# k2-fsa/Flow2GAN

Hardware: AMD Instinct MI355X
Metric: audio-seconds/sec (train step, G+D fwd/bwd) mel_24k_base (higher is better)
Workload: dtype f32 (fp32-class products on the bf16 matrix pipe for the long reductions and the direct MRD convs: every fp32 operand as three bf16 pieces = 24 significand bits, the six v_mfma_f32_32x32x16_bf16 products with i + j <= 2 per fp32 product, fp32 accumulate, error <= 2^-23 per product; short reductions ; 1 GPU; mel_24k_base GAN stage-2 train step: D-step + G-step, each on its own batch (MPD+MRD+FM+multi-scale mel), fwd+bwd+grad all-reduce, no optimizer (metric is fwd/bwd); per_gpu_batch=64, gan=gan_multi_scale_mel_recon, parallelism=dp1, optimizer=none

## Files before the change

### flow2gan_amd/csrc/multi.hip

```cpp
#include "common.h"
#include "split_f16.h"

namespace {

__device__ __forceinline__ void run_fill(const f2g_multi_entry& e, long long b, long long nb) {
  float* x = reinterpret_cast<float*>(e.out);
  const long long n = ((long long)e.n[1] << 32) | (unsigned)e.n[0];
  const float v = __int_as_float((int)e.s[0]);
  for (long long i = b * 256 + threadIdx.x; i < n; i += nb * 256) x[i] = v;
}

__device__ __forceinline__ void run_permute4(const f2g_multi_entry& e, long long b, long long nb) {
  float* out = reinterpret_cast<float*>(e.out);
  const float* in = reinterpret_cast<const float*>(e.in);
  const int n1 = e.n[1], n2 = e.n[2], n3 = e.n[3];
  const long long total = (long long)e.n[0] * n1 * n2 * n3;
  for (long long i = b * 256 + threadIdx.x; i < total; i += nb * 256) {
    long long r = i;
    const int i3 = (int)(r % n3); r /= n3;
    const int i2 = (int)(r % n2); r /= n2;
    const int i1 = (int)(r % n1); r /= n1;
    out[i] = in[r * e.s[0] + i1 * e.s[1] + i2 * e.s[2] + i3 * e.s[3]];
  }
}

__device__ __forceinline__ void run_copy3(const f2g_multi_entry& e, long long b, long long nb) {
  float* out = reinterpret_cast<float*>(e.out);
  const float* in = reinterpret_cast<const float*>(e.in);
  const int n1 = e.n[1], n2 = e.n[2], acc = e.n[3];
  const long long total = (long long)e.n[0] * n1 * n2;
  for (long long i = b * 256 + threadIdx.x; i < total; i += nb * 256) {
    const int c = (int)(i % n2);
    const long long q = i / n2;
    const int r = (int)(q % n1);
    const long long bb = q / n1;
    const float v = in[bb * e.s[2] + r * e.s[3] + c];
    float* o = out + bb * e.s[0] + r * e.s[1] + c;
    *o = acc ? *o + v : v;
  }
}

__device__ __forceinline__ void run_split3(const f2g_multi_entry& e, long long b, long long nb) {
  __bf16* dst = reinterpret_cast<__bf16*>(e.out);
  const float* src = reinterpret_cast<const float*>(e.in);
  const int K = e.n[1];
  const long long rows = e.n[0], ld = e.s[0], total = rows * (K / 4);
  for (long long i = b * 256 + threadIdx.x; i < total; i += nb * 256) {
    const long long r = i / (K / 4);
    const int k4 = (int)(i - r * (K / 4)) * 4;
    const float4 v = *reinterpret_cast<const float4*>(src + r * ld + k4);
    const float x[4] = {v.x, v.y, v.z, v.w};
    unsigned short p[3][4];
#pragma unroll
    for (int q = 0; q < 4; ++q) {
      const __bf16 a = (__bf16)x[q];
      const float r1 = x[q] - (float)a;
      const __bf16 c = (__bf16)r1;
      const __bf16 d = (__bf16)(r1 - (float)c);
      p[0][q] = __builtin_bit_cast(unsigned short, a);
      p[1][q] = __builtin_bit_cast(unsigned short, c);
      p[2][q] = __builtin_bit_cast(unsigned short, d);
    }
    __bf16* o = dst + (r * (K / 32) + k4 / 32) * 96 + (k4 & 31);
#pragma unroll
    for (int q = 0; q < 3; ++q)
      *reinterpret_cast<uint2*>(o + 32 * q) =
          make_uint2(p[q][0] | ((unsigned)p[q][1] << 16), p[q][2] | ((unsigned)p[q][3] << 16));
  }
}

__device__ __forceinline__ void run_split3g(const f2g_multi_entry& e, long long b, long long nb) {
  unsigned char* dst = reinterpret_cast<unsigned char*>(e.out);
  const float* src = reinterpret_cast<const float*>(e.in);
  const int K = e.n[1], K8 = K / 8, T = K / 32;
  const long long rows = e.n[0], ld = e.s[0], total = rows * K8;
  for (long long i = b * 256 + threadIdx.x; i < total; i += nb * 256) {
    const int li = (int)(i & 31);
    const long long q = i >> 5;
    const int c8 = (int)(q % K8);
    const long long j = q / K8;
    const float* p = src + (j * 32 + li) * ld + c8 * 8;
    const float4 v0 = *reinterpret_cast<const float4*>(p), v1 = *reinterpret_cast<const float4*>(p + 4);
    unsigned a[3], bq[3], c[3], dq[3];
    f2g_split3_pair(v0.x, v0.y, a[0], a[1], a[2]);
    f2g_split3_pair(v0.z, v0.w, bq[0], bq[1], bq[2]);
    f2g_split3_pair(v1.x, v1.y, c[0], c[1], c[2]);
    f2g_split3_pair(v1.z, v1.w, dq[0], dq[1], dq[2]);
    unsigned char* o = dst + ((((j * T + (c8 >> 2)) * 12 + (c8 & 3)) * 32) + li) * 16;
#pragma unroll
    for (int pc = 0; pc < 3; ++pc)
      *reinterpret_cast<uint4*>(o + pc * (4 * 32 * 16)) = make_uint4(a[pc], bq[pc], c[pc], dq[pc]);
  }
}

__device__ __forceinline__ void run_split_f16(const f2g_multi_entry& e, long long b, long long nb) {
  float* dst = reinterpret_cast<float*>(e.out);
  f2g_split_f16x2_rows<false>(dst, dst + e.s[1], reinterpret_cast<const float*>(e.in), e.s[0], e.n[0], e.n[1],
                       b * 4 + (threadIdx.x >> 6), nb * 4);
}

__global__ __launch_bounds__(256) void multi_kernel(const f2g_multi_desc d) {
  int i = 0;
  long long first = 0;
  while (i + 1 < d.n && (long long)blockIdx.x >= first + d.e[i].blocks) first += d.e[i++].blocks;
  const f2g_multi_entry& e = d.e[i];
  const long long b = (long long)blockIdx.x - first, nb = e.blocks;
  switch (e.kind) {
    case F2G_MULTI_FILL: run_fill(e, b, nb); break;
    case F2G_MULTI_PERMUTE4: run_permute4(e, b, nb); break;
    case F2G_MULTI_COPY3: run_copy3(e, b, nb); break;
    case F2G_MULTI_SPLIT3: run_split3(e, b, nb); break;
    case F2G_MULTI_SPLIT_F16: run_split_f16(e, b, nb); break;
    default: run_split3g(e, b, nb); break;
  }
}

}

extern "C" int f2g_multi(const f2g_multi_desc* d, f2g_stream_t stream) {
  if (!d || d->n < 0 || d->n > F2G_MULTI_MAX) return F2G_EINVAL;
  long long grid = 0;
  for (int i = 0; i < d->n; ++i) {
    const f2g_multi_entry& e = d->e[i];
    if (!e.out || (e.kind != F2G_MULTI_FILL && !e.in) || e.blocks < 1 || e.kind < 0 || e.kind > F2G_MULTI_SPLIT_F16)
      return F2G_EINVAL;
    if (e.kind == F2G_MULTI_SPLIT3G && (e.n[0] & 31)) return F2G_EINVAL;
    if ((e.kind == F2G_MULTI_SPLIT3 || e.kind == F2G_MULTI_SPLIT3G) &&
        (e.n[1] < 32 || (e.n[1] % 32) || e.s[0] < e.n[1] || (e.s[0] & 3) || (((uintptr_t)e.in) & 15) ||
         (((uintptr_t)e.out) & 15)))
      return F2G_EINVAL;
    if (e.kind == F2G_MULTI_SPLIT_F16 &&
        (e.n[0] < 0 || e.n[1] < 32 || (e.n[1] % 32) || e.n[1] > F2G_F16_MAX_K || e.s[0] < e.n[1] || (e.s[0] & 3) ||
         e.s[1] <= 0 || (((uintptr_t)e.in) & 15) || (((uintptr_t)e.out) & 15)))
      return F2G_EINVAL;
    grid += e.blocks;
  }
  if (grid == 0) return F2G_OK;
  if (grid >= (1ll << 31)) return F2G_EINVAL;
  hipLaunchKernelGGL(multi_kernel, dim3((unsigned)grid), dim3(256), 0, (hipStream_t)stream, *d);
  return f2g_check_launch();
}
```

### flow2gan_amd/fused.py

```python
from __future__ import annotations

import os
import random
from typing import List, Optional

import torch

from . import ops
from .models.modules import dft_matrices
from .ops import gemm, mat, win1d

LIMIT_PROB = 0.6


def _limit_draw(training: bool) -> bool:
    return bool(training and random.random() < LIMIT_PROB)


def frames_lens(audio_lens_cpu: Optional[List[int]], hop: int, device):
    if audio_lens_cpu is None:
        return None
    return torch.tensor([1 + int(l) // hop for l in audio_lens_cpu], dtype=torch.int32,
                        device=device)


BLOCK_KEYS = ("dwconv.weight", "dwconv.bias", "norm.log_scale", "norm.bias", "pwconv1.weight",
              "pwconv1.bias", "act.weight", "pwconv2.weight", "pwconv2.bias",
              "residual_scale.scale")


def block_params(blk) -> list:
    return [blk.dwconv.weight, blk.dwconv.bias, blk.norm.log_scale, blk.norm.bias,
            blk.pwconv1.weight, blk.pwconv1.bias, blk.act.weight, blk.pwconv2.weight,
            blk.pwconv2.bias, blk.residual_scale.scale]


class _Blk:

    __slots__ = ("w_dw", "b_dw", "log_scale", "beta", "w1", "b1", "alpha", "w2", "b2", "gamma",
                 "C", "H", "K")

    def __init__(self, p: list):
        (self.w_dw, self.b_dw, self.log_scale, self.beta, self.w1, self.b1, self.alpha, self.w2,
         self.b2, self.gamma) = p
        self.C = self.w_dw.shape[0]
        self.K = self.w_dw.shape[2]
        self.H = self.w1.shape[0]


_APPLY_GRAD = True

GRAD_SINK = None


def sink_register(params):
    sink = GRAD_SINK
    if sink is None or not _APPLY_GRAD:
        return None
    key = sink.add_use(params)
    return None if key is None else (sink, key)


def deliver_grads(ticket, params, grads):
    if ticket is None:
        return grads
    sink, key = ticket
    if GRAD_SINK is not sink:
        return grads
    sink.deliver(key, params, grads)
    return [None] * len(grads)


class GradAwareFunction(torch.autograd.Function):

    @classmethod
    def apply(cls, *args):
        global _APPLY_GRAD
        prev = _APPLY_GRAD
        _APPLY_GRAD = torch.is_grad_enabled()
        try:
            return super().apply(*args)
        finally:
            _APPLY_GRAD = prev


def _keep(ctx) -> bool:
    return _APPLY_GRAD and any(ctx.needs_input_grad)


def block_fwd(bp: _Blk, x, B, F, lens, cproj=None, ldcp=0, Fc=0, up=1, cp_off=0, te=None, ldte=0,
              te_off=0, keep: bool = True):
    dev = x.device
    rows, Cc, Hh = B * F, bp.C, bp.H
    fmt = ops.operand_formats_ok(Cc, Hh)
    if fmt == 2 and not keep and bp.K == 7 and ops.fused_mlp_applies(Cc, Hh) \
            and x.stride(0) % 4 == 0:
        out = ops.empty(rows, Cc, device=dev)
        ops.fused_block(x, B, F, Cc, bp.K, lens, bp.w_dw, bp.b_dw, bp.beta, bp.log_scale.reshape(1),
                        ops.mlp_pack(bp.w1, bp.w2), bp.b1, bp.alpha, bp.b2, bp.gamma.reshape(Cc), out,
                        Hh, cproj, ldcp, Fc, up, cp_off, te, ldte, te_off)
        return out, None, (None, None, None, 0)
    if fmt == 2 and not keep:
        z = torch.empty(rows, Cc, device=dev, dtype=torch.bfloat16)
        ops.dwnorm_fwd(x, z, B, F, Cc, bp.K, lens, bp.w_dw, bp.b_dw, bp.beta, bp.log_scale.reshape(1),
                       cproj, ldcp, Fc, up, cp_off, te, ldte, te_off, z_format=2)
        if ops.fused_mlp_applies(Cc, Hh):
            out = ops.empty(rows, Cc, device=dev)
            ops.fused_mlp(z, ops.mlp_pack(bp.w1, bp.w2), bp.b1,
                          bp.alpha, bp.b2, x, bp.gamma.reshape(Cc), out, rows, Cc, Hh)
            return out, z, (None, None, None, 0)
        a = torch.empty(rows, Hh, device=dev, dtype=torch.bfloat16)
        gemm(mat(z, rows, Cc, split=2), mat(bp.w1.reshape(Hh, Cc)), a, bias=bp.b1, prelu=bp.alpha,
             split_k=1)
        out = ops.empty(rows, Cc, device=dev)
        gemm(mat(a, rows, Hh, split=2), mat(bp.w2.reshape(Cc, Hh)), out, bias=bp.b2, res=x,
             gamma=bp.gamma.reshape(Cc))
        return out, z, (a, a, None, 0)
    zsplit = 1 if fmt == 1 else 0
    z = ops.empty(rows, Cc, device=dev)
    ops.dwnorm_fwd(x, z, B, F, Cc, bp.K, lens, bp.w_dw, bp.b_dw, bp.beta, bp.log_scale.reshape(1),
                   cproj, ldcp, Fc, up, cp_off, te, ldte, te_off, z_format=zsplit)
    a = ops.empty(rows, Hh, device=dev)
    if keep:
        p = ops.empty(rows, Hh, device=dev)
        share = ops.split_sharing(z, p)
        with share:
            gemm(mat(z, rows, Cc, split=zsplit), mat(bp.w1.reshape(Hh, Cc)), a, bias=bp.b1,
                 prelu=bp.alpha, prelu_out=p)
            out = ops.empty(rows, Cc, device=dev)
            gemm(mat(p, rows, Hh), mat(bp.w2.reshape(Cc, Hh)), out, bias=bp.b2, res=x,
                 gamma=bp.gamma.reshape(Cc))
        return out, z, (a, p, share, zsplit)
    p = a
    gemm(mat(z, rows, Cc, split=zsplit), mat(bp.w1.reshape(Hh, Cc)), a, bias=bp.b1, prelu=bp.alpha)
    out = ops.empty(rows, Cc, device=dev)
    gemm(mat(p, rows, Hh), mat(bp.w2.reshape(Cc, Hh)), out, bias=bp.b2, res=x,
         gamma=bp.gamma.reshape(Cc))
    return out, z, (a, p, None, zsplit)


def block_bwd(bp: _Blk, x, z, a, gout, B, F, lens, limit_norm: bool, limit_scale: bool,
              cproj=None, ldcp=0, Fc=0, up=1, cp_off=0, te=None, ldte=0, te_off=0, g_cproj=None,
              g_te=None, g_cproj_store=False):
    a, p_act, share, zsplit = a
    if share is None:
        share = ops.split_sharing()
    dev = x.device
    rows, Cc, Hh = B * F, bp.C, bp.H
    (g_w2, g_b2, g_alpha, g_b1, g_w1, g_beta, g_ls, g_wdw, g_bdw, g_gamma) = ops.zeros_many(
        [(Cc, Hh), (Cc,), (Hh,), (Hh,), (Hh, Cc), (Cc,), (1,), (Cc, 1, bp.K), (Cc,), (Cc, 1)], dev)
    ops.colsum(g_b2, gout, rows, Cc)
    with share, ops.split_sharing(gout):
        ops.wgrad(gout, Cc, gout.stride(0), mat(p_act, rows, Hh), g_w2)
        gemm(mat(gout, rows, Cc), mat(bp.w2.reshape(Cc, Hh)), a, form=1, aux=a, alpha_n=bp.alpha,
             colsum_alpha=g_alpha, colsum=g_b1)
    with share, ops.split_sharing(a):
        ops.wgrad(a, Hh, a.stride(0), mat(z, rows, Cc, split=zsplit), g_w1)
        gemm(mat(a, rows, Hh), mat(bp.w1.reshape(Hh, Cc)), z, form=1)
    share.drop()
    du = ops.empty(rows, Cc, device=dev)
    ops.dwnorm_bwd(x, z, du, B, F, Cc, bp.K, lens, bp.w_dw, bp.b_dw, bp.beta,
                   bp.log_scale.reshape(1), cproj, ldcp, Fc, up, cp_off, te, ldte, te_off,
                   g_cproj=g_cproj, g_te=g_te, g_beta=g_beta, g_log_scale=g_ls,
                   g_cproj_store=g_cproj_store)
    gx = ops.empty(rows, Cc, device=dev)
    ops.dwconv_bwd(du, x, gx, B, F, Cc, bp.K, lens, bp.w_dw, gres=gout, gamma=bp.gamma.reshape(Cc),
                   g_w=g_wdw, g_b=g_bdw, g_gamma=g_gamma)
    if limit_norm:
        ops.limit_grad(g_ls, bp.log_scale.reshape(1), -1.5, 1.5)
    if limit_scale:
        ops.limit_grad(g_gamma, bp.gamma, 0.5, 1.0)
    grads = [g_wdw, g_bdw, g_ls.reshape(()), g_beta, g_w1.reshape(Hh, Cc, 1), g_b1, g_alpha,
             g_w2.reshape(Cc, Hh, 1), g_b2, g_gamma]
    return gx, grads


def cond_encoder_params(enc) -> list:
    p = [enc.in_proj.weight, enc.in_proj.bias, enc.in_norm.log_scale, enc.in_norm.bias]
    for blk in enc.blocks:
        p += block_params(blk)
    return p


class CondEncoderFn(GradAwareFunction):

    @staticmethod
    def forward(ctx, mel, training: bool, lens_cpu, *params):
        dev = mel.device
        B, nm, Fm = mel.shape
        lens = None if lens_cpu is None else torch.tensor([int(v) for v in lens_cpu], dtype=torch.int32,
                                                          device=dev)
        w_in, b_in, ls_in, beta_in = params[:4]
        Cc = w_in.shape[0]
        nblk = (len(params) - 4) // len(BLOCK_KEYS)
        blks = [_Blk(list(params[4 + i * 10: 14 + i * 10])) for i in range(nblk)]
        rows = B * Fm
        melr = ops.empty(rows, nm, device=dev)
        ops.bct_to_rows(melr, mel.contiguous(), B, nm, Fm)
        wp = ops.empty(Cc, 3 * nm, device=dev)
        ops.permute4(wp, w_in, (Cc, 3, nm, 1), (nm * 3, 1, 3, 0))
        h0 = ops.empty(rows, Cc, device=dev)
        gemm(win1d(melr, B, Fm, nm, Fm, 1, 1, 3), mat(wp), h0, bias=b_in)
        flags = [_limit_draw(training)]
        x = ops.empty(rows, Cc, device=dev)
        ops.biasnorm_fwd(h0, x, rows, Cc, beta_in, ls_in.reshape(1))
        saved = []
        for bp in blks:
            fn = _limit_draw(training)
            y, z, a = block_fwd(bp, x, B, Fm, lens, keep=_keep(ctx))
            flags.append((fn, _limit_draw(training)))
            saved.append((x, z, a))
            x = y
        if _keep(ctx):
            ctx.saved = (melr, wp, h0, saved)
            ctx.params = params
            ctx.dims = (B, nm, Fm, Cc)
            ctx.flags = flags
            ctx.lens = lens
        return x

    @staticmethod
    def backward(ctx, g):
        melr, wp, h0, saved = ctx.saved
        params = ctx.params
        B, nm, Fm, Cc = ctx.dims
        dev = g.device
        rows = B * Fm
        w_in, b_in, ls_in, beta_in = params[:4]
        nblk = len(saved)
        blks = [_Blk(list(params[4 + i * 10: 14 + i * 10])) for i in range(nblk)]
        g = g.contiguous()
        grads_blocks = [None] * nblk
        for i in reversed(range(nblk)):
            x, z, a = saved[i]
            fn, fs = ctx.flags[1 + i]
            g, gb = block_bwd(blks[i], x, z, a, g, B, Fm, ctx.lens, fn, fs)
            grads_blocks[i] = gb
        g_beta, g_ls, g_bin, g_wp = ops.zeros_many([(Cc,), (1,), (Cc,), (Cc, 3 * nm)], dev)
        gh0 = ops.empty(rows, Cc, device=dev)
        ops.biasnorm_bwd(h0, g, gh0, rows, Cc, beta_in, ls_in.reshape(1), g_beta, g_ls)
        if ctx.flags[0]:
            ops.limit_grad(g_ls, ls_in.reshape(1), -1.5, 1.5)
        ops.colsum(g_bin, gh0, rows, Cc)
        ops.wgrad(gh0, Cc, gh0.stride(0), win1d(melr, B, Fm, nm, Fm, 1, 1, 3), g_wp)
        g_win = ops.empty(Cc, nm, 3, device=dev)
        ops.permute4(g_win, g_wp, (Cc, nm, 3, 1), (3 * nm, 1, nm, 0))
        g_mel = None
        if ctx.needs_input_grad[0]:
            gw = ops.empty(rows, 3 * nm, device=dev)
            gemm(mat(gh0, rows, Cc), mat(wp), gw, form=1)
            gm = ops.zeros(rows, nm, device=dev)
            for tap in range(3):
                sh = tap - 1
                f0, n = max(0, -sh), Fm - abs(sh)
                if n > 0:
                    ops.copy3(gm, Fm * nm, nm, gw, Fm * 3 * nm, 3 * nm, B, n, nm, accumulate=True,
                              out_offset=(f0 + sh) * nm, in_offset=f0 * 3 * nm + tap * nm)
            g_mel = ops.rows_to_bct(ops.empty(B, nm, Fm, device=dev), gm, B, nm, Fm)
        out = [g_mel, None, None, g_win, g_bin, g_ls.reshape(()), g_beta]
        for gb in grads_blocks:
            out += gb
        ctx.saved = None
        return tuple(out)


def cond_path_params(dec) -> list:
    p = [dec.cond_mlp[0].weight, dec.cond_mlp[0].bias, dec.cond_mlp[1].weight,
         dec.cond_mlp[2].weight, dec.cond_mlp[2].bias]
    for blk in dec.blocks:
        p += [blk.cond_proj.weight, blk.cond_proj.bias]
    return p


def _stack_rows(ws, cols, dev):
    def build(ts):
        Cc = ts[0].shape[0]
        out = ops.empty(len(ts) * Cc, cols, device=dev)
        for j, w in enumerate(ts):
            ops.copy3(out, 0, cols, w, 0, cols, 1, Cc, cols, out_offset=j * Cc * cols)
        return out
    return ops.derived_multi(list(ws), ("stack_rows", cols), build)


def _stack_vecs(bs, dev):
    def build(ts):
        Cc = ts[0].shape[0]
        out = ops.empty(len(ts) * Cc, device=dev)
        for j, b in enumerate(ts):
            ops.copy3(out, 0, 0, b, 0, 0, 1, 1, Cc, out_offset=j * Cc)
        return out
    return ops.derived_multi(list(bs), "stack_vecs", build)


class CondPathFn(GradAwareFunction):

    @staticmethod
    def forward(ctx, cond, B: int, Fc: int, Fce: int, *params):
        dev = cond.device
        w0, b0, alpha, w2, b2 = params[:5]
        wcs, bcs = list(params[5::2]), list(params[6::2])
        Dc, Hc = w0.shape[1], w0.shape[0]
        Cc, nblk = wcs[0].shape[0], len(wcs)
        if Fce == Fc:
            cext = cond
        else:
            cext = ops.zeros(B * Fce, Dc, device=dev)
            n = min(Fc, Fce)
            ops.copy3(cext, Fce * Dc, Dc, cond, Fc * Dc, Dc, B, n, Dc)
        rows = B * Fce
        keep = _keep(ctx)
        wstack = _stack_rows(wcs, Dc, dev)
        bstack = _stack_vecs(bcs, dev)
        cproj = ops.empty(rows, nblk * Cc, device=dev)
        if (not keep) and ops.GEMM_PRECISION == 2 and Dc % 64 == 0 and Hc % 64 == 0:
            a = torch.empty(rows, Hc, device=dev, dtype=torch.bfloat16)
            gemm(mat(cext, rows, Dc), mat(w0.reshape(Hc, Dc)), a, bias=b0, prelu=alpha, split_k=1)
            cm = torch.empty(rows, Dc, device=dev, dtype=torch.bfloat16)
            gemm(mat(a, rows, Hc, split=2), mat(w2.reshape(Dc, Hc)), cm, bias=b2, split_k=1)
            gemm(mat(cm, rows, Dc, split=2), mat(wstack), cproj, bias=bstack)
            return cproj
        a = ops.empty(rows, Hc, device=dev)
        pact = ops.empty(rows, Hc, device=dev) if keep else a
        gemm(mat(cext, rows, Dc), mat(w0.reshape(Hc, Dc)), a, bias=b0, prelu=alpha,
             prelu_out=pact if keep else None)
        cm = ops.empty(rows, Dc, device=dev)
        gemm(mat(pact, rows, Hc), mat(w2.reshape(Dc, Hc)), cm, bias=b2)
        gemm(mat(cm, rows, Dc), mat(wstack), cproj, bias=bstack)
        if keep:
            ctx.saved = (cext, (a, pact), cm, wstack)
            ctx.params = params
            ctx.dims = (B, Fc, Fce, Dc, Hc, Cc, nblk)
        return cproj

    @staticmethod
    def backward(ctx, g):
        cext, (a, pact), cm, wstack = ctx.saved
        params = ctx.params
        B, Fc, Fce, Dc, Hc, Cc, nblk = ctx.dims
        w0, b0, alpha, w2, b2 = params[:5]
        dev = g.device
        rows = B * Fce
        g = g.contiguous()
        NC = nblk * Cc
        g_wstack, g_bstack, g_b2, g_w2, g_alpha, g_b0, g_w0 = ops.zeros_many(
            [(NC, Dc), (NC,), (Dc,), (Dc, Hc), (Hc,), (Hc,), (Hc, Dc)], dev)
        ops.colsum(g_bstack, g, rows, NC)
        ops.wgrad(g, NC, g.stride(0), mat(cm, rows, Dc), g_wstack)
        g_cm = ops.empty(rows, Dc, device=dev)
        gemm(mat(g, rows, NC), mat(wstack), g_cm, form=1)
        ops.colsum(g_b2, g_cm, rows, Dc)
        ops.wgrad(g_cm, Dc, g_cm.stride(0), mat(pact, rows, Hc), g_w2)
        gemm(mat(g_cm, rows, Dc), mat(w2.reshape(Dc, Hc)), a, form=1, aux=a, alpha_n=alpha,
             colsum_alpha=g_alpha, colsum=g_b0)
        ops.wgrad(a, Hc, a.stride(0), mat(cext, rows, Dc), g_w0)
        g_cond = None
        if ctx.needs_input_grad[0]:
            g_cext = ops.empty(rows, Dc, device=dev)
            gemm(mat(a, rows, Hc), mat(w0.reshape(Hc, Dc)), g_cext, form=1)
            if Fce == Fc:
                g_cond = g_cext
            else:
                g_cond = ops.zeros(B * Fc, Dc, device=dev)
                n = min(Fc, Fce)
                ops.copy3(g_cond, Fc * Dc, Dc, g_cext, Fce * Dc, Dc, B, n, Dc)
        out = [g_cond, None, None, None, g_w0.reshape(Hc, Dc, 1), g_b0, g_alpha,
               g_w2.reshape(Dc, Hc, 1), g_b2]
        for j in range(nblk):
            out.append(g_wstack[j * Cc:(j + 1) * Cc].reshape(Cc, Dc, 1))
            out.append(g_bstack[j * Cc:(j + 1) * Cc])
        ctx.saved = None
        return tuple(out)


def decoder_params(d) -> list:
    p = [d.in_proj.weight, d.in_proj.bias, d.in_norm.log_scale, d.in_norm.bias,
         d.time_mlp[0].weight, d.time_mlp[0].bias, d.time_mlp[2].weight, d.time_mlp[2].bias,
         d.out_proj.weight, d.out_proj.bias]
    for blk in d.blocks:
        p += block_params(blk) + [blk.time_embed_proj.weight, blk.time_embed_proj.bias]
    return p


def branch_params(est) -> list:
    return decoder_params(est.decoder)


N_BRANCH_HEAD = 10
N_PER_BLOCK = 12


class _BranchView:
    def __init__(self, params: list):
        (self.w_in, self.b_in, self.ls_in, self.beta_in, self.tw0, self.tb0, self.tw2, self.tb2,
         self.w_out, self.b_out) = params[:N_BRANCH_HEAD]
        rest = params[N_BRANCH_HEAD:]
        self.nblk = len(rest) // N_PER_BLOCK
        self.blks = [_Blk(list(rest[i * N_PER_BLOCK: i * N_PER_BLOCK + 10]))
                     for i in range(self.nblk)]
        self.tew = [rest[i * N_PER_BLOCK + 10] for i in range(self.nblk)]
        self.teb = [rest[i * N_PER_BLOCK + 11] for i in range(self.nblk)]
        self.C = self.w_in.shape[0]
        self.Cin = self.w_in.shape[1]
        self.Dt = self.tw0.shape[1]
        self.Ht = self.tw0.shape[0]


def _spec_ld(Cin: int) -> int:
    return (Cin + 63) // 64 * 64


def _pad_cols(w2d, Kp: int):
    def build(t):
        n, k = t.shape
        out = ops.zeros(n, Kp, device=t.device)
        ops.copy3(out, 0, Kp, t, 0, t.stride(0), 1, n, k)
        return out
    return w2d if w2d.shape[1] == Kp else ops.derived(w2d, ("padc", Kp), build)


def _pad_rows(w2d, Np: int):
    def build(t):
        n, k = t.shape
        out = ops.zeros(Np, k, device=t.device)
        ops.copy3(out, 0, k, t, 0, t.stride(0), 1, n, k)
        return out
    return w2d if w2d.shape[0] == Np else ops.derived(w2d, ("padr", Np), build)


def _pad_vec(b, Np: int):
    def build(t):
        out = ops.zeros(Np, device=t.device)
        ops.copy3(out, 0, 0, t, 0, 0, 1, 1, t.shape[0])
        return out
    return b if b.shape[0] == Np else ops.derived(b, ("padv", Np), build)


def _time_path(bv: _BranchView, t):
    dev = t.device
    n = t.shape[0]
    Dt, Ht = bv.Dt, bv.Ht
    emb = ops.empty(n, Dt, device=dev)
    ops.time_embedding(emb, t, Dt)
    th = ops.empty(n, Ht, device=dev)
    gemm(mat(emb), mat(bv.tw0), th, bias=bv.tb0)
    ts = ops.empty(n, Ht, device=dev)
    ops.silu(ts, th)
    te = ops.empty(n, Dt, device=dev)
    gemm(mat(ts), mat(bv.tw2), te, bias=bv.tb2)
    tew = _stack_rows(bv.tew, Dt, dev)
    teb = _stack_vecs(bv.teb, dev)
    te_all = ops.empty(n, bv.nblk * bv.C, device=dev)
    gemm(mat(te), mat(tew), te_all, bias=teb)
    return emb, th, ts, te, tew, te_all


def time_path_bwd(bv: _BranchView, tp, g_te_all, B: int, acc):
    emb, th, ts, te, tew, _ = tp
    g_tew, g_teb, g_tb2, g_tw2, g_tb0, g_tw0 = acc
    dev = g_te_all.device
    Dt, Ht, NC = bv.Dt, bv.Ht, bv.nblk * bv.C
    ops.colsum(g_teb, g_te_all, B, NC)
    ops.wgrad(g_te_all, NC, NC, mat(te, B, Dt), g_tew)
    g_te = ops.empty(B, Dt, device=dev)
    gemm(mat(g_te_all, B, NC), mat(tew), g_te, form=1)
    ops.colsum(g_tb2, g_te, B, Dt)
    ops.wgrad(g_te, Dt, Dt, mat(ts, B, Ht), g_tw2)
    g_ts = ops.empty(B, Ht, device=dev)
    gemm(mat(g_te, B, Dt), mat(bv.tw2), g_ts, form=1)
    g_th = ops.empty(B, Ht, device=dev)
    ops.silu_bwd(g_th, g_ts, th)
    ops.colsum(g_tb0, g_th, B, Ht)
    ops.wgrad(g_th, Ht, Ht, mat(emb, B, Dt), g_tw0)


def time_paths_ahead(flat, nparams, t_all, n_steps: int):
    dev = t_all.device
    nb = len(nparams)
    B = t_all.shape[0] // n_steps
    views, off = [], 0
    for i in range(nb):
        views.append(_BranchView(list(flat[off: off + nparams[i]])))
        off += nparams[i]
    lanes = ops.Lanes(dev, nb, "timepath")
    full = []
    for i in range(nb):
        with lanes.lane(i):
            full.append(_time_path(views[i], t_all)[-1])
    return lanes, [[full[i][k * B: (k + 1) * B] for i in range(nb)] for k in range(n_steps)]


def _branch_pre(bv: _BranchView, meta, x, t, cproj, training, keep, te_pre=None):
    n_fft, hop, up, window = meta
    dev = x.device
    B, T = x.shape
    N = n_fft
    F = 1 + T // hop
    rows = B * F
    Cc, Cin = bv.C, bv.Cin
    Wd, Wi = dft_matrices(N, dev)
    ldp = _spec_ld(Cin)
    bf16_chain = (not keep) and ops.GEMM_PRECISION == 2 and N % 64 == 0
    if ops.fft_applies(N):
        packed = torch.empty(rows, ldp, device=dev, dtype=torch.bfloat16) if bf16_chain \
            else ops.empty(rows, ldp, device=dev)
        ops.stft_fft(x, N, hop, F, packed, zero_pad=True)
        pk = mat(packed, rows, ldp, split=2 if bf16_chain else 0)
    elif bf16_chain:
        packed = torch.empty(rows, ldp, device=dev, dtype=torch.bfloat16)
        gemm(ops.stft_frames(x, N, hop, F), mat(_pad_rows(Wd, ldp)), packed, split_k=1, true_n=Cin)
        pk = mat(packed, rows, ldp, split=2)
    else:
        packed = ops.empty(rows, ldp, device=dev)
        gemm(ops.stft_frames(x, N, hop, F), mat(_pad_rows(Wd, ldp)), packed, split_k=1, true_n=Cin)
        pk = mat(packed, rows, ldp)
    h0 = ops.empty(rows, Cc, device=dev)
    gemm(pk, mat(_pad_cols(bv.w_in.reshape(Cc, Cin), ldp)), h0, bias=bv.b_in, split_k=1, true_k=Cin)
    flags = [_limit_draw(training)]
    xcur = ops.empty(rows, Cc, device=dev)
    ops.biasnorm_fwd(h0, xcur, rows, Cc, bv.beta_in, bv.ls_in.reshape(1))
    NC = bv.nblk * Cc
    if te_pre is not None:
        emb = th = ts = te = tew = None
        te_all = te_pre
    else:
        emb, th, ts, te, tew, te_all = _time_path(bv, t)
    return dict(packed=packed, h0=h0, xcur=xcur, emb=emb, th=th, ts=ts, te=te, tew=tew, te_all=te_all,
                flags=flags, F=F, rows=rows, NC=NC, Fce=cproj.shape[0] // B, ldp=ldp,
                bf16_chain=bf16_chain, blocks=[])


def _branch_post(st, bv: _BranchView, meta, x_shape, wbranch_row, wscale, pred, accumulate, lens_f,
                 lanes=None, ola: bool = True):
    n_fft, hop, up, window = meta
    B, T = x_shape
    N, F, rows, ldp = n_fft, st["F"], st["rows"], st["ldp"]
    Cc, Cin = bv.C, bv.Cin
    xcur = st["xcur"]
    dev = xcur.device
    Wd, Wi = dft_matrices(N, dev)
    ifft = ops.fft_applies(N)
    ybf = st["bf16_chain"] and lens_f is None
    yspec = torch.empty(rows, ldp, device=dev, dtype=torch.bfloat16) if ybf else ops.empty(rows, ldp, device=dev)
    gemm(mat(xcur, rows, Cc), mat(_pad_rows(bv.w_out.reshape(Cin, Cc), ldp)), yspec,
         bias=_pad_vec(bv.b_out, ldp), split_k=1, true_n=Cin)
    if lens_f is not None:
        ops.mask_rows(yspec, B, F, Cin, lens_f)
    frames = ops.empty(rows, N, device=dev)
    if ifft:
        ops.istft_fft(yspec, N, F, frames)
    else:
        gemm(mat(yspec, rows, ldp, split=2 if ybf else 0), mat(_pad_cols(Wi, ldp)), frames, split_k=1, true_k=Cin)
    if not ola:
        return frames
    if lanes is not None:
        lanes.chain_enter()
    ops.istft_ola(frames, pred, B, F, N, hop, T, window, wbranch_row, wscale, accumulate)
    if lanes is not None:
        lanes.chain_leave()
    return None


def _branch_forward(bv: _BranchView, meta, x, t, cproj, wbranch_row, wscale, pred, accumulate,
                    lens_f, training, keep, lanes=None, te_pre=None):
    up = meta[2]
    B = x.shape[0]
    st = _branch_pre(bv, meta, x, t, cproj, training, keep, te_pre)
    Cc, F, NC = bv.C, st["F"], st["NC"]
    xcur = st["xcur"]
    for j, bp in enumerate(bv.blks):
        fn = _limit_draw(training)
        y, z, a = block_fwd(bp, xcur, B, F, lens_f, cproj, NC, st["Fce"], up, j * Cc, st["te_all"], NC,
                            j * Cc, keep=keep)
        st["flags"].append((fn, _limit_draw(training)))
        if keep:
            st["blocks"].append((xcur, z, a))
        xcur = y
    st["xcur"] = xcur
    _branch_post(st, bv, meta, x.shape, wbranch_row, wscale, pred, accumulate, lens_f, lanes)
    if keep:
        return dict(packed=st["packed"], h0=st["h0"], blocks=st["blocks"], x_last=xcur, emb=st["emb"],
                    th=st["th"], ts=st["ts"], te=st["te"], tew=st["tew"], te_all=st["te_all"],
                    flags=st["flags"], F=F)
    return None


def _multi_applies(views, x, keep) -> bool:
    if keep or not ops.FUSED_MULTI:
        return False
    if not (2 <= len(views) <= 4) or len({bv.nblk for bv in views}) != 1:
        return False
    for bv in views:
        for bp in bv.blks:
            if ops.operand_formats_ok(bp.C, bp.H) != 2 or bp.K != 7 or not ops.fused_mlp_applies(bp.C, bp.H):
                return False
    return True


def _branches_forward_multi(views, metas, x, t, cprojs, wbranch, wscale, pred, lens_list, training,
                            te_pre=None):
    nb = len(views)
    dev = x.device
    B = x.shape[0]
    sts = [None] * nb
    lanes = ops.Lanes(dev, nb, "branch")
    for i in range(nb):
        with lanes.lane(i):
            sts[i] = _branch_pre(views[i], metas[i], x, t, cprojs[i], training, False,
                                 None if te_pre is None else te_pre[i])
            for _ in range(2 * views[i].nblk):
                _limit_draw(training)
    lanes.join()
    for j in range(views[0].nblk):
        entries = []
        for i in range(nb):
            bv, st = views[i], sts[i]
            bp = bv.blks[j]
            Cc = bv.C
            entries.append(dict(
                x=st["xcur"], B=B, F=st["F"], Cc=Cc, K=bp.K, lens=lens_list[i], w_dw=bp.w_dw, b_dw=bp.b_dw,
                beta=bp.beta, log_scale=bp.log_scale.reshape(1), wp=ops.mlp_pack(bp.w1, bp.w2), b1=bp.b1,
                alpha=bp.alpha, b2=bp.b2, gamma=bp.gamma.reshape(Cc), out=ops.empty(st["rows"], Cc, device=dev),
                Hh=bp.H, cproj=cprojs[i], ldcp=st["NC"], Fc=st["Fce"], up=metas[i][2], cp_off=j * Cc,
                te=st["te_all"], ldte=st["NC"], te_off=j * Cc))
        outs = ops.fused_block_multi(entries)
        for i in range(nb):
            sts[i]["xcur"] = outs[i]
    lanes = ops.Lanes(dev, nb, "branch")
    frames = [None] * nb
    for i in range(nb):
        with lanes.lane(i):
            frames[i] = _branch_post(sts[i], views[i], metas[i], x.shape, None, wscale, pred, i > 0,
                                     lens_list[i], lanes, ola=False)
    lanes.join()
    ops.istft_ola_multi([(frames[i], sts[i]["F"], metas[i][0], metas[i][1], metas[i][3],
                          None if wbranch is None else wbranch[i]) for i in range(nb)],
                        pred, B, x.shape[1], wscale)


def _branch_backward(bv: _BranchView, meta, sv, x_shape, cproj, g_pred, wbranch_row, wscale,
                     lens_f, g_x, accumulate_gx, g_cproj, need_gx, lanes=None):
    n_fft, hop, up, window = meta
    dev = g_pred.device
    B, T = x_shape
    N = n_fft
    F = sv["F"]
    rows = B * F
    Cc, Cin = bv.C, bv.Cin
    NC = bv.nblk * Cc
    Wd, Wi = dft_matrices(N, dev)
    ldp = _spec_ld(Cin)
    Fce = cproj.shape[0] // B
    gfr = ops.empty(rows, N, device=dev)
    ops.istft_ola_bwd(g_pred, gfr, B, F, N, hop, T, window, wbranch_row, wscale)
    if ops.fft_applies(N):
        gy = ops.empty(rows, ldp, device=dev)
        ops.istft_fft_adjoint(gfr, N, F, gy, zero_pad=True)
    else:
        gy = ops.empty(rows, ldp, device=dev)
        gemm(mat(gfr, rows, N), mat(_pad_cols(Wi, ldp)), gy, form=1, true_n=Cin)
    if lens_f is not None:
        ops.mask_rows(gy, B, F, Cin, lens_f)
    Dt, Ht = bv.Dt, bv.Ht
    (g_wout, g_bout, g_te_all, g_beta, g_ls, g_bin, g_win, g_tew, g_teb, g_tb2, g_tw2, g_tb0,
     g_tw0) = ops.zeros_many([(Cin, Cc), (Cin,), (B, NC), (Cc,), (1,), (Cc,), (Cc, Cin), (NC, Dt), (NC,), (Dt,),
                              (Dt, Ht), (Ht,), (Ht, Dt)], dev)
    ops.colsum(g_bout, gy, rows, Cin)
    x_last = sv["x_last"]
    ops.wgrad(gy, Cin, ldp, mat(x_last, rows, Cc), g_wout)
    g = ops.empty(rows, Cc, device=dev)
    gemm(mat(gy, rows, ldp), mat(_pad_rows(bv.w_out.reshape(Cin, Cc), ldp)), g, form=1, true_k=Cin)
    block_grads = [None] * bv.nblk
    flags = sv["flags"]
    for j in reversed(range(bv.nblk)):
        xj, z, a = sv["blocks"][j]
        fn, fs = flags[1 + j]
        g, gb = block_bwd(bv.blks[j], xj, z, a, g, B, F, lens_f, fn, fs, cproj, NC, Fce, up,
                          j * Cc, sv["te_all"], NC, j * Cc, g_cproj=g_cproj, g_te=g_te_all,
                          g_cproj_store=True)
        block_grads[j] = gb
    gh0 = ops.empty(rows, Cc, device=dev)
    ops.biasnorm_bwd(sv["h0"], g, gh0, rows, Cc, bv.beta_in, bv.ls_in.reshape(1), g_beta, g_ls)
    if flags[0]:
        ops.limit_grad(g_ls, bv.ls_in.reshape(1), -1.5, 1.5)
    ops.colsum(g_bin, gh0, rows, Cc)
    ops.wgrad(gh0, Cc, gh0.stride(0), mat(sv["packed"], rows, Cin), g_win)
    if need_gx:
        gpacked = ops.empty(rows, ldp, device=dev)
        gemm(mat(gh0, rows, Cc), mat(_pad_cols(bv.w_in.reshape(Cc, Cin), ldp)), gpacked, form=1, true_n=Cin)
        gxf = ops.empty(rows, N, device=dev)
        if ops.fft_applies(N):
            ops.stft_fft_adjoint(gpacked, N, F, gxf)
        else:
            gemm(mat(gpacked, rows, ldp), mat(_pad_rows(Wd, ldp)), gxf, form=1, true_k=Cin)
        if lanes is not None:
            lanes.chain_enter()
        ops.frames_fold(gxf, g_x, B, F, N, hop, T, accumulate_gx)
        if lanes is not None:
            lanes.chain_leave()
    time_path_bwd(bv, (sv["emb"], sv["th"], sv["ts"], sv["te"], sv["tew"], sv["te_all"]), g_te_all, B,
                  (g_tew, g_teb, g_tb2, g_tw2, g_tb0, g_tw0))
    out = [g_win.reshape(Cc, Cin, 1), g_bin, g_ls.reshape(()), g_beta, g_tw0, g_tb0, g_tw2, g_tb2,
           g_wout.reshape(Cin, Cc, 1), g_bout]
    for j in range(bv.nblk):
        out += block_grads[j]
        out.append(g_tew[j * Cc:(j + 1) * Cc])
        out.append(g_teb[j * Cc:(j + 1) * Cc])
    return out


class ModelEvalFn(GradAwareFunction):

    @staticmethod
    def forward(ctx, x, t, wbranch, metas, lens_cpu, training: bool, nparams, *args):
        bscale = None
        te_pre = None
        if metas and metas[-1][0] == "te":
            te_pre = metas[-1][1]
            metas = metas[:-1]
        if metas and metas[-1][0] == "scale":
            bscale = float(metas[-1][1])
            metas = metas[:-1]
        nb = len(metas)
        if bscale is None:
            bscale = 1.0 / nb
        cprojs = list(args[:nb])
        flat = args[nb:]
        dev = x.device
        x = x.contiguous()
        B, T = x.shape
        pred = ops.empty(B, T, device=dev)
        keep = _keep(ctx)
        saved, views, lens_list = [], [], []
        off = 0
        for i in range(nb):
            views.append(_BranchView(list(flat[off: off + nparams[i]])))
            off += nparams[i]
            lens_list.append(frames_lens(lens_cpu, metas[i][1], dev))
            dft_matrices(metas[i][0], dev)
        if keep:
            te_pre = None
        if _multi_applies(views, x, keep):
            _branches_forward_multi(views, metas, x, t, cprojs, wbranch, bscale, pred, lens_list, training,
                                    te_pre)
            saved = [None] * nb
        else:
            lanes = ops.Lanes(dev, nb, "branch")
            for i in range(nb):
                wrow = None if wbranch is None else wbranch[i]
                with lanes.lane(i):
                    sv = _branch_forward(views[i], metas[i], x, t, cprojs[i], wrow, bscale, pred,
                                         i > 0, lens_list[i], training, keep, lanes,
                                         None if te_pre is None else te_pre[i])
                saved.append(sv)
            lanes.join()
        if keep:
            ctx.tickets = [sink_register(list(flat[sum(nparams[:i]): sum(nparams[:i + 1])]))
                           for i in range(nb)]
            ctx.flat = flat
            ctx.saved = saved
            ctx.views = views
            ctx.lens = lens_list
            ctx.x_shape = (B, T)
            ctx.cprojs = cprojs
            ctx.wbranch = wbranch
            ctx.metas = metas
            ctx.bscale = bscale
            ctx.nparams = nparams
        return pred

    @staticmethod
    def backward(ctx, g_pred):
        nb = len(ctx.metas)
        dev = g_pred.device
        g_pred = g_pred.contiguous()
        B, T = ctx.x_shape
        need_gx = ctx.needs_input_grad[0]
        g_x = ops.empty(B, T, device=dev) if need_gx else None
        g_cprojs, g_flat = [], []
        lanes = ops.Lanes(dev, nb, "branch")
        for i in range(nb):
            cproj = ctx.cprojs[i]
            need_gc = ctx.needs_input_grad[7 + i]
            wrow = None if ctx.wbranch is None else ctx.wbranch[i]
            with lanes.lane(i):
                g_cp = ops.zeros(cproj.shape[0], cproj.shape[1], device=dev) if need_gc else None
                gl = _branch_backward(ctx.views[i], ctx.metas[i], ctx.saved[i], (B, T), cproj,
                                      g_pred, wrow, ctx.bscale, ctx.lens[i], g_x, i > 0, g_cp,
                                      need_gx, lanes)
                off = sum(ctx.nparams[:i])
                g_flat += deliver_grads(ctx.tickets[i], list(ctx.flat[off: off + ctx.nparams[i]]), gl)
            g_cprojs.append(g_cp)
        lanes.join()
        ctx.saved = None
        ctx.flat = None
        return tuple([g_x, None, None, None, None, None, None] + g_cprojs + g_flat)


class AxpbyFn(torch.autograd.Function):

    @staticmethod
    def forward(ctx, x0, x1, a: float, b: float):
        ctx.ab = (a, b)
        y = torch.empty_like(x0)
        return ops.axpby_rows(y, x0.contiguous(), x1.contiguous(), sa=a, sb=b)

    @staticmethod
    def backward(ctx, g):
        a, b = ctx.ab
        g = g.contiguous()
        g0 = g1 = None
        if ctx.needs_input_grad[0]:
            g0 = ops.axpby_rows(torch.empty_like(g), g, None, sa=a)
        if ctx.needs_input_grad[1]:
            g1 = ops.axpby_rows(torch.empty_like(g), g, None, sa=b)
        return g0, g1, None, None


def stft_packed(x, n_fft: int, hop: int):
    dev = x.device
    B, T = x.shape
    F = 1 + T // hop
    Wd, _ = dft_matrices(n_fft, dev)
    packed = ops.empty(B * F, ops.pad4(n_fft + 2), device=dev)
    if ops.fft_applies(n_fft):
        ops.stft_fft(x, n_fft, hop, F, packed)
    else:
        gemm(ops.stft_frames(x, n_fft, hop, F), mat(Wd), packed, split_k=1)
    return packed, F


def filterbank_spec(x, n_fft: int, hop: int, fb, power: int):
    dev = x.device
    packed, F = stft_packed(x, n_fft, hop)
    rows = packed.shape[0]
    nb = n_fft // 2 + 1
    spec = ops.empty(rows, ops.pad4(nb), device=dev)
    ops.spec_power(spec, packed, rows, nb, power)
# ... 107 lines not shown
```

### flow2gan_amd/fused_disc.py

```python
from __future__ import annotations

from typing import List

import torch

from . import ops
from .fused import deliver_grads, filterbank_spec, filterbank_spec_bwd, sink_register
from .models.modules import dft_matrices
from .ops import gemm, mat, win1d, win2d

SLOPE = 0.1


def stack_pair(real, fake):
    B, T = real.shape
    x2 = ops.empty(2 * B, T, device=real.device)
    ops.copy3(x2, 0, T, real.contiguous(), 0, T, 1, B, T)
    ops.copy3(x2, 0, T, fake.contiguous(), 0, T, 1, B, T, out_offset=B * T)
    return x2


def pack_conv_weight(w):
    Cout, Cin, kh, kw = w.shape
    out = ops.empty(Cout, kh * kw * Cin, device=w.device)
    ops.permute4(out, w, (Cout, kh * kw, Cin, 1), (Cin * kh * kw, 1, kh * kw, 0))
    return out


def unpack_conv_grad(gp, shape):
    Cout, Cin, kh, kw = shape
    out = ops.empty(Cout, Cin, kh, kw, device=gp.device)
    ops.permute4(out, gp, (Cout, Cin, kh * kw, 1), (Cin * kh * kw, 1, Cin, 0))
    return out


def _residues(k: int, stride: int, pad: int, n_in: int):
    out = []
    for rho in range(stride):
        j0 = (rho + pad) % stride
        nt = len(range(j0, k, stride))
        e0 = (rho + pad - j0) // stride
        Lq = (n_in - rho + stride - 1) // stride
        out.append((rho, j0, nt, e0, max(Lq, 0)))
    return out


MPD_CH = (1, 32, 128, 512, 1024, 1024)
MPD_STRIDE = (3, 3, 3, 3, 1)


def mpd_params(mpd) -> list:
    p = []
    for d in mpd.discriminators:
        for c in d.convs:
            p += [c.weight, c.bias]
        p += [d.conv_post.weight, d.conv_post.bias]
    return p


HALO = 2


def _halo_rows(S: int, H: int, Cc: int, dev, x3: bool = False):
    buf = ops.empty(S * (H + 2 * HALO), Cc, device=dev)
    if Cc % 4 == 0:
        ops.zero_halo(buf, S, H + 2 * HALO, Cc, HALO, HALO)
    else:
        ops.fill_(buf, 0.0)
    if x3:
        ops.x3_reserve(buf, (S, H + 2 * HALO, Cc, HALO, HALO))
    return buf


def _halo_map(H: int, Cc: int):
    return (H, (H + 2 * HALO) * Cc, Cc, HALO * Cc)


def unhalo(y, S: int, H: int):
    return y.view(S, H + 2 * HALO, y.shape[1])[:, HALO:HALO + H]


def _mpd_forward_one(x2, p: int, prm: list, keep_images: bool = False):
    dev = x2.device
    S2, T = x2.shape
    H = (T + p - 1) // p
    S = S2 * p
    img = ops.empty(S * H, 1, device=dev)
    ops.period_fold(img, x2, S2, T, p, H)
    acts, hs = [img], [H]
    shares = [None] * 6
    x = img
    for l in range(5):
        w, b = prm[2 * l], prm[2 * l + 1]
        Cin, Cout, st = MPD_CH[l], MPD_CH[l + 1], MPD_STRIDE[l]
        Hout = (H + 4 - 5) // st + 1
        wp = ops.derived(w, "pack", pack_conv_weight)
        y = _halo_rows(S, Hout, Cout, dev, x3=(0 < l < 4))
        if l == 0:
            ops.mpd0_fwd(x, S, H, Hout, HALO, w.reshape(Cout, 5), b, SLOPE, y)
        else:
            A = win1d(x, S, H + 2 * HALO, Cin, Hout, st, 0, 5)
            if keep_images:
                shares[l] = ops.split_sharing(x)
                with shares[l]:
                    gemm(A, mat(wp), y, bias=b, lrelu=SLOPE, rowmap=_halo_map(Hout, Cout), x3_out=(l < 4))
            else:
                gemm(A, mat(wp), y, bias=b, lrelu=SLOPE, rowmap=_halo_map(Hout, Cout), x3_out=(l < 4))
        acts.append(y)
        hs.append(Hout)
        x, H = y, Hout
    wpost, bpost = prm[10], prm[11]
    wpp = ops.derived(wpost, "pack", pack_conv_weight)
    scores = ops.empty(S * H, 1, device=dev)
    ops.mpdpost_fwd(x, S, H, HALO, wpp, bpost, scores)
    return dict(acts=acts, hs=hs, scores=scores, S=S, p=p, shares=shares)


def _dgrad_weight(w, stride: int, j0: int, nt: int):
    def build(t):
        Cout, Cin, K = t.shape[0], t.shape[1], t.shape[2] * t.shape[3]
        out = ops.empty(Cin, nt * Cout, device=t.device)
        ops.permute4(out, t, (Cin, nt, Cout, 1), (K, -stride, Cin * K, 0),
                     in_offset=j0 + stride * (nt - 1))
        return out
    return ops.derived(w, ("dgradT", stride, j0, nt), build)


def _conv1d_dgrad(g_pre, S, Hout, Cout, w, stride, pad, Hin, mask=None, fm=None, colsum=None):
    Cin, K = w.shape[1], w.shape[2] * w.shape[3]
    dev = g_pre.device
    want_img = 2 * Cin >= ops.X6_MIN_K
    gx = _halo_rows(S, Hin, Cin, dev, x3=want_img)
    for rho, j0, nt, e0, Lq in _residues(K, stride, pad, Hin):
        if Lq == 0:
            continue
        wq = _dgrad_weight(w, stride, j0, nt)
        wpad = (nt - 1) - e0
        A = win1d(g_pre, S, Hout + 2 * HALO, Cout, Lq, 1, wpad - HALO, nt)
        rm = (Lq, (Hin + 2 * HALO) * Cin, stride * Cin, (HALO + rho) * Cin)
        gemm(A, mat(wq), gx, rowmap=rm, mask=mask, fm=fm, colsum=colsum, x3_out=want_img)
    return gx


class MPDFusedLanding:

    def __init__(self, st, Sx: int, roff: int, g1, train_disc: bool):
        self.acts, self.hs, self.Sx, self.roff, self.g1, self.train_disc = st["acts"], st["hs"], Sx, roff, g1, train_disc

    def __call__(self, l_out, producer, cs):
        y, Sx, g1 = self.acts[l_out], self.Sx, self.g1
        Hp_, C_ = self.hs[l_out] + 2 * HALO, y.shape[1]
        mk = (y, self.roff * Hp_ * C_, SLOPE)
        fk = None
        if (not self.train_disc) and l_out >= 2:
            fk = (y, 0, 1.0 / (Sx * self.hs[l_out] * C_), g1)
        if l_out == 5 or (ops.GEMM_PRECISION == 3 and l_out in (3, 4)):
            return producer(mk, fk, cs)
        gm = producer(None, None, None)
        gm._f2g_x3_bad = True
        n_ = Sx * Hp_ * C_
        if self.train_disc:
            ops.lrelu_bwd_colsum(gm, y, None, 0.0, SLOPE, Sx * Hp_, C_, C_, cs, y_off=mk[1])
        elif fk is not None:
            ops.lrelu_bwd(gm, y, y, fk[2], SLOPE, 1, n_, n_, wdev=g1, y_off=mk[1], r_off=0)
        else:
            ops.lrelu_bwd(gm, y, None, 0.0, SLOPE, 1, n_, n_, y_off=mk[1])
        return gm


class MPDUpstreamLanding:

    def __init__(self, st, B: int, ups: dict):
        self.acts, self.hs, self.S, self.p, self.B, self.ups = st["acts"], st["hs"], st["S"], st["p"], B, ups

    def __call__(self, l_out, producer, cs):
        gm = producer(None, None, None)
        gm._f2g_x3_bad = True
        y, Hl, p = self.acts[l_out], self.hs[l_out], self.p
        Hp_, C_ = Hl + 2 * HALO, y.shape[1]
        u = self.ups.get(l_out)
        if u is not None:
            ub, uc, uh, uw = u.stride()
            ops.lrelu_bwd_add(gm, y, (self.B, p, Hl), (p * Hp_ * C_, Hp_ * C_, C_), C_, u, (ub, uw, uh, uc),
                              SLOPE, colsum=cs, g_off=HALO * C_)
        elif cs is not None:
            ops.lrelu_bwd_colsum(gm, y, None, 0.0, SLOPE, self.S * Hp_, C_, C_, cs)
        else:
            n_ = self.S * Hp_ * C_
            ops.lrelu_bwd(gm, y, None, 0.0, SLOPE, 1, n_, n_)
        return gm


def _mpd_backward_one(st, prm: list, gs, seqs, need_w: bool, need_x: bool, land, top: int = 4):
    acts, hs, S = st["acts"], st["hs"], st["S"]
    Sx, roff = seqs
    dev = acts[0].device
    grads_p = [None] * 12
    unpack = []
    zbuf = None
    if need_w:
        zshapes = [(1, 3 * 1024), (1,)]
        for l in range(5):
            zshapes += [(MPD_CH[l + 1], 5 * MPD_CH[l]), (MPD_CH[l + 1],)]
        zbuf = ops.zeros_many(zshapes, dev)

    def bias_acc(l_out):
        return zbuf[2 * l_out + 1] if need_w else None

    if gs is not None:
        H5, wpost = hs[5], prm[10]
        if need_w:
            ops.mpdpost_wgrad(acts[5], S, H5, HALO, gs, zbuf[0])
            unpack.append((10, zbuf[0], wpost.shape))
            ops.colsum(zbuf[1], gs, S * H5, 1)
            grads_p[11] = zbuf[1]
        g = land(5, lambda mk, fk, ck: ops.mpdpost_dgrad(
            gs, Sx, H5, HALO, ops.derived(wpost, "pack", pack_conv_weight),
            _halo_rows(Sx, H5, 1024, dev, x3=mk is not None), g_off=roff * H5, mask=mk, fm=fk, colsum=ck), bias_acc(5))
        top = 4
    else:
        g = land(top + 1, lambda mk, fk, ck: ops.zeros(Sx * (hs[top + 1] + 2 * HALO), MPD_CH[top + 1], device=dev),
                 bias_acc(top + 1))
    for l in reversed(range(top + 1)):
        w = prm[2 * l]
        Cin, Cout, stv = MPD_CH[l], MPD_CH[l + 1], MPD_STRIDE[l]
        Hin, Hout = hs[l], hs[l + 1]
        Hp = Hout + 2 * HALO
        with ops.split_sharing(g), (st["shares"][l] or ops.split_sharing()):
            if need_w:
                grads_p[2 * l + 1] = zbuf[2 + 2 * l + 1]
                gwp = zbuf[2 + 2 * l]
                if l == 0:
                    ops.mpd0_wgrad(acts[0], S, Hin, Hout, HALO, g, gwp)
                else:
                    X = win1d(acts[l], S, Hin + 2 * HALO, Cin, Hp, stv, HALO * stv, 5,
                              unbounded=True)
                    ops.wgrad(g, Cout, Cout, X, gwp)
                unpack.append((2 * l, gwp, w.shape))
            if l > 0:
                g = land(l, lambda mk, fk, ck: _conv1d_dgrad(g, Sx, Hout, Cout, w, stv, 2, Hin, mask=mk, fm=fk,
                                                             colsum=ck), bias_acc(l))
            elif need_x:
                gx0 = ops.empty(Sx * Hin, 1, device=dev)
                g = ops.mpd0_dgrad(g, Sx, Hin, Hout, HALO, w.reshape(Cout, 5), gx0)
    if need_w:
        with ops.weight_batch():
            for slot_, gwp_, shape_ in unpack:
                grads_p[slot_] = unpack_conv_grad(gwp_, shape_)
    return (g if need_x else None), grads_p


class MPDLossFn(torch.autograd.Function):

    @staticmethod
    def forward(ctx, real, fake, train_disc: bool, periods, *params):
        dev = real.device
        B, T = real.shape
        x2 = stack_pair(real, fake)
        losses = ops.zeros(2, device=dev)
        saved = []
        lanes = ops.Lanes(dev, len(periods), "mpd")
        for i, p in enumerate(periods):
          with lanes.lane(i):
            prm = list(params[12 * i: 12 * i + 12])
            st = _mpd_forward_one(x2, p, prm, keep_images=train_disc)
            S, H5 = st["S"], st["hs"][5]
            nh = (S // 2) * H5
            sc = st["scores"]
            if train_disc:
                ops.hinge_loss(losses, None, sc, nh, -1.0, 1.0 / nh)
                ops.hinge_loss(losses, None, sc, nh, +1.0, 1.0 / nh, s_off=nh)
            else:
                ops.hinge_loss(losses, None, sc, nh, -1.0, 1.0 / nh, s_off=nh)
                for l in range(2, 6):
                    y = st["acts"][l]
                    Hl, Cl = st["hs"][l], y.shape[1]
                    nflat = (S // 2) * (Hl + 2 * HALO) * Cl
                    nval = (S // 2) * Hl * Cl
                    ops.l1_loss_ab(losses, None, y, 0, y, nflat, 1, nflat, nflat, 1.0 / nval,
                                   loss_offset=1)
                ops.l1_loss_ab(losses, None, sc, 0, sc, nh, 1, nh, nh, 1.0 / nh, loss_offset=1)
            saved.append(st)
        lanes.join()
        ctx.saved = saved
        ctx.params = params
        ctx.meta = (B, T, train_disc, tuple(periods))
        ctx.tickets = [sink_register(list(params[12 * i: 12 * i + 12])) if train_disc else None
                       for i in range(len(periods))]
        return losses[0], losses[1]

    @staticmethod
    def backward(ctx, g0, g1):
        B, T, train_disc, periods = ctx.meta
        params = ctx.params
        dev = g0.device
        g0 = g0.reshape(1).contiguous()
        g1 = g1.reshape(1).contiguous()
        pgrads: List = []
        g_fake = None if train_disc else ops.zeros(B, T, device=dev)
        lanes = ops.Lanes(dev, len(periods), "mpd")
        for i, p in enumerate(periods):
          with lanes.lane(i):
            prm = list(params[12 * i: 12 * i + 12])
            st = ctx.saved[i]
            sc, S = st["scores"], st["S"]
            H5 = st["hs"][5]
            nh = (S // 2) * H5
            gs = ops.empty(S * H5, 1, device=dev)
            if train_disc:
                ops.hinge_loss(None, gs, sc, nh, -1.0, 1.0 / nh, wdev=g0)
                ops.hinge_loss(None, gs, sc, nh, +1.0, 1.0 / nh, wdev=g0, s_off=nh)
                Sx, roff = S, 0
            else:
                ops.hinge_loss(None, gs, sc, nh, -1.0, 1.0 / nh, wdev=g0, s_off=nh)
                ops.lrelu_bwd(gs, sc, sc, 1.0 / nh, 1.0, 1, nh, nh, wdev=g1, g_off=nh, y_off=nh,
                              r_off=0)
                Sx, roff = S // 2, S // 2
            g, grads_p = _mpd_backward_one(st, prm, gs, (Sx, roff), train_disc, not train_disc,
                                           MPDFusedLanding(st, Sx, roff, g1, train_disc))
            if not train_disc:
                lanes.chain_enter()
                ops.period_fold_bwd(g_fake, g, B, T, p, st["hs"][0], True)
                lanes.chain_leave()
            pgrads += deliver_grads(ctx.tickets[i], prm, grads_p)
        lanes.join()
        ctx.saved = None
        return tuple([None, g_fake, None, None] + pgrads)


MRD_BANDS = ((0.0, 0.1), (0.1, 0.25), (0.25, 0.5), (0.5, 0.75), (0.75, 1.0))
MRD_LAYERS = ((9, 1), (9, 2), (9, 2), (9, 2), (3, 1))
MRD_CH = 32

_DFT_INT_CACHE = {}


def dft_interleaved(n_fft: int, device):
    key = (n_fft, str(device))
    if key not in _DFT_INT_CACHE:
        wd, _ = dft_matrices(n_fft, device)
        nb = n_fft // 2 + 1
        wi = torch.stack([wd[:nb], wd[nb:]], dim=1).reshape(2 * nb, n_fft).contiguous()
        wi._f2g_const = True
        _DFT_INT_CACHE[key] = wi
    return _DFT_INT_CACHE[key]


def mrd_params(mrd) -> list:
    p = []
    for d in mrd.discriminators:
        for stack in d.band_convs:
            for c in stack:
                p += [c.weight, c.bias]
        p += [d.conv_post.weight, d.conv_post.bias]
    return p


N_MRD_PARAMS = 5 * 5 * 2 + 2


def _band_edges(n_fft: int):
    nb = n_fft // 2 + 1
    return [(int(lo * nb), int(hi * nb)) for lo, hi in MRD_BANDS]


def _mrd_forward_one(x2, win: int, prm: list):
    dev = x2.device
    S, T = x2.shape
    hop = win // 4
    Ft = 1 + T // hop
    nb = win // 2 + 1
    xn = ops.empty(S, T, device=dev)
    stats = ops.empty(S, 3, device=dev)
    ops.peaknorm_fwd(xn, stats, x2, S, T)
    ldp = ops.pad4(2 * nb)
    packed = ops.empty(S * Ft, ldp, device=dev)
    if ops.fft_applies(win):
        ops.stft_fft(xn, win, hop, Ft, packed, interleaved=True)
    else:
        gemm(ops.stft_frames(xn, win, hop, Ft), mat(dft_interleaved(win, dev)),
             packed, split_k=1)
    bands = _band_edges(win)
    widths = []
    for lo, hi in bands:
        w = [hi - lo]
        for kw, sw in MRD_LAYERS:
            w.append((w[-1] + 2 * (kw // 2) - kw) // sw + 1)
        widths.append(w)
    Wcat = sum(w[5] for w in widths)
    cat = ops.empty(S * Ft * Wcat, MRD_CH, device=dev)
    acts = []
    foff = 0
    foffs = []
    for bi in range(len(bands)):
        foffs.append(foff)
        foff += widths[bi][5]
    for bi, (lo, hi) in enumerate(bands):
        foff = foffs[bi]
        ws = widths[bi]
# ... 12 lines not shown
            if l == 0 and ops.GEMM_PRECISION in (0, 1, 3):
                y = ops.empty(S * Ft * Wout, MRD_CH, device=dev)
                ops.conv2ch_fwd(packed, Ft * ldp, ldp, lo * 2, S, Ft, Win, wp, b, SLOPE, y)
            elif l in (1, 2, 3) and ops.GEMM_PRECISION in (0, 1, 3):
                y = ops.empty(S * Ft * Wout, MRD_CH, device=dev)
                ops.conv32_s2_fwd(x, S, Ft, Win, Wout, wp, b, SLOPE, y)
            elif l < 4:
                y = ops.empty(S * Ft * Wout, MRD_CH, device=dev)
                gemm(A, mat(wp), y, bias=b, lrelu=SLOPE)
            elif ops.GEMM_PRECISION == 3 and Wout <= ops.CONV33_MAX_W:
                y = None
                ops.conv33(x, S, Ft, Wout, wp, b, SLOPE, cat, y_off=foff * MRD_CH, y_line=Wcat * MRD_CH,
                           y_seq=Ft * Wcat * MRD_CH)
            else:
                y = None
                gemm(A, mat(wp), cat, bias=b, lrelu=SLOPE,
                     rowmap=(Wout, Wcat * MRD_CH, MRD_CH, foff * MRD_CH))
            layer_out.append(y)
            x, x_is_spec = y, False
        acts.append(layer_out)
    wpost, bpost = prm[50], prm[51]
    scores = ops.empty(S * Ft * Wcat, 1, device=dev)
    w9 = ops.derived(wpost, "pack", pack_conv_weight)
    if ops.GEMM_PRECISION in (0, 1, 3):
        ops.convpost_fwd(cat, S, Ft, Wcat, w9, bpost, scores)
    else:
        gemm(win2d(cat, S, Ft, Wcat, MRD_CH, Wcat, 3, 3, 1, 1, 1), mat(w9), scores, bias=bpost)
    return dict(xn=xn, stats=stats, packed=packed, ldp=ldp, Ft=Ft, nb=nb, hop=hop, bands=bands,
                widths=widths, Wcat=Wcat, cat=cat, acts=acts, scores=scores)


def _conv2d_dgrad(g_pre, S, H, Wout, Cout, w, sw, Win, gx, *, g_line=None, g_seq=None, g_off=0,
                  x_line=None, x_off=0, mask=None, fm=None, colsum=None):
    Cin, kh, kw = w.shape[1], w.shape[2], w.shape[3]
    dev = g_pre.device
    pw = kw // 2
    if (ops.GEMM_PRECISION in (0, 1, 3) and Cin == MRD_CH and Cout == MRD_CH and kw == 9
            and sw == 2 and x_line is None and x_off == 0):
        def build_t(t):
            out = ops.empty(kh * kw, Cin, Cout, device=t.device)
            ops.permute4(out, t, (kh * kw, Cin, Cout, 1), (1, kh * kw, Cin * kh * kw, 0))
            return out
        wT = ops.derived(w, "dgrad_taps", build_t)
        ops.conv32_s2_dgrad(g_pre, S, H, Win, Wout, wT, gx, g_seq=g_seq, g_line=g_line, g_off=g_off,
                            mask=mask, fm=fm, colsum=colsum)
        return gx
    if (ops.GEMM_PRECISION == 3 and Cin == MRD_CH and Cout == MRD_CH
            and kh == 3 and kw == 3 and sw == 1 and x_line is None and x_off == 0 and fm is None
            and Win <= ops.CONV33_MAX_W):
        def build_f(t):
            out = ops.empty(Cin, kh * kw * Cout, device=t.device)
            ops.permute4(out, t, (Cin, kh * kw, Cout, 1), (kh * kw, -1, Cin * kh * kw, 0), in_offset=kh * kw - 1)
            return out
        wf = ops.derived(w, "dgrad33", build_f)
        ops.conv33(g_pre, S, H, Win, wf, None, 0.0, gx, x_off=g_off, x_line=g_line, x_seq=g_seq, form=1,
                   mask=mask, colsum=colsum)
        return gx
    if x_line is None:
        x_line = Win * Cin
    for rho, j0, ntw, e0, Lq in _residues(kw, sw, pw, Win):
        if Lq == 0:
            continue
        def build(t, j0=j0, ntw=ntw):
            out = ops.empty(kh * ntw * Cout, Cin, device=t.device)
            ops.permute4(out, t, (kh, ntw, Cout, Cin), (-kw, -sw, Cin * kh * kw, kh * kw),
                         in_offset=(kh - 1) * kw + j0 + sw * (ntw - 1))
            return out
        wq = ops.derived(w, ("dgrad2d", sw, j0, ntw), build)
        A = win2d(g_pre, S, H, Wout, Cout, Lq, kh, ntw, 1, 1, (ntw - 1) - e0, line_stride=g_line,
                  seq_stride=g_seq, offset=g_off)
        gemm(A, mat(wq), gx, form=1, rowmap=(Lq, x_line, sw * Cin, x_off + rho * Cin), mask=mask,
             fm=fm, colsum=colsum)
    return gx


def _mrd_foffs(st) -> list:
    foffs, foff = [], 0
    for ws in st["widths"]:
        foffs.append(foff)
        foff += ws[5]
    return foffs


class MRDFusedLanding:
    fused = True

    def __init__(self, st, Sx: int, soff: int, g1, train_disc: bool):
        self.st, self.Sx, self.soff, self.g1, self.train_disc = st, Sx, soff, g1, train_disc
        self.foffs = _mrd_foffs(st)

    def __call__(self, bi, l_out, producer, cs):
        st, Sx, soff, g1, train_disc = self.st, self.Sx, self.soff, self.g1, self.train_disc
        Ft, C = st["Ft"], MRD_CH
        Wl = st["widths"][bi][l_out + 1]
        if l_out == 4:
            gcat, cat, ldc, foff = producer(None, None, None), st["cat"], st["Wcat"] * C, self.foffs[bi]
            y_off = soff * Ft * ldc + foff * C
            if train_disc:
                ops.lrelu_bwd(gcat, cat, None, 0.0, SLOPE, Sx * Ft, Wl * C, ldc, g_off=foff * C, y_off=y_off)
            else:
                ops.lrelu_bwd(gcat, cat, cat, 1.0 / (Sx * Ft * Wl * C), SLOPE, Sx * Ft, Wl * C, ldc,
                              wdev=g1, g_off=foff * C, y_off=y_off, r_off=foff * C)
            return gcat
        yb = st["acts"][bi][l_out]
        nb_ = Sx * Ft * Wl * C
        mk = (yb, soff * Ft * Wl * C, SLOPE)
        fmk = (yb, 0, 1.0 / nb_, g1) if ((not train_disc) and l_out >= 1) else None
        if (train_disc and ops.GEMM_PRECISION == 3 and ops.CONV32_X6
                and (l_out < 3 or Wl <= ops.CONV33_MAX_W)):
            return producer(mk, fmk, cs)
        gx = producer(None, None, None)
        if train_disc:
            ops.lrelu_bwd_colsum(gx, yb, None, 0.0, SLOPE, Sx * Ft * Wl, C, C, cs, y_off=mk[1])
        elif fmk is not None:
            ops.lrelu_bwd(gx, yb, yb, fmk[2], SLOPE, 1, nb_, nb_, wdev=g1, y_off=mk[1], r_off=0)
        else:
            ops.lrelu_bwd(gx, yb, None, 0.0, SLOPE, 1, nb_, nb_, y_off=mk[1])
        return gx


class MRDUpstreamLanding:
    fused = False

    def __init__(self, st, S: int, g_maps):
        self.st, self.S, self.g_maps = st, S, g_maps
        self.foffs = _mrd_foffs(st)

    def __call__(self, bi, l_out, producer, cs):
        st, S = self.st, self.S
        Ft, C = st["Ft"], MRD_CH
        Wl = st["widths"][bi][l_out + 1]
        gm = producer(None, None, None)
        u = self.g_maps[4 * bi + l_out - 1] if l_out >= 1 else None
        if l_out == 4:
            y, line, off = st["cat"], st["Wcat"] * C, self.foffs[bi] * C
        else:
            y, line, off = st["acts"][bi][l_out], Wl * C, 0
        if u is not None:
            ub, uc, uf, uw = u.stride()
            ops.lrelu_bwd_add(gm, y, (S, Ft, Wl), (Ft * line, line, C), C, u, (ub, uf, uw, uc), SLOPE,
                              colsum=cs, g_off=off)
        elif l_out == 4:
            ops.lrelu_bwd(gm, y, None, 0.0, SLOPE, S * Ft, Wl * C, line, g_off=off, y_off=off)
            if cs is not None:
                ops.colsum_strided(cs, gm, S * Ft, Wl, C, line, off)
        elif cs is not None:
            ops.lrelu_bwd_colsum(gm, y, None, 0.0, SLOPE, S * Ft * Wl, C, C, cs)
        else:
            nb_ = S * Ft * Wl * C
            ops.lrelu_bwd(gm, y, None, 0.0, SLOPE, 1, nb_, nb_)
        return gm


def _mrd_backward_one(st, prm: list, x, win: int, gs, seqs, need_w: bool, need_x: bool, land, tops=None):
    Ft, Wcat, nb, ldp, hop = st["Ft"], st["Wcat"], st["nb"], st["ldp"], st["hop"]
    cat, packed = st["cat"], st["packed"]
    S, T = x.shape
    Sx, soff = seqs
    dev = cat.device
    C = MRD_CH
    direct = ops.GEMM_PRECISION in (0, 1, 3)
    grads_w = [None] * N_MRD_PARAMS
    unpack = []
    gcat = None
    if gs is not None:
        wpost = prm[50]
        if need_w:
            if land.fused:
                gwp = ops.zeros(1, 9 * C, device=dev)
            else:
                gwp, gb = ops.zeros_many([(1, 9 * C), (1,)], dev)
            if direct:
                ops.convpost_wgrad(cat, S, Ft, Wcat, gs, gwp)
            else:
                ops.wgrad(gs, 1, 1, win2d(cat, S, Ft, Wcat, C, Wcat, 3, 3, 1, 1, 1), gwp)
            unpack.append((50, gwp, wpost.shape))
            if land.fused:
                gb = ops.zeros(1, device=dev)
            ops.colsum(gb, gs, S * Ft * Wcat, 1)
            grads_w[51] = gb
        gcat = ops.empty(Sx * Ft * Wcat, C, device=dev)
        if direct:
            ops.convpost_dgrad(gs, Sx, Ft, Wcat, ops.derived(wpost, "pack", pack_conv_weight),
                               gcat, g_off=soff * Ft * Wcat)
        else:
            _conv2d_dgrad(gs, Sx, Ft, Wcat, 1, wpost, 1, Wcat, gcat, g_off=soff * Ft * Wcat)
        tops = [4] * len(st["bands"])
    elif 4 in tops:
        gcat = ops.zeros(Sx * Ft * Wcat, C, device=dev)
    g_packed = None
    if need_x:
        g_packed = ops.empty(Sx * Ft, ldp, device=dev) if gs is not None else ops.zeros(Sx * Ft, ldp, device=dev)
    ldc = Wcat * C
    foffs = _mrd_foffs(st)

    def accumulators():
        return ops.zeros_many([(C,)] * 5 + [(C, 3 * kw_ * (2 if l_ == 0 else C))
                                            for l_, (kw_, _sw) in enumerate(MRD_LAYERS)], dev)

    for bi, (lo, hi) in enumerate(st["bands"]):
        foff, ws, top = foffs[bi], st["widths"][bi], tops[bi]
        if top is None:
            continue
        W4 = ws[5]
        gbs = [None] * 5
        if need_w and not land.fused:
            zs = accumulators()
            gbs, gwps = zs[:5], zs[5:]
        g = None
        if top == 4:
            land(bi, 4, lambda mk, fk, ck: gcat, gbs[4])
        else:
            g = land(bi, top, lambda mk, fk, ck: ops.zeros(Sx * Ft * ws[top + 1], C, device=dev), gbs[top])
        if need_w and land.fused:
            zs = accumulators()
            gbs, gwps = zs[:5], zs[5:]
        for l in reversed(range(top + 1)):
            kw, sw = MRD_LAYERS[l]
            w = prm[(bi * 5 + l) * 2]
            Cin = 2 if l == 0 else C
            Win, Wout = ws[l], ws[l + 1]
            if l == 4:
                dy_line, dy_seq, dy_off, dy_t = ldc, Ft * ldc, foff * C, gcat
            else:
                dy_line, dy_seq, dy_off, dy_t = None, None, 0, g
            if need_w:
                x_in = packed if l == 0 else st["acts"][bi][l - 1]
                if l == 0:
                    X = win2d(x_in, S, Ft, Win, Cin, Wout, 3, kw, sw, 1, kw // 2,
                              line_stride=ldp, seq_stride=Ft * ldp, offset=lo * 2)
                else:
                    X = win2d(x_in, S, Ft, Win, Cin, Wout, 3, kw, sw, 1, kw // 2)
                gwp = gwps[l]
                if l == 4:
                    dY = win1d(gcat, S * Ft, Wcat, C, W4, 1, -foff, 1)
                else:
                    dY = mat(g, S * Ft * Wout, C)
                tiles = ((3 * kw * Cin + 255) // 256)
                if l == 0 and direct:
                    ops.conv2ch_wgrad(packed, Ft * ldp, ldp, lo * 2, S, Ft, Win, g, gwp)
                elif l in (1, 2, 3) and direct:
                    ops.conv32_s2_wgrad(x_in, g, S, Ft, Win, Wout, gwp)
                elif (l == 4 and ops.GEMM_PRECISION == 3
                      and Wout <= ops.CONV33_MAX_W):
                    ops.conv33_wgrad(x_in, gcat, S, Ft, Wout, gwp, g_off=foff * C, g_line=ldc, g_seq=Ft * ldc)
                else:
                    gemm(dY, X, gwp, form=2, atomic=True,
                         split_k=ops.split_for(X.rows, tiles))
                unpack.append(((bi * 5 + l) * 2, gwp, w.shape))
                if l == 4 and land.fused:
                    ops.colsum_strided(gbs[4], gcat, S * Ft, W4, C, ldc, foff * C)
                grads_w[(bi * 5 + l) * 2 + 1] = gbs[l]
            if l > 0:
                gx = ops.empty(Sx * Ft * Win, Cin, device=dev)
                g = land(bi, l - 1, lambda mk, fk, ck: _conv2d_dgrad(
                    dy_t, Sx, Ft, Wout, C, w, sw, Win, gx, g_line=dy_line, g_seq=dy_seq, g_off=dy_off,
                    mask=mk, fm=fk, colsum=ck), gbs[l - 1])
            elif need_x and direct:
                def build_c2t(t):
                    out = ops.empty(27, 2, C, device=t.device)
                    ops.permute4(out, t, (27, 2, C, 1), (1, 27, 2 * 27, 0))
                    return out
                ops.conv2ch_dgrad(g, Sx, Ft, Win, ops.derived(w, "c2t", build_c2t), g_packed,
                                  Ft * ldp, ldp, lo * 2)
            elif need_x:
                _conv2d_dgrad(dy_t, Sx, Ft, Wout, C, w, sw, Win, g_packed, g_line=dy_line,
                              g_seq=dy_seq, g_off=dy_off, x_line=ldp, x_off=lo * 2)
    g_x = None
    if need_x:
        gfr = ops.empty(Sx * Ft, win, device=dev)
        if ops.fft_applies(win):
            ops.stft_fft_adjoint(g_packed, win, Ft, gfr, interleaved=True)
        else:
            gemm(mat(g_packed, Sx * Ft, 2 * nb), mat(dft_interleaved(win, dev)), gfr, form=1)
        gxn = ops.empty(Sx, T, device=dev)
        ops.frames_fold(gfr, gxn, Sx, Ft, win, hop, T, False)
        g_x = ops.empty(Sx, T, device=dev)
        ops.peaknorm_bwd(g_x, gxn, x, st["stats"], Sx, T, row_off=soff)
    if need_w:
        with ops.weight_batch():
            for slot_, gwp_, shape_ in unpack:
                grads_w[slot_] = unpack_conv_grad(gwp_, shape_)
    return g_x, grads_w


class MRDLossFn(torch.autograd.Function):

    @staticmethod
    def forward(ctx, real, fake, train_disc: bool, fft_sizes, *params):
        dev = real.device
        B, T = real.shape
        x2 = stack_pair(real, fake)
        losses = ops.zeros(2, device=dev)
        saved = []
        for win in fft_sizes:
            dft_interleaved(win, dev)
        lanes = ops.Lanes(dev, len(fft_sizes), "mrd")
        for i, win in enumerate(fft_sizes):
          with lanes.lane(i):
            prm = list(params[N_MRD_PARAMS * i: N_MRD_PARAMS * (i + 1)])
            st = _mrd_forward_one(x2, win, prm)
            Ft, Wcat = st["Ft"], st["Wcat"]
            nh = B * Ft * Wcat
            sc = st["scores"]
            if train_disc:
                ops.hinge_loss(losses, None, sc, nh, -1.0, 1.0 / nh)
                ops.hinge_loss(losses, None, sc, nh, +1.0, 1.0 / nh, s_off=nh)
            else:
                ops.hinge_loss(losses, None, sc, nh, -1.0, 1.0 / nh, s_off=nh)
                foff = 0
                for bi in range(5):
                    ws = st["widths"][bi]
                    for l in range(1, 4):
                        y = st["acts"][bi][l]
                        n = y.numel() // 2
                        ops.l1_loss_ab(losses, None, y, 0, y, n, 1, n, n, 1.0 / n, loss_offset=1)
                    cat = st["cat"]
                    cols = ws[5] * MRD_CH
                    ld = Wcat * MRD_CH
                    half = B * Ft * ld
                    ops.l1_loss_ab(losses, None, cat, foff * MRD_CH, cat, half + foff * MRD_CH,
                                   B * Ft, cols, ld, 1.0 / (B * Ft * cols), loss_offset=1)
                    foff += ws[5]
                ops.l1_loss_ab(losses, None, sc, 0, sc, nh, 1, nh, nh, 1.0 / nh, loss_offset=1)
            saved.append(st)
        lanes.join()
        ctx.saved = saved
        ctx.x2 = x2
        ctx.params = params
        ctx.meta = (B, T, train_disc, tuple(fft_sizes))
        return losses[0], losses[1]

    @staticmethod
    def backward(ctx, g0, g1):
        B, T, train_disc, fft_sizes = ctx.meta
        params = ctx.params
        dev = g0.device
        g0 = g0.reshape(1).contiguous()
        g1 = g1.reshape(1).contiguous()
        pgrads: List = []
        g_fake = None if train_disc else ops.zeros(B, T, device=dev)
        lanes = ops.Lanes(dev, len(fft_sizes), "mrd")
        for i, win in enumerate(fft_sizes):
          with lanes.lane(i):
            prm = list(params[N_MRD_PARAMS * i: N_MRD_PARAMS * (i + 1)])
            st = ctx.saved[i]
            sc = st["scores"]
            S = 2 * B
            nh = B * st["Ft"] * st["Wcat"]
            gs = ops.empty(S * st["Ft"] * st["Wcat"], 1, device=dev)
            if train_disc:
                ops.hinge_loss(None, gs, sc, nh, -1.0, 1.0 / nh, wdev=g0)
                ops.hinge_loss(None, gs, sc, nh, +1.0, 1.0 / nh, wdev=g0, s_off=nh)
                Sx, soff = S, 0
            else:
                ops.hinge_loss(None, gs, sc, nh, -1.0, 1.0 / nh, wdev=g0, s_off=nh)
                ops.lrelu_bwd(gs, sc, sc, 1.0 / nh, 1.0, 1, nh, nh, wdev=g1, g_off=nh, y_off=nh,
                              r_off=0)
                Sx, soff = B, B
            gx2, grads_w = _mrd_backward_one(st, prm, ctx.x2, win, gs, (Sx, soff), train_disc, not train_disc,
                                             MRDFusedLanding(st, Sx, soff, g1, train_disc))
            if not train_disc:
                lanes.chain_enter()
                ops.axpby_rows(g_fake, g_fake, gx2, sa=1.0, sb=1.0)
                lanes.chain_leave()
            pgrads += grads_w
        lanes.join()
        ctx.saved = None
        return tuple([None, g_fake, None, None] + pgrads)


class MelReconLossFn(torch.autograd.Function):

    @staticmethod
    def forward(ctx, real, fake, specs):
        dev = real.device
        B, T = real.shape
        x2 = stack_pair(real, fake)
        loss = ops.zeros(1, device=dev)
        saved = []
        for n_fft, hop, fb in specs:
            dft_matrices(n_fft, dev)
        lanes = ops.Lanes(dev, len(specs), "mel")
        for i, (n_fft, hop, fb) in enumerate(specs):
          with lanes.lane(i):
            S, packed, spec, F = filterbank_spec(x2, n_fft, hop, fb, 1)
            n = B * F * fb.shape[1]
            ops.l1_loss_ab(loss, None, S, 0, S, n, 1, n, n, 1.0 / n, clip=1e-7)
            saved.append((S, packed, F))
        lanes.join()
        ctx.saved = saved
        ctx.specs = specs
        ctx.dims = (B, T)
        return loss.reshape(())

    @staticmethod
    def backward(ctx, g):
        B, T = ctx.dims
        dev = g.device
        gw = g.reshape(1).contiguous()
        g_fake = ops.empty(B, T, device=dev)
        lanes = ops.Lanes(dev, len(ctx.specs), "mel")
        for i, (n_fft, hop, fb) in enumerate(ctx.specs):
          with lanes.lane(i):
            S, packed, F = ctx.saved[i]
            nm = fb.shape[1]
            n = B * F * nm
            gS = ops.empty(B * F, nm, device=dev)
            ops.call("f2g_l1_loss", None, ops.ptr(gS), ops.ptr(S), ops.ptr(S) + 4 * n, 1, n, n,
                     1.0 / n, 1e-7, ops.ptr(gw))
            filterbank_spec_bwd(gS, packed[B * F:], n_fft, hop, fb, 1, B, T, F, g_fake, i > 0,
                                lanes)
        lanes.join()
        ctx.saved = None
        return None, g_fake, None
```

### flow2gan_amd/leaf.py

```python
from __future__ import annotations

from typing import List, Optional

import torch

from . import fused, ops
from . import fused_disc as FD
from .fused import GradAwareFunction, _Blk, _BranchView, _keep, _limit_draw
from .ops import gemm, mat


class BctToRowsFn(torch.autograd.Function):

    @staticmethod
    def forward(ctx, x):
        B, Cc, F = x.shape
        ctx.dims = (B, Cc, F)
        rows = ops.empty(B * F, Cc, device=x.device)
        return ops.bct_to_rows(rows, x.contiguous().float(), B, Cc, F)

    @staticmethod
    def backward(ctx, g):
        B, Cc, F = ctx.dims
        g = g.contiguous()
# ... 98 lines not shown
    @staticmethod
    def backward(ctx, g):
        n_fft, hop, B, K, F, T = ctx.meta
        dev = g.device
        rows = B * F
        gfr = ops.empty(rows, n_fft, device=dev)
        ops.istft_ola_bwd(g.contiguous(), gfr, B, F, n_fft, hop, T, ctx.window, None, 1.0)
        ld = ops.pad4(2 * K)
        gy = ops.empty(rows, ld, device=dev)
        if ops.fft_applies(n_fft):
            ops.istft_fft_adjoint(gfr, n_fft, F, gy, zero_pad=True)
        else:
            _, Wi = fused.dft_matrices(n_fft, dev)
            gemm(mat(gfr, rows, n_fft), mat(Wi), gy, form=1)
        out = ops.empty(B, K, F, 2, device=dev)
        ops.permute4(out, gy, (B, K, F, 2), (F * ld, 1, ld, K))
        return out, None, None, None


def istft(spec, n_fft: int, hop: int, window):
    return IstftFn.apply(torch.view_as_real(spec), n_fft, hop, window)


class FilterbankSpecFn(torch.autograd.Function):

    @staticmethod
    def forward(ctx, x, n_fft: int, hop: int, fb, power: int):
        x = x.contiguous().float()
        B, T = x.shape
        S, packed, _, F = fused.filterbank_spec(x, n_fft, hop, fb, power)
        nf = fb.shape[1]
        out = ops.rows_to_bct(ops.empty(B, nf, F, device=x.device), S, B, nf, F)
        ctx.saved = packed
        ctx.meta = (n_fft, hop, power, B, T, F, nf)
        ctx.fb = fb
        return out

    @staticmethod
    def backward(ctx, g):
        n_fft, hop, power, B, T, F, nf = ctx.meta
        dev = g.device
        gS = ops.bct_to_rows(ops.empty(B * F, nf, device=dev), g.contiguous(), B, nf, F)
        gx = ops.empty(B, T, device=dev)
        fused.filterbank_spec_bwd(gS, ctx.saved, n_fft, hop, ctx.fb, power, B, T, F, gx, False)
        ctx.saved = None
        return gx, None, None, None, None


def filterbank_spectrogram(waveform, n_fft: int, hop: int, fb, power: int):
    lead = waveform.shape[:-1]
    x = waveform.reshape(-1, waveform.shape[-1])
    y = FilterbankSpecFn.apply(x, n_fft, hop, fb, power)
    return y.reshape(*lead, y.shape[1], y.shape[2])


class ChannelScaleFn(torch.autograd.Function):

    @staticmethod
    def forward(ctx, x, scale, limit: bool):
        x = x.contiguous().float()
        B, Cc, T = x.shape
        dev = x.device
        tiled = ops.empty(B, Cc, device=dev)
        ops.copy3(tiled, Cc, 0, scale, 0, 0, B, 1, Cc)
        y = ops.axpby_rows(ops.empty(B * Cc, T, device=dev), x.view(B * Cc, T), None, ca=tiled.view(-1))
        ctx.saved = (x, scale, tiled)
        ctx.limit = limit
        return y.view(B, Cc, T)

    @staticmethod
    def backward(ctx, g):
        x, scale, tiled = ctx.saved
        B, Cc, T = x.shape
        dev = g.device
        g = g.contiguous()
        gx = ops.axpby_rows(ops.empty(B * Cc, T, device=dev), g.view(B * Cc, T), None, ca=tiled.view(-1))
        gr = ops.bct_to_rows(ops.empty(B * T, Cc, device=dev), g, B, Cc, T)
        xr = ops.bct_to_rows(ops.empty(B * T, Cc, device=dev), x, B, Cc, T)
        gs = ops.zeros(Cc, 1, device=dev)
        ops.colsum(gs, gr, B * T, Cc, b=xr)
        if ctx.limit:
            ops.limit_grad(gs, scale, 0.5, 1.0)
        ctx.saved = None
        return gx.view(B, Cc, T), gs, None


class BiasNormFn(torch.autograd.Function):

    @staticmethod
    def forward(ctx, x, bias, log_scale, limit: bool):
        B, Cc, T = x.shape
        dev = x.device
        xr = ops.bct_to_rows(ops.empty(B * T, Cc, device=dev), x.contiguous().float(), B, Cc, T)
        yr = ops.biasnorm_fwd(xr, ops.empty(B * T, Cc, device=dev), B * T, Cc, bias, log_scale.reshape(1))
        ctx.saved = (xr, bias, log_scale)
        ctx.limit = limit
        ctx.dims = (B, Cc, T)
        return ops.rows_to_bct(ops.empty(B, Cc, T, device=dev), yr, B, Cc, T)

    @staticmethod
    def backward(ctx, g):
        xr, bias, log_scale = ctx.saved
        B, Cc, T = ctx.dims
        dev = g.device
        gr = ops.bct_to_rows(ops.empty(B * T, Cc, device=dev), g.contiguous(), B, Cc, T)
        g_beta, g_ls = ops.zeros_many([(Cc,), (1,)], dev)
        gxr = ops.biasnorm_bwd(xr, gr, ops.empty(B * T, Cc, device=dev), B * T, Cc, bias,
                               log_scale.reshape(1), g_beta, g_ls)
        if ctx.limit:
            ops.limit_grad(g_ls, log_scale.reshape(1), -1.5, 1.5)
        ctx.saved = None
        return ops.rows_to_bct(ops.empty(B, Cc, T, device=dev), gxr, B, Cc, T), g_beta, g_ls.reshape(()), None


class BlockFn(GradAwareFunction):

    @staticmethod
    def forward(ctx, x, cond, te, lens_cpu, training: bool, *params):
        dev = x.device
        B, Cc, F = x.shape
        bp = _Blk(list(params[:10]))
        rest = list(params[10:])
        wc = bc = wt = bt = None
        if cond is not None:
            wc, bc = rest[0], rest[1]
            rest = rest[2:]
        if te is not None:
            wt, bt = rest[0], rest[1]
        rows = B * F
        keep = _keep(ctx)
        xr = ops.bct_to_rows(ops.empty(rows, Cc, device=dev), x.contiguous().float(), B, Cc, F)
        cr = cproj = tep = None
        if cond is not None:
            Dc = cond.shape[1]
            cr = ops.bct_to_rows(ops.empty(rows, Dc, device=dev), cond.contiguous().float(), B, Dc, F)
            cproj = ops.empty(rows, Cc, device=dev)
            gemm(mat(cr, rows, Dc), mat(wc.reshape(Cc, Dc)), cproj, bias=bc)
        if te is not None:
            te = te.contiguous().float()
            tep = ops.empty(B, Cc, device=dev)
            gemm(mat(te), mat(wt), tep, bias=bt)
        lens = _lens_dev(lens_cpu, dev)
        fn = _limit_draw(training)
        y, z, a = fused.block_fwd(bp, xr, B, F, lens, cproj, Cc, F, 1, 0, tep, Cc, 0, keep=keep)
        fs = _limit_draw(training)
        if keep:
            ctx.saved = (xr, z, a, cr, cproj, te, tep, lens)
            ctx.params = params
            ctx.flags = (fn, fs)
            ctx.dims = (B, Cc, F)
        return ops.rows_to_bct(ops.empty(B, Cc, F, device=dev), y, B, Cc, F)

    @staticmethod
    def backward(ctx, g):
        xr, z, a, cr, cproj, te, tep, lens = ctx.saved
        params = ctx.params
        B, Cc, F = ctx.dims
        dev = g.device
        rows = B * F
        bp = _Blk(list(params[:10]))
        rest = list(params[10:])
        gr = ops.bct_to_rows(ops.empty(rows, Cc, device=dev), g.contiguous(), B, Cc, F)
        g_cp = ops.zeros(rows, Cc, device=dev) if cproj is not None else None
        g_tep = ops.zeros(B, Cc, device=dev) if tep is not None else None
        gx, gb = fused.block_bwd(bp, xr, z, a, gr, B, F, lens, ctx.flags[0], ctx.flags[1], cproj, Cc, F, 1, 0,
                                 tep, Cc, 0, g_cproj=g_cp, g_te=g_tep, g_cproj_store=True)
        out = [ops.rows_to_bct(ops.empty(B, Cc, F, device=dev), gx, B, Cc, F), None, None, None, None] + gb
        if cproj is not None:
            wc = rest[0]
            rest = rest[2:]
            Dc = cr.shape[1]
            g_wc, g_bc = ops.zeros_many([(Cc, Dc), (Cc,)], dev)
            ops.colsum(g_bc, g_cp, rows, Cc)
            ops.wgrad(g_cp, Cc, g_cp.stride(0), mat(cr, rows, Dc), g_wc)
            if ctx.needs_input_grad[1]:
                g_cr = ops.empty(rows, Dc, device=dev)
                gemm(mat(g_cp, rows, Cc), mat(wc.reshape(Cc, Dc)), g_cr, form=1)
                out[1] = ops.rows_to_bct(ops.empty(B, Dc, F, device=dev), g_cr, B, Dc, F)
            out += [g_wc.reshape(Cc, Dc, 1), g_bc]
        if tep is not None:
            wt = rest[0]
            Dt = te.shape[1]
            g_wt, g_bt = ops.zeros_many([(Cc, Dt), (Cc,)], dev)
            ops.colsum(g_bt, g_tep, B, Cc)
            ops.wgrad(g_tep, Cc, Cc, mat(te, B, Dt), g_wt)
            if ctx.needs_input_grad[2]:
                out[2] = ops.empty(B, Dt, device=dev)
                gemm(mat(g_tep, B, Cc), mat(wt), out[2], form=1)
            out += [g_wt, g_bt]
        ctx.saved = None
        return tuple(out)


def block_forward(blk, x, cond=None, time_embed=None, mask=None):
    B, _, F = x.shape
    params = fused.block_params(blk)
    if cond is not None:
        params += [blk.cond_proj.weight, blk.cond_proj.bias]
    if time_embed is not None:
        params += [blk.time_embed_proj.weight, blk.time_embed_proj.bias]
    return BlockFn.apply(x, cond, time_embed, mask_to_lens(mask, B, F), blk.training, *params)


class DecoderRowsFn(GradAwareFunction):

    @staticmethod
    def forward(ctx, xr, t, cproj, B: int, F: int, lens_cpu, training: bool, *params):
        dev = xr.device
        bv = _BranchView(list(params))
        Cc, Cin, Cout = bv.C, bv.Cin, bv.w_out.shape[0]
        rows, NC = B * F, bv.nblk * bv.C
        keep = _keep(ctx)
        lens = _lens_dev(lens_cpu, dev)
        h0 = ops.empty(rows, Cc, device=dev)
        gemm(mat(xr, rows, Cin), mat(bv.w_in.reshape(Cc, Cin)), h0, bias=bv.b_in, split_k=1)
        flags = [_limit_draw(training)]
        xcur = ops.biasnorm_fwd(h0, ops.empty(rows, Cc, device=dev), rows, Cc, bv.beta_in, bv.ls_in.reshape(1))
        tp = fused._time_path(bv, t) if t is not None else None
        te_all = None if tp is None else tp[-1]
        blocks = []
        for j, bp in enumerate(bv.blks):
            fn = _limit_draw(training)
            y, z, a = fused.block_fwd(bp, xcur, B, F, lens, cproj, NC, F, 1, j * Cc, te_all, NC, j * Cc, keep=keep)
            flags.append((fn, _limit_draw(training)))
            if keep:
                blocks.append((xcur, z, a))
            xcur = y
        out = ops.empty(rows, Cout, device=dev)
        gemm(mat(xcur, rows, Cc), mat(bv.w_out.reshape(Cout, Cc)), out, bias=bv.b_out, split_k=1)
        if keep:
            ctx.saved = (xr, h0, blocks, xcur, tp, cproj, lens)
            ctx.params = params
            ctx.flags = flags
            ctx.dims = (B, F)
        return out

    @staticmethod
    def backward(ctx, gy):
        xr, h0, blocks, x_last, tp, cproj, lens = ctx.saved
        B, F = ctx.dims
        bv = _BranchView(list(ctx.params))
        flags = ctx.flags
        dev = gy.device
        Cc, Cin, Cout = bv.C, bv.Cin, bv.w_out.shape[0]
        rows, NC = B * F, bv.nblk * bv.C
        Dt, Ht = bv.Dt, bv.Ht
        gy = gy.contiguous()
        (g_wout, g_bout, g_te_all, g_beta, g_ls, g_bin, g_win, g_tew, g_teb, g_tb2, g_tw2, g_tb0,
         g_tw0) = ops.zeros_many([(Cout, Cc), (Cout,), (B, NC), (Cc,), (1,), (Cc,), (Cc, Cin), (NC, Dt), (NC,),
                                  (Dt,), (Dt, Ht), (Ht,), (Ht, Dt)], dev)
        ops.colsum(g_bout, gy, rows, Cout)
        ops.wgrad(gy, Cout, gy.stride(0), mat(x_last, rows, Cc), g_wout)
        g = ops.empty(rows, Cc, device=dev)
        gemm(mat(gy, rows, Cout), mat(bv.w_out.reshape(Cout, Cc)), g, form=1)
        need_gc = ctx.needs_input_grad[2]
        g_cp = ops.zeros(rows, NC, device=dev)
        block_grads = [None] * bv.nblk
        te_all = None if tp is None else tp[-1]
        for j in reversed(range(bv.nblk)):
            xj, z, a = blocks[j]
            fn, fs = flags[1 + j]
            g, gb = fused.block_bwd(bv.blks[j], xj, z, a, g, B, F, lens, fn, fs, cproj, NC, F, 1, j * Cc,
                                    te_all, NC, j * Cc, g_cproj=g_cp, g_te=g_te_all if tp is not None else None,
                                    g_cproj_store=True)
            block_grads[j] = gb
        gh0 = ops.empty(rows, Cc, device=dev)
        ops.biasnorm_bwd(h0, g, gh0, rows, Cc, bv.beta_in, bv.ls_in.reshape(1), g_beta, g_ls)
        if flags[0]:
            ops.limit_grad(g_ls, bv.ls_in.reshape(1), -1.5, 1.5)
        ops.colsum(g_bin, gh0, rows, Cc)
        ops.wgrad(gh0, Cc, gh0.stride(0), mat(xr, rows, Cin), g_win)
        g_xr = None
        if ctx.needs_input_grad[0]:
            g_xr = ops.empty(rows, Cin, device=dev)
            gemm(mat(gh0, rows, Cc), mat(bv.w_in.reshape(Cc, Cin)), g_xr, form=1)
        if tp is not None:
            fused.time_path_bwd(bv, tp, g_te_all, B, (g_tew, g_teb, g_tb2, g_tw2, g_tb0, g_tw0))
        out = [g_xr, None, g_cp if need_gc else None, None, None, None, None,
               g_win.reshape(Cc, Cin, 1), g_bin, g_ls.reshape(()), g_beta, g_tw0, g_tb0, g_tw2, g_tb2,
               g_wout.reshape(Cout, Cc, 1), g_bout]
        for j in range(bv.nblk):
            out += block_grads[j]
            out.append(g_tew[j * Cc:(j + 1) * Cc])
            out.append(g_teb[j * Cc:(j + 1) * Cc])
        ctx.saved = None
        return tuple(out)


def decoder_forward(dec, x, cond, t=None, mask=None):
    B, _, F = x.shape
    assert cond.shape[0] == B and cond.shape[2] == F, "cond must be at the frame rate of x"
    xr = BctToRowsFn.apply(x)
    cr = BctToRowsFn.apply(cond)
    cproj = fused.CondPathFn.apply(cr, B, F, F, *fused.cond_path_params(dec))
    tt = None if t is None else t.flatten().contiguous().float()
    yr = DecoderRowsFn.apply(xr, tt, cproj, B, F, mask_to_lens(mask, B, F), dec.training,
                             *fused.decoder_params(dec))
    return RowsToBctFn.apply(yr, B, dec.out_channels, F)


def audio_convnext_forward(est, audio, cond, t=None, audio_lens=None):
    assert t is not None, "the HIP branch is time-conditioned (generator.py always passes t)"
    B, T = audio.shape
    cr = BctToRowsFn.apply(cond)
    F = 1 + T // est.hop_length
    up = est.cond_upsample_factor
    Fce = (F + up - 1) // up
    cproj = fused.CondPathFn.apply(cr, B, cond.shape[2], Fce, *fused.cond_path_params(est.decoder))
    params = fused.branch_params(est)
    metas = ((est.n_fft, est.hop_length, up, est.ifft.window), ("scale", 1.0))
    lens_cpu = None if audio_lens is None else [int(v) for v in audio_lens]
    return fused.ModelEvalFn.apply(audio.float(), t.flatten().contiguous().float(), None, metas, lens_cpu,
                                   est.training, (len(params),), cproj, *params)


def cond_encoder_forward(enc, x, mask=None):
    B, _, F = x.shape
    rows = fused.CondEncoderFn.apply(x.float(), enc.training, mask_to_lens(mask, B, F),
                                     *fused.cond_encoder_params(enc))
    return RowsToBctFn.apply(rows, B, enc.channels, F)


class DiscPFn(GradAwareFunction):

    @staticmethod
    def forward(ctx, x, p: int, *params):
        ctx.set_materialize_grads(False)
        keep = _keep(ctx)
        x = x.contiguous()
        B, T = x.shape
        st = FD._mpd_forward_one(x, p, list(params), keep_images=keep and any(ctx.needs_input_grad[2:]))
        outs = []
        for l in range(2, 6):
            y = st["acts"][l]
            H, Cc = st["hs"][l], y.shape[1]
            outs.append(FD.unhalo(y, B * p, H).reshape(B, p, H, Cc).permute(0, 3, 2, 1))
        sc = st["scores"].view(B, p, st["hs"][5], 1).permute(0, 3, 2, 1)
        if keep:
            ctx.saved = st
            ctx.params = params
            ctx.dims = (B, T, p)
        return (sc,) + tuple(outs)

    @staticmethod
    def backward(ctx, g_sc, *g_maps):
        st, prm = ctx.saved, list(ctx.params)
        B, T, p = ctx.dims
        need_x, need_w = ctx.needs_input_grad[0], any(ctx.needs_input_grad[2:])
        hs, S = st["hs"], st["S"]
        dev = st["scores"].device
        ups = {l: g_maps[l - 2] for l in range(2, 6)}
        ctx.saved = None
        if g_sc is None and all(u is None for u in g_maps):
            return tuple([None, None] + [None] * 12)
        gs, top = None, 4
        if g_sc is not None:
            gs = ops.empty(S * hs[5], 1, device=dev)
            sb, _, sh, sw = g_sc.stride()
            ops.permute4(gs, g_sc, (B, p, hs[5], 1), (sb, sw, sh, 0))
        else:
            top = max(l for l in range(2, 6) if ups[l] is not None) - 1
        g, grads_p = FD._mpd_backward_one(st, prm, gs, (S, 0), need_w, need_x, FD.MPDUpstreamLanding(st, B, ups), top)
        g_x = None
        if need_x:
            g_x = ops.empty(B, T, device=dev)
            ops.period_fold_bwd(g_x, g, B, T, p, hs[0], False)
        return tuple([g_x, None] + grads_p)


def discriminator_p_forward(d, x):
    out = DiscPFn.apply(x, d.period, *d._params())
    sc = out[0]
    return torch.flatten(sc, 1, -1), list(out[1:]) + [sc]


class DiscRFn(GradAwareFunction):

    @staticmethod
    def forward(ctx, x, win: int, *params):
        ctx.set_materialize_grads(False)
        keep = _keep(ctx)
        x = x.contiguous()
        B, T = x.shape
        st = FD._mrd_forward_one(x, win, list(params))
        Ft, Wcat, C = st["Ft"], st["Wcat"], FD.MRD_CH
        cat = st["cat"].view(B, Ft, Wcat, C)
        outs = []
        foff = 0
        for bi in range(5):
            ws = st["widths"][bi]
# ... 119 lines not shown
```

### flow2gan_amd/ops.py

```python
from __future__ import annotations

import ctypes as C
from typing import Optional

import torch

from . import _lib as L
from ._opts import opt
from ._lib import DwconvBwd, DwnormBwd, DwnormFwd, Epilogue, GemmDesc, Operand, call, ptr


def empty(*shape, device, dtype=torch.float32):
    return torch.empty(*shape, device=device, dtype=dtype)


def zeros(*shape, device):
    t = torch.empty(*shape, device=device, dtype=torch.float32)
    fill_(t, 0.0)
    return t


def fill_(t, v: float):
    if BATCH is not None and t.numel() > 0:
        import struct
        n = t.numel()
        BATCH.add(0, ptr(t), 4 * n, None, 0, (n & 0xffffffff, n >> 32, 0, 0),
                  (struct.unpack("<i", struct.pack("<f", float(v)))[0], 0, 0, 0), n, (t,))
        return t
    call("f2g_fill", ptr(t), float(v), t.numel())
    return t


def zero_halo(buf, nseq: int, rows_per_seq: int, Cc: int, lo: int, hi: int):
    call("f2g_zero_halo", ptr(buf), nseq, rows_per_seq, Cc, lo, hi)
    return buf


def pad4(n: int) -> int:
    return (n + 3) // 4 * 4


import weakref

WEIGHT_EPOCH = 0
_OWNER_EPOCH: dict = {}
_DERIVED: dict = {}


def bump_weight_epoch(params=None) -> None:
    global WEIGHT_EPOCH
    if params is None:
        WEIGHT_EPOCH += 1
        return
    for t in params:
        owner = t._base if t._base is not None else t
        _OWNER_EPOCH[id(owner)] = _OWNER_EPOCH.get(id(owner), 0) + 1


def _stamp(owner) -> tuple:
    if getattr(owner, "_f2g_const", False) and not isinstance(owner, torch.nn.Parameter):
        return (owner._version,)
    return (owner._version, WEIGHT_EPOCH, _OWNER_EPOCH.get(id(owner), 0))


DERIVED_KEEP = None


def weights_signature(params) -> tuple:
    ps = list(params)
    return (WEIGHT_EPOCH, tuple(p._version for p in ps),
            tuple(_OWNER_EPOCH.get(id(p), 0) for p in ps))


def derived(t, tag, build):
    out = _derived(t, tag, build)
    if DERIVED_KEEP is not None:
        DERIVED_KEEP.append(out)
    return out


def _derived(t, tag, build):
    import os
    if os.environ.get("F2G_WEIGHT_CACHE", "1") == "0":
        return build(t)
    owner = t._base if t._base is not None else t
    oid = id(owner)
    ent = _DERIVED.get(oid)
    if ent is None or ent[0]() is not owner:
        def _gone(_r, oid=oid, d=_DERIVED, e=_OWNER_EPOCH, rc=_RECIPES):
            d.pop(oid, None)
            e.pop(oid, None)
            rc.pop(oid, None)
        ent = (weakref.ref(owner, _gone), {})
        _DERIVED[oid] = ent
    slot = ent[1]
    key = (tag, t.data_ptr(), tuple(t.shape), tuple(t.stride()))
    stamp = _stamp(owner)
    hit = slot.get(key)
    if hit is not None and hit[0] == stamp:
        if hit[2] is not None and not _REPLAYING:
            hit[2][2] = True
        return hit[1]
    out = build(t)
    rec = None
    if isinstance(out, torch.Tensor):
        out._f2g_const = True
        spec = (tuple(t.shape), tuple(t.stride()), t.storage_offset() - owner.storage_offset())
        parent = getattr(owner, "_f2g_recipe", None)
        if isinstance(owner, torch.nn.Parameter) or parent is not None:
            root_ref, chain = (weakref.ref(owner), ()) if parent is None else parent
            chain = chain + ((tag, build, spec),)
            root = root_ref()
            if root is not None and len(chain) <= 4:
                ckey = tuple((c[0], c[2]) for c in chain)
                rec = _RECIPES.setdefault(id(root), {}).get(ckey)
                if rec is None or rec[0]() is not root:
                    rec = [root_ref, chain, False]
                    _RECIPES[id(root)][ckey] = rec
                else:
                    rec[1] = chain
                if not _REPLAYING:
                    rec[2] = True
                out._f2g_recipe = (root_ref, chain)
    slot[key] = (stamp, out, rec)
    return out


_DERIVED_MULTI: dict = {}


def derived_multi(ts, tag, build):
    out = _derived_multi(ts, tag, build)
    if DERIVED_KEEP is not None:
        DERIVED_KEEP.append(out)
    return out


def _derived_multi(ts, tag, build):
    import os
    if os.environ.get("F2G_WEIGHT_CACHE", "1") == "0":
        return build(ts)
    key = (tag,) + tuple(id(t) for t in ts)
    stamp = tuple(_stamp(t._base if t._base is not None else t) for t in ts)
    ent = _DERIVED_MULTI.get(key)
    if ent is not None and ent[0] == stamp and all(r() is t for r, t in zip(ent[2], ts)):
        return ent[1]
    out = build(ts)
    out._f2g_const = True
    if len(_DERIVED_MULTI) > 4096:
        _DERIVED_MULTI.clear()
    _DERIVED_MULTI[key] = (stamp, out, [weakref.ref(t) for t in ts])
    return out



BATCH = None
EAGER_REBUILD = opt("eager_rebuild", True)
_RECIPES: dict = {}
_REPLAYING = False


MULTI_CAP = min(L.MULTI_MAX, max(1, opt("multi_cap", L.MULTI_MAX)))


class WeightBatch:

    MAX_BLOCKS = 512

    def __init__(self):
        self.ops = []
        self.keep = []
        self.starts = []
        self.ranges = {}
        self.rstarts = []
        self.rranges = {}
        self.longest = 0

    def _level_over(self, starts, ranges, lo, hi):
        import bisect
        lvl = -1
        i = bisect.bisect_left(starts, hi)
        while i > 0:
            i -= 1
            st = starts[i]
            if lo - st >= self.longest:
                break
            end, l = ranges[st]
            if end > lo:
                lvl = max(lvl, l)
        return lvl

    def add(self, kind, out_ptr, out_bytes, rd_ptr, rd_bytes, n, s, items, tensors, in_ptr=None, reads_out=False):
        import bisect
        self.longest = max(self.longest, out_bytes, rd_bytes or 0)
        lvl = self._level_over(self.starts, self.ranges, out_ptr, out_ptr + out_bytes)
        lvl = max(lvl, self._level_over(self.rstarts, self.rranges, out_ptr, out_ptr + out_bytes))
        if rd_ptr is not None:
            lvl = max(lvl, self._level_over(self.starts, self.ranges, rd_ptr, rd_ptr + rd_bytes))
        lvl += 1
        old = self.ranges.get(out_ptr)
        if old is None:
            bisect.insort(self.starts, out_ptr)
        self.ranges[out_ptr] = (max(out_ptr + out_bytes, old[0] if old else 0), max(lvl, old[1] if old else 0))
        if rd_ptr is not None:
            oldr = self.rranges.get(rd_ptr)
            if oldr is None:
                bisect.insort(self.rstarts, rd_ptr)
            self.rranges[rd_ptr] = (max(rd_ptr + rd_bytes, oldr[0] if oldr else 0), max(lvl, oldr[1] if oldr else 0))
        self.ops.append((lvl, kind, out_ptr, in_ptr if in_ptr is not None else rd_ptr, tuple(n), tuple(s), items))
        self.keep.extend(tensors)

    def flush(self):
        if not self.ops:
            return 0
        launches = 0
        ops_, self.ops = sorted(self.ops, key=lambda o: o[0]), []
        i = 0
        while i < len(ops_):
            lvl = ops_[i][0]
            d = L.MultiDesc()
            k = 0
            while i < len(ops_) and ops_[i][0] == lvl and k < MULTI_CAP:
                _, kind, out_ptr, in_ptr, n, s, items = ops_[i]
                e = d.e[k]
                e.out, e.inp, e.kind = out_ptr, in_ptr, kind
                e.blocks = max(1, min(self.MAX_BLOCKS, (items + 255) // 256))
                for j in range(4):
                    e.n[j], e.s[j] = int(n[j]), int(s[j])
                k += 1
                i += 1
            d.n = k
            call("f2g_multi", C.byref(d))
            launches += 1
        self.keep = []
        self.starts, self.ranges, self.rstarts, self.rranges, self.longest = [], {}, [], {}, 0
        return launches


class weight_batch:

    def __enter__(self):
        global BATCH
        self.prev = BATCH
        if self.prev is None:
            BATCH = WeightBatch()
            L.PRE_CALL = BATCH.flush
        return BATCH

    def __exit__(self, *exc):
        global BATCH
        if self.prev is None:
            b, BATCH = BATCH, None
            L.PRE_CALL = None
            b.flush()
        return False


def rebuild_derived(params) -> int:
    global _REPLAYING
    if not EAGER_REBUILD or GEMM_PRECISION in (1, 2):
        return 0
    n = 0
    roots = {}
    for p_ in params:
        o = p_._base if p_._base is not None else p_
        roots[id(o)] = o
    import time
    t_host = time.perf_counter()
    _REPLAYING = True
    try:
        with torch.no_grad(), weight_batch():
            for rid, root in roots.items():
                rec = _RECIPES.get(rid)
                if not rec:
                    continue
                for key in sorted(rec, key=len):
                    ent = rec[key]
                    if ent[0]() is not root:
                        del rec[key]
                        continue
                    if not ent[2]:
                        continue
                    ent[2] = False
                    cur = root
                    for tag, build, spec in ent[1]:
                        shape, stride, off = spec
                        cur = _derived(cur.as_strided(shape, stride, cur.storage_offset() + off), tag, build)
                    n += 1
    finally:
        _REPLAYING = False
        REBUILD_STATS[0] += time.perf_counter() - t_host
        REBUILD_STATS[1] += n
    return n


REBUILD_STATS = [0.0, 0]


def transposed(w2d):
    def build(t):
        n, k = t.shape
        out = torch.empty(k, n, device=t.device, dtype=torch.float32)
        permute4(out, t, (k, n, 1, 1), (1, t.stride(0), 0, 0))
        return out
    return derived(w2d, "T", build)


def mat(t, rows: Optional[int] = None, cols: Optional[int] = None, ld: Optional[int] = None,
        alpha=None, lrelu_src=None, slope: float = 0.0, offset: int = 0, split: int = 0) -> Operand:
    if rows is None:
        rows = t.shape[0]
    if ld is None:
        ld = t.stride(0) if t.dim() == 2 else (cols if cols is not None else t.shape[-1])
    if cols is None:
        cols = t.shape[-1]
    o = Operand()
    o.base = ptr(t) + (2 if split == 2 else 4) * offset
    o.split = split
    o.rows, o.cols = rows, cols
    o.P1 = o.P0 = 1
    o.seglen = cols
    o.step1, o.pad1, o.L1 = 0, 0, 1
    o.step0, o.pad0, o.unit, o.L0u = 0, 0, 1, cols
    o.seq_stride, o.line_stride = ld, 0
    o.reflect = 0
    o.alpha = ptr(alpha)
    o.lrelu_src = None if lrelu_src is None else ptr(lrelu_src) + 4 * offset
    o.lrelu_slope = slope
    o._keep = (t, alpha, lrelu_src)
    o._src = t if (offset == 0 and t.dim() == 2 and rows == t.shape[0] and cols == t.shape[1]
                   and ld == t.stride(0) and alpha is None and lrelu_src is None) else None
    return o


def win1d(t, nseq: int, L_in: int, unit: int, L_out: int, step: int, pad: int, taps: int,
          reflect: bool = False, seq_stride: Optional[int] = None, lrelu_src=None,
          slope: float = 0.0, offset: int = 0, unbounded: bool = False) -> Operand:
    o = Operand()
    o.base = ptr(t) + 4 * offset
    o.rows, o.cols = nseq * L_out, taps * unit
    o.P1, o.P0 = 1, L_out
    o.seglen = taps * unit
    o.step1, o.pad1, o.L1 = 0, 0, 1
    o.step0, o.pad0, o.unit, o.L0u = step, pad, unit, L_in * unit
    o.seq_stride = seq_stride if seq_stride is not None else L_in * unit
    o.line_stride = 0
    o.reflect = 1 if reflect else 0
    o.alpha = None
    o.lrelu_src = None if lrelu_src is None else ptr(lrelu_src) + 4 * offset
    o.lrelu_slope = slope
    o.unbounded = 1 if (unbounded and offset == 0 and t.is_contiguous()
                        and t.numel() == nseq * o.seq_stride) else 0
    o._keep = (t, lrelu_src)
    return o


def win2d(t, nseq: int, H: int, W: int, Cin: int, W_out: int, kh: int, kw: int, stride_w: int,
          pad_h: int, pad_w: int, line_stride: Optional[int] = None,
          seq_stride: Optional[int] = None, offset: int = 0, lrelu_src=None,
          slope: float = 0.0) -> Operand:
    o = Operand()
    o.base = ptr(t) + 4 * offset
    o.rows, o.cols = nseq * H * W_out, kh * kw * Cin
    o.P1, o.P0 = H, W_out
    o.seglen = kw * Cin
    o.step1, o.pad1, o.L1 = 1, pad_h, H
    o.step0, o.pad0, o.unit, o.L0u = stride_w, pad_w, Cin, W * Cin
    o.line_stride = line_stride if line_stride is not None else W * Cin
    o.seq_stride = seq_stride if seq_stride is not None else H * o.line_stride
    o.reflect = 0
    o.alpha = None
    o.lrelu_src = None if lrelu_src is None else ptr(lrelu_src) + 4 * offset
    o.lrelu_slope = slope
    o._keep = (t, lrelu_src)
    return o


def _ask_with_x3_out(d, out, out_offset: int, x3_out: bool, prelu_out, ask):
    buf = getattr(out, "_f2g_x3_buf", None) if x3_out else None
    if buf is not None and X6F != 1 and not getattr(out, "_f2g_x3_bad", False) \
            and out_offset % 32 == 0 and prelu_out is None:
        d.E.x3_out = ptr(buf) + (out_offset // 32) * 192
    how = ask()
    if not how and d.E.x3_out:
        d.E.x3_out = None
        how = ask()
    return how


def gemm(A: Operand, Bm: Operand, out, form: int = 0, ldc: Optional[int] = None, *, bias=None,
         res=None, ldres: Optional[int] = None, gamma=None, aux=None, ldaux: Optional[int] = None,
         alpha_n=None, colsum_alpha=None, colsum=None, lrelu: float = 0.0, scale: float = 0.0,
         accumulate: bool = False, atomic: bool = False, split_k: int = 0, out_offset: int = 0,
         rowmap=None, prelu=None, prelu_out=None, mask=None, fm=None, x3_out: bool = False,
         true_k: Optional[int] = None, true_n: Optional[int] = None):
    if form == 1:
        src = getattr(Bm, "_src", None)
        if src is not None and src.shape[0] % 32 == 0 and src.shape[1] > 64:
            Bm, form = mat(transposed(src)), 0
    d = GemmDesc()
    d.A, d.B = A, Bm
    e = Epilogue()
    e.C = ptr(out) + 4 * out_offset
    e.ldc = ldc if ldc is not None else out.stride(0)
    e.c_bf16 = 1 if out.dtype == torch.bfloat16 else 0
    if rowmap is not None:
        e.P0o, e.seq_stride_o, e.row_stride_o, e.off_o = rowmap
    else:
        e.P0o = 0
    e.bias = ptr(bias)
    e.res = ptr(res)
    e.ldres = ldres if ldres is not None else (res.stride(0) if res is not None else 0)
    e.gamma = ptr(gamma)
    e.aux = ptr(aux)
    e.ldaux = ldaux if ldaux is not None else (aux.stride(0) if aux is not None else 0)
    e.alpha_n = ptr(alpha_n)
    e.colsum_alpha = ptr(colsum_alpha)
    e.colsum = ptr(colsum)
    e.lrelu_slope = lrelu
    e.scale = scale
    e.accumulate = 1 if accumulate else 0
    e.atomic = 1 if atomic else 0
    e.prelu_slope = ptr(prelu)
    e.prelu_out = ptr(prelu_out)
    e.ld_prelu_out = prelu_out.stride(0) if prelu_out is not None else 0
    if mask is not None:
        e.mask_src = ptr(mask[0]) + 4 * mask[1]
        e.mask_slope = float(mask[2])
        if fm is not None:
            e.fm_ref = ptr(fm[0]) + 4 * fm[1]
            e.fm_w = float(fm[2])
            e.fm_wdev = ptr(fm[3])
    d.E = e
    d.form = form
    if split_k == -1:
        tiles = ((A.cols + 127) // 128) * ((Bm.cols + 127) // 128)
        split_k = split_for(A.rows, tiles)
        if form == 2 and GEMM_PRECISION == 0 and atomic:
            d.split_k, d.precision = split_k, 0
            if L.lib.f2g_gemm_wgrad_lean(C.byref(d)):
                split_k = split_for(A.rows, tiles, True)
    d.split_k = split_k
    d.precision = GEMM_PRECISION
    f16 = _fp16x3_gemm(d, A, Bm, out, form, atomic, split_k, out_offset, x3_out, prelu_out)
    if GEMM_PRECISION == 3 and f16:
        if x3_out and not d.E.x3_out:
            out._f2g_x3_bad = True
    elif GEMM_PRECISION == 3:
        d.precision = 0
        in_kernel = X6F == 1
        if X6F == 2 and X6F_MIN_K <= A.cols < X6_MIN_K and (
                (Bm.rows >= X6F_MIN_N and ((A.rows + 127) // 128) * ((Bm.rows + 127) // 128) >= X6F_MIN_TILES)
                or (A.rows >= X6F_TALL_ROWS and Bm.rows >= 128)):
            in_kernel = True
        if X6F == 2 and 128 <= A.cols < X6_MIN_K and A.rows >= X6F_TALL_ROWS and Bm.rows == 32:
            in_kernel = True
        if X6F == 2 and X6_MIN_K <= A.cols < X6_NOPASS_K and A.P0 == 1 and A.P1 == 1 and not _is_const(A._keep[0]):
            in_kernel = True
        if form == 0 and A.split == 0 and Bm.split == 0 and A.rows >= X6_MIN_ROWS \
                and (A.cols >= X6_MIN_K or in_kernel) and not atomic \
                and split_k <= 1 and out.dtype == torch.float32 and _x3_window_ok(A):
            how = _ask_with_x3_out(d, out, out_offset, x3_out, prelu_out, lambda: L.lib.f2g_gemm_x6_ok(C.byref(d)))
            if how:
                if in_kernel and not (how & 4):
                    in_kernel = False
                    how = how if A.cols >= X6_MIN_K else 0
                if how:
                    if not in_kernel:
                        d.A, d.B = _x3_operand(A), _x3_operand(Bm)
                    elif Bm.P0 == 1 and Bm.P1 == 1 and _is_const(Bm._keep[0]):
                        d.B = _x3_operand(Bm, frag_major=X6G and Bm.rows % 32 == 0 and Bm.rows > 32)
                    d.precision = 3
            if d.precision != 3:
                d.E.x3_out = None
        if form == 2 and atomic and A.split == 0 and Bm.split == 0 and A.lrelu_src is None \
                and A.rows >= X6_MIN_K and L.lib.f2g_gemm_lean_ok(C.byref(d)):
            d.precision = 3
        if x3_out:
            if d.E.x3_out:
                out._f2g_x3 = out._f2g_x3_buf
            else:
                out._f2g_x3_bad = True
    if (GEMM_PRECISION == 1 and form in (0, 2)) or (GEMM_PRECISION == 2 and form == 0):
        ok = L.lib.f2g_gemm_lean_ok(C.byref(d))
        if GEMM_PRECISION == 2 and (ok & 2):
            d.A, d.B = _bf16_operand(A), _bf16_operand(Bm)
        elif ok:
            d.A, d.B = _split_operand(A), _split_operand(Bm)
    parts = None
    if COLSUM_PARTS and d.precision in (3, 4) and form == 0 and (colsum is not None or colsum_alpha is not None) \
            and A.rows >= COLSUM_PARTS_MIN_ROWS:
        nrows = L.lib.f2g_gemm_colsum_part_rows(C.byref(d))
        if nrows > 0:
            ncol = Bm.rows
            both = colsum is not None and colsum_alpha is not None
            parts = torch.empty(nrows, (2 if both else 1) * ncol, device=out.device, dtype=torch.float32)
            d.E.colsum_part_ld = parts.stride(0)
            if colsum_alpha is not None:
                d.E.colsum_alpha = ptr(parts)
            if colsum is not None:
                d.E.colsum = ptr(parts) + (4 * ncol if both else 0)
    if GEMM_TIMER is not None:
        GEMM_TIMER.launch(d, A, Bm, form, true_k, true_n)
    else:
        call("f2g_gemm", C.byref(d))
    if parts is not None:
        nrows, ncol = parts.shape[0], Bm.rows
        if colsum is not None and colsum_alpha is not None and ptr(colsum) == ptr(colsum_alpha) + 4 * ncol:
            call("f2g_colsum", ptr(colsum_alpha), ptr(parts), parts.stride(0), None, 0, nrows, 2 * ncol)
            return out
        if colsum_alpha is not None:
            call("f2g_colsum", ptr(colsum_alpha), ptr(parts), parts.stride(0), None, 0, nrows, ncol)
        if colsum is not None:
            call("f2g_colsum", ptr(colsum), ptr(parts) + (4 * ncol if colsum_alpha is not None else 0),
                 parts.stride(0), None, 0, nrows, ncol)
    return out


import os as _os

COLSUM_PARTS = opt("colsum_parts", True)
COLSUM_PARTS_MIN_ROWS = 2048

def split3(img, src, src_off_bytes: int, ld: int, rows: int, K: int):
    if BATCH is not None and rows > 0:
        BATCH.add(3, ptr(img), rows * K * 6, ptr(src) + src_off_bytes, 4 * ((rows - 1) * ld + K), (rows, K, 0, 0),
                  (ld, 0, 0, 0), rows * (K // 4), (img, src))
        return img
    call("f2g_split_bf16x3", ptr(img), ptr(src) + src_off_bytes, ld, rows, K)
    return img


def split3g(img, src, src_off_bytes: int, ld: int, rows: int, K: int):
    assert rows % 32 == 0 and K % 32 == 0
    if BATCH is not None and rows > 0:
        BATCH.add(4, ptr(img), rows * K * 6, ptr(src) + src_off_bytes, 4 * ((rows - 1) * ld + K), (rows, K, 0, 0),
                  (ld, 0, 0, 0), rows * (K // 8), (img, src))
        return img
    d = L.MultiDesc()
    e = d.e[0]
    e.out, e.inp, e.kind = ptr(img), ptr(src) + src_off_bytes, 4
    e.blocks = max(1, min(WeightBatch.MAX_BLOCKS, (rows * (K // 8) + 255) // 256))
    e.n[0], e.n[1], e.s[0] = rows, K, ld
    d.n = 1
    call("f2g_multi", C.byref(d))
    return img


def split_bf16(t):
    out = torch.empty_like(t)
    call("f2g_split_bf16", ptr(out), ptr(t), t.numel())
    out._f2g_const = getattr(t, "_f2g_const", False)
    return out


_SHARES: dict = {}


class split_sharing:

    def __init__(self, *tensors):
        self.ts = [t for t in tensors if t is not None]
        self.imgs = {}

    def __enter__(self):
        for t in self.ts:
            _SHARES.setdefault(id(t), []).append(self)
        return self

    def __exit__(self, *exc):
        for t in self.ts:
            st = _SHARES.get(id(t))
            if st:
                st.pop()
                if not st:
                    del _SHARES[id(t)]
        return False

    def drop(self):
        self.imgs = {}

    def image(self, t, base: int):
        key = (id(t), base)
        img = self.imgs.get(key)
        if img is None:
            n = t.numel() - (base - ptr(t)) // 4
            img = torch.empty(n, device=t.device, dtype=torch.float32)
            call("f2g_split_bf16", ptr(img), base, n)
            self.imgs[key] = img
        return img


def to_bf16(t):
    out = torch.empty(t.shape, device=t.device, dtype=torch.bfloat16)
    call("f2g_to_bf16", ptr(out), ptr(t), t.numel())
    out._f2g_const = getattr(t, "_f2g_const", False)
    return out


def _bf16_operand(o: Operand) -> Operand:
    if o.split == 2:
        return o
    if o.split:
        raise L.F2GError("a split-bf16 image cannot serve as a bf16 operand")
    t = o._keep[0]
    n = Operand()
    C.memmove(C.byref(n), C.byref(o), C.sizeof(Operand))
    if _is_const(t) and t.is_contiguous() and t.numel() % 4 == 0 and (o.base - ptr(t)) % 16 == 0:
        img = derived(t, "bf16", to_bf16)
        n.base = ptr(img) + (o.base - ptr(t)) // 2
    else:
        nseq = o.rows // (o.P0 * o.P1)
        nseg = o.cols // min(o.seglen, o.cols)
        if o.P0 == 1 and o.P1 == 1:
            extent = (o.rows - 1) * o.seq_stride + o.cols
        else:
            extent = (nseq - 1) * o.seq_stride + \
                ((o.P1 - 1) * o.step1 - o.pad1 + nseg - 1) * o.line_stride + \
                ((o.P0 - 1) * o.step0 - o.pad0) * o.unit + min(o.seglen, o.cols)
        extent = (extent + 3) // 4 * 4
        img = torch.empty(extent, device=t.device, dtype=torch.bfloat16)
        call("f2g_to_bf16", ptr(img), o.base, extent)
        n.base = ptr(img)
    n.split = 2
    n._keep = (img,) + tuple(o._keep)
    return n


X6_MIN_ROWS = opt("x6_min_rows", 1024)
X6_MIN_K = opt("x6_min_k", 2048)


def _x3_operand(o: Operand, frag_major: bool = False) -> Operand:
    t = o._keep[0]
    rows, K, ld = o.rows, o.cols, o.seq_stride
    off = o.base - ptr(t)
    if o.P0 == 1 and o.P1 == 1:
        def build(tt):
            img = torch.empty(rows * K * 3, device=tt.device, dtype=torch.bfloat16)
            split3(img, tt, off, ld, rows, K)
            return img
        if frag_major:
            assert _is_const(t) and rows % 32 == 0

            def build_g(tt):
                imgf = torch.empty(rows * K * 3, device=tt.device, dtype=torch.bfloat16)
                split3g(imgf, tt, off, ld, rows, K)
                return imgf
            imgf = derived(t, ("x3g", off, rows, K, ld), build_g)
            n = Operand()
            C.memmove(C.byref(n), C.byref(o), C.sizeof(Operand))
            n.base = ptr(imgf)
            n.split = 4
            n._keep = (imgf,) + tuple(o._keep)
            return n
        img = derived(t, ("x3", off, rows, K, ld), build) if _is_const(t) else build(t)
        shift = 0
    else:
        img = getattr(t, "_f2g_x3", None)
        if img is None or getattr(t, "_f2g_x3_bad", False):
            img = x3_flat_image(t)
        elif X3_CHECK:
            ref = x3_flat_image(t)
            torch.cuda.synchronize()
            neq = img.view(torch.int16) != ref.view(torch.int16)
            if bool(neq.any()):
                idx = neq.nonzero()[:, 0]
                e = (idx // 96) * 32 + idx % 32
# ... 692 lines not shown
    return [e["out"] for e in entries]


FUSED_MULTI = opt("fused_multi", True)


def _dw_desc(x, ldx, z, ldz, B, F, Cc, K, lens, w_dw, b_dw, beta, log_scale, cproj, ldcp, Fc, up,
             cp_off, te, ldte, te_off, rstd) -> DwnormFwd:
    f = DwnormFwd()
    f.x, f.ldx = ptr(x), ldx
    f.z, f.ldz = ptr(z), ldz
    f.B, f.F, f.C, f.K = B, F, Cc, K
    f.lens = ptr(lens)
    f.w_dw, f.b_dw, f.beta, f.log_scale = ptr(w_dw), ptr(b_dw), ptr(beta), ptr(log_scale)
    f.cproj = None if cproj is None else ptr(cproj) + 4 * cp_off
    f.ldcp, f.Fc, f.up = ldcp, Fc, up
    f.te = None if te is None else ptr(te) + 4 * te_off
    f.ldte = ldte
    f.rstd = ptr(rstd)
    return f


def dwnorm_fwd(x, z, B, F, Cc, K, lens, w_dw, b_dw, beta, log_scale, cproj=None, ldcp=0, Fc=0,
               up=1, cp_off=0, te=None, ldte=0, te_off=0, rstd=None, z_format: int = 0):
    f = _dw_desc(x, x.stride(0), z, z.stride(0), B, F, Cc, K, lens, w_dw, b_dw, beta, log_scale,
                 cproj, ldcp, Fc, up, cp_off, te, ldte, te_off, rstd)
    f.z_format = z_format
    if GEMM_TIMER is not None:
        nb = 4.0 * B * F * Cc * (2.0 + (1.0 / up if cproj is not None else 0.0))
        GEMM_TIMER.time_hbm(lambda: call("f2g_dwnorm_fwd", C.byref(f)), nb, "dwnorm_fwd")
    else:
        call("f2g_dwnorm_fwd", C.byref(f))
    return z


def dwnorm_bwd(x, gz, du, B, F, Cc, K, lens, w_dw, b_dw, beta, log_scale, cproj=None, ldcp=0,
               Fc=0, up=1, cp_off=0, te=None, ldte=0, te_off=0, g_cproj=None, g_te=None,
               g_beta=None, g_log_scale=None, g_cproj_store=False):
    d = DwnormBwd()
    d.f = _dw_desc(x, x.stride(0), None, 0, B, F, Cc, K, lens, w_dw, b_dw, beta, log_scale, cproj,
                   ldcp, Fc, up, cp_off, te, ldte, te_off, None)
    d.gz, d.ldgz = ptr(gz), gz.stride(0)
    d.du, d.lddu = ptr(du), du.stride(0)
    d.g_cproj = None if g_cproj is None else ptr(g_cproj) + 4 * cp_off
    d.g_cproj_store = 1 if (g_cproj_store and g_cproj is not None) else 0
    d.g_te = None if g_te is None else ptr(g_te) + 4 * te_off
    d.g_beta, d.g_log_scale = ptr(g_beta), ptr(g_log_scale)
    ws = torch.empty(L.lib.f2g_dwnorm_bwd_workspace(B, F, Cc, up if cproj is not None else 1),
                     device=x.device, dtype=torch.float32)
    d.partials = ptr(ws)
    if GEMM_TIMER is not None:
        nb = 4.0 * B * F * Cc * (3.0 + ((1.0 / up if cproj is not None else 0.0)
                                      + (1.0 / up if g_cproj is not None else 0.0)))
        GEMM_TIMER.time_hbm(lambda: call("f2g_dwnorm_bwd", C.byref(d)), nb, "dwnorm_bwd")
    else:
        call("f2g_dwnorm_bwd", C.byref(d))
    return du


def dwconv_bwd(du, x, gx, B, F, Cc, K, lens, w_dw, gres=None, gamma=None, g_w=None, g_b=None,
               g_gamma=None):
    d = DwconvBwd()
    d.du, d.lddu = ptr(du), du.stride(0)
    d.x, d.ldx = ptr(x), x.stride(0)
    d.gx, d.ldgx = ptr(gx), gx.stride(0)
    d.B, d.F, d.C, d.K = B, F, Cc, K
    d.lens = ptr(lens)
    d.w_dw = ptr(w_dw)
    d.gres = ptr(gres)
    d.ldgres = gres.stride(0) if gres is not None else 0
    d.gamma = ptr(gamma)
    d.g_w, d.g_b, d.g_gamma = ptr(g_w), ptr(g_b), ptr(g_gamma)
    ws = torch.empty(L.lib.f2g_dwconv_bwd_workspace(B, F, Cc, K), device=x.device,
                     dtype=torch.float32)
    d.partials = ptr(ws)
    if GEMM_TIMER is not None:
        GEMM_TIMER.time_hbm(lambda: call("f2g_dwconv_bwd", C.byref(d)), 16.0 * B * F * Cc, "dwconv_bwd")
    else:
        call("f2g_dwconv_bwd", C.byref(d))
    return gx


def biasnorm_fwd(x, y, rows, Cc, beta, log_scale):
    call("f2g_biasnorm_fwd", ptr(x), x.stride(0), ptr(y), y.stride(0), rows, Cc, ptr(beta),
         ptr(log_scale))
    return y


def biasnorm_bwd(x, gy, gx, rows, Cc, beta, log_scale, g_beta, g_log_scale):
    call("f2g_biasnorm_bwd", ptr(x), x.stride(0), ptr(gy), gy.stride(0), ptr(gx), gx.stride(0),
         rows, Cc, ptr(beta), ptr(log_scale), ptr(g_beta), ptr(g_log_scale))
    return gx


def istft_ola(frames, out, B, F, n_fft, hop, T, window, wbranch, wscale, accumulate):
    call("f2g_istft_ola", ptr(frames), frames.stride(0), ptr(out), B, F, n_fft, hop, T,
         ptr(window), ptr(wbranch), float(wscale), 1 if accumulate else 0)


def istft_ola_multi(entries, out, B, T, wscale, accumulate=False):
    d = L.OlaMultiDesc()
    d.n = len(entries)
    for i, (frames, F, n_fft, hop, window, wbranch) in enumerate(entries):
        d.frames[i], d.ldf[i] = ptr(frames), frames.stride(0)
        d.F[i], d.n_fft[i], d.hop[i] = F, n_fft, hop
        d.window[i], d.wbranch[i] = ptr(window), ptr(wbranch)
    call("f2g_istft_ola_multi", C.byref(d), ptr(out), B, T, float(wscale), 1 if accumulate else 0)
    return out


def istft_ola_bwd(gout, gframes, B, F, n_fft, hop, T, window, wbranch, wscale):
    call("f2g_istft_ola_bwd", ptr(gout), ptr(gframes), gframes.stride(0), B, F, n_fft, hop, T,
         ptr(window), ptr(wbranch), float(wscale))


def frames_fold(gframes, gx, B, F, n_fft, hop, T, accumulate):
    call("f2g_frames_fold", ptr(gframes), gframes.stride(0), ptr(gx), B, F, n_fft, hop, T,
         1 if accumulate else 0)


def axpby_rows(y, x0, x1, ca=None, cb=None, sa=1.0, sb=1.0):
    rows = x0.shape[0]
    cols = x0.numel() // rows
    call("f2g_axpby_rows", ptr(y), ptr(x0), ptr(x1), ptr(ca), ptr(cb), float(sa), float(sb), rows,
         cols)
    return y


def clamp(y, x, lo, hi):
    call("f2g_clamp", ptr(y), ptr(x), float(lo), float(hi), x.numel())
    return y


def silu(y, x):
    call("f2g_silu", ptr(y), ptr(x), x.numel())
    return y


def silu_bwd(gx, gy, x):
    call("f2g_silu_bwd", ptr(gx), ptr(gy), ptr(x), x.numel())
    return gx


def time_embedding(out, t, dim, scale=1000.0):
    call("f2g_time_embedding", ptr(out), ptr(t), t.numel(), dim, float(scale))
    return out


def mask_rows(x, B, F, Cc, lens):
    call("f2g_mask_rows", ptr(x), x.stride(0), B, F, Cc, ptr(lens))
    return x


def colsum(out, a, rows, cols, b=None, out_offset=0):
    call("f2g_colsum", ptr(out) + 4 * out_offset, ptr(a), a.stride(0), ptr(b),
         b.stride(0) if b is not None else 0, rows, cols)
    return out


def colsum_strided(out, a, nrows, W, Cc, ld, off):
    tmp = zeros(W * Cc, device=a.device)
    call("f2g_colsum", ptr(tmp), ptr(a) + 4 * off, ld, None, 0, nrows, W * Cc)
    call("f2g_colsum", ptr(out), ptr(tmp), Cc, None, 0, W, Cc)


def bct_to_rows(out, x, B, Cc, F):
    call("f2g_bct_to_rows", ptr(out), out.stride(0), ptr(x), B, Cc, F)
    return out


def rows_to_bct(out, x, B, Cc, F):
    call("f2g_rows_to_bct", ptr(out), ptr(x), x.stride(0), B, Cc, F)
    return out


def permute4(out, x, dims, strides, in_offset=0):
    n0, n1, n2, n3 = dims
    s0, s1, s2, s3 = strides
    if BATCH is not None and n0 * n1 * n2 * n3 > 0:
        lo = sum(min(0, (n - 1) * st) for n, st in zip(dims, strides))
        hi = sum(max(0, (n - 1) * st) for n, st in zip(dims, strides)) + 1
        BATCH.add(1, ptr(out), 4 * n0 * n1 * n2 * n3, ptr(x) + 4 * (in_offset + lo), 4 * (hi - lo), dims, strides,
                  n0 * n1 * n2 * n3, (out, x), in_ptr=ptr(x) + 4 * in_offset)
        return out
    call("f2g_permute4", ptr(out), ptr(x) + 4 * in_offset, n0, n1, n2, n3, s0, s1, s2, s3)
    return out


def copy3(out, so0, so1, x, si0, si1, n0, n1, n2, accumulate=False, out_offset=0, in_offset=0):
    if BATCH is not None and n0 * n1 * n2 > 0 and min(so0, so1, si0, si1) >= 0:
        BATCH.add(2, ptr(out) + 4 * out_offset, 4 * ((n0 - 1) * so0 + (n1 - 1) * so1 + n2),
                  ptr(x) + 4 * in_offset, 4 * ((n0 - 1) * si0 + (n1 - 1) * si1 + n2),
                  (n0, n1, n2, 1 if accumulate else 0), (so0, so1, si0, si1), n0 * n1 * n2, (out, x),
                  reads_out=bool(accumulate))
        return out
    call("f2g_copy3", ptr(out) + 4 * out_offset, so0, so1, ptr(x) + 4 * in_offset, si0, si1, n0,
         n1, n2, 1 if accumulate else 0)
    return out


def spec_power(out, packed, rows, nb, power):
    call("f2g_spec_power", ptr(out), out.stride(0), ptr(packed), packed.stride(0), rows, nb, power)
    return out


def spec_power_bwd(gpacked, gout, packed, rows, nb, power):
    call("f2g_spec_power_bwd", ptr(gpacked), gpacked.stride(0), ptr(gout), gout.stride(0),
         ptr(packed), rows, nb, power)
    return gpacked


def fm_spec_loss(loss, g_err, s_err, s_gt, B, F, nf, lens, eps, power, lo, hi, inv_denom):
    call("f2g_fm_spec_loss", ptr(loss), ptr(g_err), ptr(s_err), ptr(s_gt), B, F, nf, ptr(lens),
         float(eps), float(power), float(lo), float(hi), float(inv_denom))


def masked_mse(loss, g_err, pred, ref, B, T, lens, inv_denom):
    call("f2g_masked_mse", ptr(loss), ptr(g_err), ptr(pred), ptr(ref), B, T, ptr(lens),
         float(inv_denom))


def l1_loss(loss, gb, a, b, rows, cols, ld, w, clip=0.0, wdev=None, loss_offset=0, off=0):
    call("f2g_l1_loss", None if loss is None else ptr(loss) + 4 * loss_offset,
         None if gb is None else ptr(gb) + 4 * off, ptr(a) + 4 * off, ptr(b) + 4 * off, rows, cols,
         ld, float(w), float(clip), ptr(wdev))


def l1_loss_ab(loss, gb, a, a_off, b, b_off, rows, cols, ld, w, clip=0.0, wdev=None,
               loss_offset=0):
    call("f2g_l1_loss", None if loss is None else ptr(loss) + 4 * loss_offset,
         None if gb is None else ptr(gb) + 4 * b_off, ptr(a) + 4 * a_off, ptr(b) + 4 * b_off, rows,
         cols, ld, float(w), float(clip), ptr(wdev))


def hinge_loss(loss, gs, s, n, sgn, w, wdev=None, loss_offset=0, s_off=0):
    call("f2g_hinge_loss", None if loss is None else ptr(loss) + 4 * loss_offset,
         None if gs is None else ptr(gs) + 4 * s_off, ptr(s) + 4 * s_off, n, float(sgn), float(w),
         ptr(wdev))


def peaknorm_fwd(y, stats, x, rows, T):
    call("f2g_peaknorm_fwd", ptr(y), ptr(stats), ptr(x), rows, T)


def peaknorm_bwd(gx, gy, x, stats, rows, T, row_off=0):
    call("f2g_peaknorm_bwd", ptr(gx), ptr(gy), ptr(x) + 4 * row_off * T, ptr(stats) + 4 * 3 * row_off, rows, T)


def lrelu_bwd(g, y_act, f_real, w, slope, rows, cols, ld, wdev=None, g_off=0, y_off=0, r_off=0):
    call("f2g_lrelu_bwd", ptr(g) + 4 * g_off, ptr(y_act) + 4 * y_off,
         None if f_real is None else ptr(f_real) + 4 * r_off, float(w), ptr(wdev), float(slope),
         rows, cols, ld)


def lrelu_bwd_colsum(g, y_act, f_real, w, slope, rows, Cc, ld, colsum, wdev=None, g_off=0, y_off=0,
                     r_off=0):
    args = ("f2g_lrelu_bwd_colsum", ptr(g) + 4 * g_off, ptr(y_act) + 4 * y_off,
            None if f_real is None else ptr(f_real) + 4 * r_off, float(w), ptr(wdev), float(slope),
            rows, Cc, ld, ptr(colsum))
    if GEMM_TIMER is not None:
        GEMM_TIMER.time_hbm(lambda: call(*args), (12.0 + (4.0 if f_real is not None else 0.0)) * rows * Cc,
                            "lrelu_bwd_colsum")
    else:
        call(*args)


def lrelu_bwd_add(g, y_act, dims, g_strides, Cc, u, u_strides, slope, colsum=None, g_off=0):
    n0, n1, n2 = dims
    gs0, gs1, gs2 = g_strides
    us0, us1, us2, usc = u_strides
    call("f2g_lrelu_bwd_add", ptr(g), ptr(y_act), g_off, n0, n1, n2, Cc, gs0, gs1, gs2,
         ptr(u), us0, us1, us2, usc, float(slope), ptr(colsum))
    return g


def zeros_many(shapes, device):
    sizes = []
    for sh in shapes:
        n = 1
        for v in sh:
            n *= v
        sizes.append(n)
    offs, total = [], 0
    for n in sizes:
        offs.append(total)
        total += (n + 63) // 64 * 64
    flat = zeros(max(total, 1), device=device)
    return [flat[o:o + n].view(*sh) for o, n, sh in zip(offs, sizes, shapes)]


def _mpd0_desc(x, S, H, Hout, halo, w=None, bias=None, slope=0.0, y=None, x_off=0, y_off=0):
    d = L.Mpd0Desc()
    d.x = None if x is None else ptr(x) + 4 * x_off
    d.S, d.H, d.Hout, d.halo = S, H, Hout, halo
    d.w, d.bias, d.slope = ptr(w), ptr(bias), slope
    d.y = ptr(y) + 4 * y_off
    return d


def mpd0_fwd(x, S, H, Hout, halo, w5, bias, slope, y):
    d = _mpd0_desc(x, S, H, Hout, halo, w5, bias, slope, y)
    _timed_hbm("f2g_mpd0_fwd", 4.0 * S * (Hout * 32 + H), C.byref(d))
    return y


def mpd0_wgrad(x, S, H, Hout, halo, g, gw):
    d = _mpd0_desc(x, S, H, Hout, halo, y=g)
    _timed_hbm("f2g_mpd0_wgrad", 4.0 * S * (Hout * 32 + H), C.byref(d), ptr(gw))
    return gw


def mpd0_dgrad(g, S, H, Hout, halo, w5, gx, g_off=0):
    d = _mpd0_desc(None, S, H, Hout, halo, w5, None, 0.0, g, y_off=g_off)
    _timed_hbm("f2g_mpd0_dgrad", 4.0 * S * (Hout * 32 + H), C.byref(d), ptr(gx))
    return gx


def _mpdpost_desc(y, S, H, halo, w3=None, bias=None, out=None, g=None, g_off=0, y_off=0):
    d = L.MpdPostDesc()
    d.y = ptr(y) + 4 * y_off
    d.S, d.H, d.halo = S, H, halo
    d.w, d.bias, d.out = ptr(w3), ptr(bias), ptr(out)
    d.g = None if g is None else ptr(g) + 4 * g_off
    return d


def mpdpost_fwd(y, S, H, halo, w3, bias, out):
    _timed_hbm("f2g_mpdpost_fwd", 4.0 * S * H * (1024 + 1), C.byref(_mpdpost_desc(y, S, H, halo, w3, bias, out)))
    return out


def mpdpost_dgrad(g, S, H, halo, w3, gy, g_off=0, mask=None, fm=None, colsum=None):
    d = _mpdpost_desc(gy, S, H, halo, w3, None, None, g, g_off)
    nbytes = 4.0 * S * H * (1024 + 1)
    if mask is not None:
        d.mask_src, d.mask_slope = ptr(mask[0]) + 4 * mask[1], float(mask[2])
        nbytes += 4.0 * S * H * 1024
        if fm is not None:
            d.fm_ref, d.fm_w, d.fm_wdev = ptr(fm[0]) + 4 * fm[1], float(fm[2]), ptr(fm[3])
            nbytes += 4.0 * S * H * 1024
    d.colsum = ptr(colsum)
    buf = getattr(gy, "_f2g_x3_buf", None)
    if buf is not None and not getattr(gy, "_f2g_x3_bad", False):
        d.x3_out = ptr(buf)
        gy._f2g_x3 = buf
        nbytes += 6.0 * S * H * 1024
    _timed_hbm("f2g_mpdpost_dgrad", nbytes, C.byref(d))
    return gy


def mpdpost_wgrad(y, S, H, halo, g, gw):
    d = _mpdpost_desc(y, S, H, halo, None, None, None, g)
    _timed_hbm("f2g_mpdpost_wgrad", 4.0 * S * H * (1024 + 1), C.byref(d), ptr(gw))
    return gw


USE_FFT = opt("fft", True)
FFT_MIN = opt("fft_min", 128)
_FFT_TABLES = {}


def fft_applies(n_fft: int) -> bool:
    return USE_FFT and FFT_MIN <= n_fft <= 4096 and (n_fft & (n_fft - 1)) == 0


def _fft_tables(n_fft: int, device):
    import math
    key = (n_fft, str(device))
    if key not in _FFT_TABLES:
        j = torch.arange(n_fft // 2, dtype=torch.float64)
        ang = 2.0 * math.pi * j / n_fft
        tw = torch.stack([torch.cos(ang), -torch.sin(ang)], dim=1).float().contiguous().to(device)
        win = torch.hann_window(n_fft, dtype=torch.float32).to(device)
        _FFT_TABLES[key] = (win, tw)
    return _FFT_TABLES[key]


def _spec_flags(spec, interleaved: bool) -> int:
    return (1 if interleaved else 0) | (2 if spec.dtype == torch.bfloat16 else 0)


FFT_REFLECT = opt("fft_reflect", True)


def stft_fft(x, n_fft: int, hop: int, F: int, spec, interleaved: bool = False, zero_pad: bool = False):
    B, T = x.shape
    pad = n_fft // 2
    win, tw = _fft_tables(n_fft, x.device)
    d = L.FftDesc()
    if FFT_REFLECT and T > pad and x.stride(1) == 1:
        xp = x
        d.x, d.x_stride, d.reflect_T = ptr(x), x.stride(0), T
    else:
        Tp = pad4(T + 2 * pad)
        xp = torch.empty(B, Tp, device=x.device, dtype=torch.float32)
        call("f2g_reflect_pad", ptr(xp), ptr(x), B, T, pad, Tp)
        d.x, d.x_stride = ptr(xp), Tp
    d.hop, d.n_fft, d.F, d.rows = hop, n_fft, F, B * F
    d.window, d.twiddle = ptr(win), ptr(tw)
    d.spec, d.ld_spec, d.interleaved = ptr(spec), spec.stride(0), _spec_flags(spec, interleaved)
    d.spec_cols = spec.shape[1] if zero_pad else 0
    call("f2g_fft_frames", C.byref(d), 0)
    d._keep = (xp, win, tw)
    return spec


def stft_fft_adjoint(gspec, n_fft: int, F: int, gframes, interleaved: bool = False):
    rows = gframes.shape[0]
    win, tw = _fft_tables(n_fft, gspec.device)
    d = L.FftDesc()
    d.hop, d.n_fft, d.F, d.rows = 0, n_fft, F, rows
    d.window, d.twiddle = ptr(win), ptr(tw)
    d.spec, d.ld_spec, d.interleaved = ptr(gspec), gspec.stride(0), 1 if interleaved else 0
    d.frames, d.ld_frames = ptr(gframes), gframes.stride(0)
    call("f2g_fft_frames", C.byref(d), 1)
    return gframes


def istft_fft(spec, n_fft: int, F: int, frames):
    win, tw = _fft_tables(n_fft, spec.device)
    d = L.FftDesc()
    d.hop, d.n_fft, d.F, d.rows = 0, n_fft, F, frames.shape[0]
    d.window, d.twiddle = ptr(win), ptr(tw)
    d.spec, d.ld_spec, d.interleaved = ptr(spec), spec.stride(0), _spec_flags(spec, False)
    d.frames, d.ld_frames = ptr(frames), frames.stride(0)
    call("f2g_fft_frames", C.byref(d), 2)
    return frames


def istft_fft_adjoint(gframes, n_fft: int, F: int, gspec, zero_pad: bool = False):
    win, tw = _fft_tables(n_fft, gframes.device)
    d = L.FftDesc()
    d.hop, d.n_fft, d.F, d.rows = 0, n_fft, F, gframes.shape[0]
    d.window, d.twiddle = ptr(win), ptr(tw)
    d.spec, d.ld_spec, d.interleaved = ptr(gspec), gspec.stride(0), 0
    d.spec_cols = gspec.shape[1] if zero_pad else 0
    d.frames, d.ld_frames = ptr(gframes), gframes.stride(0)
    call("f2g_fft_frames", C.byref(d), 3)
    return gspec


def stft_frames(x, n_fft: int, hop: int, F: int) -> Operand:
    B, T = x.shape
    pad = n_fft // 2
    Tp = pad4(T + 2 * pad)
    if hop % 4 or n_fft % 32:
        return win1d(x, B, T, 1, F, hop, pad, n_fft, reflect=True)
    xp = torch.empty(B, Tp, device=x.device, dtype=torch.float32)
    call("f2g_reflect_pad", ptr(xp), ptr(x), B, T, pad, Tp)
    return win1d(xp, B, Tp, 1, F, hop, 0, n_fft)


def period_fold(out, x, B, T, p, H):
    call("f2g_period_fold", ptr(out), ptr(x), B, T, p, H)


def period_fold_bwd(gx, gout, B, T, p, H, accumulate):
    call("f2g_period_fold_bwd", ptr(gx), ptr(gout), B, T, p, H, 1 if accumulate else 0)


def limit_grad(g, p, lo, hi):
    call("f2g_limit_grad", ptr(g), ptr(p), float(lo), float(hi), g.numel())
    return g


def log_clip_(x, clip=1e-7):
    call("f2g_log_clip", ptr(x), x.numel(), float(clip))
    return x
```

### include/flow2gan_hip.h

```cpp
#ifndef FLOW2GAN_HIP_H
#define FLOW2GAN_HIP_H

#include <stdint.h>

#ifdef __cplusplus
extern "C" {
#endif

typedef void* f2g_stream_t;

enum {
  F2G_OK = 0,
  F2G_EINVAL = -1,
  F2G_ELAUNCH = -2,
};

const char* f2g_version(void);
const char* f2g_last_error(void);

int f2g_set_option(const char* name, int32_t value);
int f2g_get_option(const char* name, int32_t* value);

typedef struct {
  const float* base;
// ... 85 lines not shown
  const float* log_scale;
  const float* cproj;
  int64_t ldcp;
  int32_t Fc, up;
  const float* te;
  int64_t ldte;
  float* rstd;
  int32_t z_format;
  int32_t _pad;
} f2g_dwnorm_fwd_desc;
int f2g_dwnorm_fwd(const f2g_dwnorm_fwd_desc* d, f2g_stream_t stream);

typedef struct {
  f2g_dwnorm_fwd_desc f;
  const float* gz;
  int64_t ldgz;
  float* du;
  int64_t lddu;
  float* g_cproj;
  float* g_te;
  float* g_beta;
  float* g_log_scale;
  float* partials;
  int32_t g_cproj_store;
  int32_t _pad2;
} f2g_dwnorm_bwd_desc;
int f2g_dwnorm_bwd(const f2g_dwnorm_bwd_desc* d, f2g_stream_t stream);
int64_t f2g_dwnorm_bwd_workspace(int32_t B, int32_t F, int32_t C, int32_t up);

typedef struct {
  const float* du;
  int64_t lddu;
  const float* x;
  int64_t ldx;
  float* gx;
  int64_t ldgx;
  int32_t B, F, C, K;
  const int32_t* lens;
  const float* w_dw;
  const float* gres;
  int64_t ldgres;
  const float* gamma;
  float* g_w;
  float* g_b;
  float* g_gamma;
  float* partials;
} f2g_dwconv_bwd_desc;
int f2g_dwconv_bwd(const f2g_dwconv_bwd_desc* d, f2g_stream_t stream);
int64_t f2g_dwconv_bwd_workspace(int32_t B, int32_t F, int32_t C, int32_t K);

int f2g_biasnorm_fwd(const float* x, int64_t ldx, float* y, int64_t ldy, int32_t rows, int32_t C,
                     const float* beta, const float* log_scale, f2g_stream_t stream);
int f2g_biasnorm_bwd(const float* x, int64_t ldx, const float* gy, int64_t ldgy, float* gx,
                     int64_t ldgx, int32_t rows, int32_t C, const float* beta,
                     const float* log_scale, float* g_beta, float* g_log_scale,
                     f2g_stream_t stream);

int f2g_istft_ola(const float* frames, int64_t ldf, float* out, int32_t B, int32_t F,
                  int32_t n_fft, int32_t hop, int32_t T, const float* window,
                  const float* wbranch, float wscale, int32_t accumulate, f2g_stream_t stream);
typedef struct {
  const float* frames[4];
  int64_t ldf[4];
  int32_t F[4], n_fft[4], hop[4];
  const float* window[4];
  const float* wbranch[4];
  int32_t n, _pad;
} f2g_ola_multi_desc;
int f2g_istft_ola_multi(const f2g_ola_multi_desc* d, float* out, int32_t B, int32_t T, float wscale,
                        int32_t accumulate, f2g_stream_t stream);
int f2g_istft_ola_bwd(const float* gout, float* gframes, int64_t ldf, int32_t B, int32_t F,
                      int32_t n_fft, int32_t hop, int32_t T, const float* window,
                      const float* wbranch, float wscale, f2g_stream_t stream);
int f2g_frames_fold(const float* gframes, int64_t ldf, float* gx, int32_t B, int32_t F,
                    int32_t n_fft, int32_t hop, int32_t T, int32_t accumulate,
                    f2g_stream_t stream);

int f2g_axpby_rows(float* y, const float* x0, const float* x1, const float* ca, const float* cb,
                   float sa, float sb, int32_t rows, int32_t cols, f2g_stream_t stream);
int f2g_clamp(float* y, const float* x, float lo, float hi, int64_t n, f2g_stream_t stream);
int f2g_silu(float* y, const float* x, int64_t n, f2g_stream_t stream);
int f2g_silu_bwd(float* gx, const float* gy, const float* x, int64_t n, f2g_stream_t stream);
int f2g_time_embedding(float* out, const float* t, int32_t B, int32_t dim, float scale,
                       f2g_stream_t stream);
int f2g_mask_rows(float* x, int64_t ld, int32_t B, int32_t F, int32_t C, const int32_t* lens,
                  f2g_stream_t stream);
int f2g_colsum(float* out, const float* a, int64_t lda, const float* b, int64_t ldb, int32_t rows,
               int32_t cols, f2g_stream_t stream);
int f2g_rows_fold_up(float* out, int64_t ldo, const float* g, int64_t ldg, int32_t B, int32_t F,
                     int32_t Fc, int32_t up, int32_t C, f2g_stream_t stream);
int f2g_bct_to_rows(float* out, int64_t ldo, const float* in, int32_t B, int32_t C, int32_t F,
                    f2g_stream_t stream);
int f2g_rows_to_bct(float* out, const float* in, int64_t ldi, int32_t B, int32_t C, int32_t F,
                    f2g_stream_t stream);
int f2g_permute4(float* out, const float* in, int32_t n0, int32_t n1, int32_t n2, int32_t n3,
                 int64_t s0, int64_t s1, int64_t s2, int64_t s3, f2g_stream_t stream);

int f2g_limit_grad(float* g, const float* p, float lo, float hi, int64_t n, f2g_stream_t stream);
int f2g_copy3(float* out, int64_t so0, int64_t so1, const float* in, int64_t si0, int64_t si1,
              int32_t n0, int32_t n1, int32_t n2, int32_t accumulate, f2g_stream_t stream);

int f2g_spec_power(float* out, int64_t ldo, const float* packed, int64_t ldp, int32_t rows,
                   int32_t nb, int32_t power, f2g_stream_t stream);
int f2g_spec_power_bwd(float* gpacked, int64_t ldp, const float* gout, int64_t ldo,
                       const float* packed, int32_t rows, int32_t nb, int32_t power,
                       f2g_stream_t stream);
int f2g_fm_spec_loss(float* loss, float* g_err, const float* s_err, const float* s_gt, int32_t B,
                     int32_t F, int32_t n_filt, const int32_t* lens, float eps, float power,
                     float lo, float hi, float inv_denom, f2g_stream_t stream);
int f2g_masked_mse(float* loss, float* g_err, const float* pred, const float* ref, int32_t B,
                   int32_t T, const int32_t* lens, float inv_denom, f2g_stream_t stream);
int f2g_l1_loss(float* loss, float* gb, const float* a, const float* b, int32_t rows, int32_t cols,
                int64_t ld, float w, float clip, const float* wdev, f2g_stream_t stream);
int f2g_hinge_loss(float* loss, float* gs, const float* s, int64_t n, float sgn, float w,
                   const float* wdev, f2g_stream_t stream);
int f2g_peaknorm_fwd(float* y, float* stats, const float* x, int32_t rows, int32_t T,
                     f2g_stream_t stream);
int f2g_peaknorm_bwd(float* gx, const float* gy, const float* x, const float* stats, int32_t rows,
                     int32_t T, f2g_stream_t stream);
int f2g_lrelu_bwd(float* g, const float* y_act, const float* f_real, float w, const float* wdev,
                  float slope, int32_t rows, int32_t cols, int64_t ld, f2g_stream_t stream);
int f2g_lrelu_bwd_colsum(float* g, const float* y_act, const float* f_real, float w,
                         const float* wdev, float slope, int32_t rows, int32_t C, int64_t ld,
                         float* colsum, f2g_stream_t stream);
int f2g_lrelu_bwd_add(float* g, const float* y_act, int64_t off, int32_t n0, int32_t n1, int32_t n2, int32_t C,
                      int64_t gs0, int64_t gs1, int64_t gs2, const float* u, int64_t us0, int64_t us1,
                      int64_t us2, int64_t usc, float slope, float* colsum, f2g_stream_t stream);
typedef struct {
  const float* x;
  int64_t x_stride;
  int32_t hop, n_fft, F, rows;
  const float* window;
  const float* twiddle;
  float* spec;
  int64_t ld_spec;
  int32_t interleaved;
  int32_t spec_cols;
  float* frames;
  int64_t ld_frames;
  int32_t reflect_T;
  int32_t _pad;
} f2g_fft_desc;
int f2g_fft_frames(const f2g_fft_desc* d, int32_t mode, f2g_stream_t stream);

int f2g_reflect_pad(float* out, const float* x, int32_t B, int32_t T, int32_t pad, int32_t Tp,
                    f2g_stream_t stream);
int f2g_period_fold(float* out, const float* x, int32_t B, int32_t T, int32_t p, int32_t H,
                    f2g_stream_t stream);
int f2g_period_fold_bwd(float* gx, const float* gout, int32_t B, int32_t T, int32_t p, int32_t H,
                        int32_t accumulate, f2g_stream_t stream);
int f2g_log_clip(float* x, int64_t n, float clip, f2g_stream_t stream);
int f2g_fill(float* x, float v, int64_t n, f2g_stream_t stream);
enum { F2G_MULTI_FILL = 0, F2G_MULTI_PERMUTE4 = 1, F2G_MULTI_COPY3 = 2, F2G_MULTI_SPLIT3 = 3, F2G_MULTI_SPLIT3G = 4,
       F2G_MULTI_SPLIT_F16 = 5 };
#define F2G_MULTI_MAX 48
typedef struct {
  void* out;
  const void* in;
  int32_t kind;
  int32_t blocks;
  int32_t n[4];
  int64_t s[4];
} f2g_multi_entry;
typedef struct {
  int32_t n;
  int32_t _pad;
  f2g_multi_entry e[F2G_MULTI_MAX];
} f2g_multi_desc;
int f2g_multi(const f2g_multi_desc* d, f2g_stream_t stream);
int f2g_bucket_arm(float* flat, int64_t n, int32_t nflags, f2g_stream_t stream);
int f2g_scale(float* x, float s, int64_t n, f2g_stream_t stream);
int f2g_zero_halo(float* buf, int32_t nseq, int32_t rows_per_seq, int32_t C, int32_t lo,
                  int32_t hi, f2g_stream_t stream);

typedef struct {
  const float* x;
  int32_t S, H, Hout, halo;
  const float* w;
  const float* bias;
  float slope;
  int32_t _pad;
  float* y;
} f2g_mpd0_desc;
int f2g_mpd0_fwd(const f2g_mpd0_desc* d, f2g_stream_t stream);
int f2g_mpd0_wgrad(const f2g_mpd0_desc* d, float* gw, f2g_stream_t stream);
int f2g_mpd0_dgrad(const f2g_mpd0_desc* d, float* gx, f2g_stream_t stream);

typedef struct {
  float* y;
  int32_t S, H, halo, _pad;
  const float* w;
  const float* bias;
  float* out;
  const float* g;
  const float* mask_src;
  const float* fm_ref;
  const float* fm_wdev;
  float mask_slope;
  float fm_w;
  float* colsum;
  void* x3_out;
} f2g_mpdpost_desc;
int f2g_mpdpost_fwd(const f2g_mpdpost_desc* d, f2g_stream_t stream);
int f2g_mpdpost_dgrad(const f2g_mpdpost_desc* d, f2g_stream_t stream);
int f2g_mpdpost_wgrad(const f2g_mpdpost_desc* d, float* gw, f2g_stream_t stream);

typedef struct {
  const float* x;
  int64_t x_seq, x_line;
  int32_t S, H, Win, Wout;
  const float* w;
  const float* bias;
  float lrelu_slope;
  int32_t precision;
  float* y;
  int64_t y_seq, y_line;
  const float* mask_src;
  const float* fm_ref;
  const float* fm_wdev;
  float mask_slope;
  float fm_w;
  float* colsum;
} f2g_conv32_desc;
int f2g_conv32_s2_fwd(const f2g_conv32_desc* d, f2g_stream_t stream);
int f2g_conv32_s2_dgrad(const f2g_conv32_desc* d, f2g_stream_t stream);
int f2g_conv32_s2_wgrad(const f2g_conv32_desc* d, float* gw, f2g_stream_t stream);
int f2g_conv32_s2_wgrad_h3(const f2g_conv32_desc* d, float* gw, f2g_stream_t stream);
int f2g_conv33_fwd(const f2g_conv32_desc* d, f2g_stream_t stream);
int f2g_conv33_wgrad(const f2g_conv32_desc* d, float* gw, f2g_stream_t stream);

typedef struct {
  const float* x;
  int64_t x_seq, x_line;
  int32_t S, H, W, _pad;
  const float* w;
  const float* bias;
  float lrelu_slope;
  int32_t _pad2;
  float* y;
  float* gw;
  const float* wt;
  float* gx;
  int64_t gx_seq, gx_line;
} f2g_conv2ch_desc;
int f2g_conv2ch_fwd(const f2g_conv2ch_desc* d, f2g_stream_t stream);
int f2g_conv2ch_wgrad(const f2g_conv2ch_desc* d, f2g_stream_t stream);
int f2g_conv2ch_dgrad(const f2g_conv2ch_desc* d, f2g_stream_t stream);
int f2g_convpost_fwd(const f2g_conv2ch_desc* d, f2g_stream_t stream);
int f2g_convpost_wgrad(const f2g_conv2ch_desc* d, f2g_stream_t stream);
int f2g_convpost_dgrad(const f2g_conv2ch_desc* d, f2g_stream_t stream);

int f2g_wave_stats(const float* x, int64_t item_stride, int64_t ch_stride, int32_t B, int32_t C,
                   const int32_t* lens, float* stats, f2g_stream_t stream);
int f2g_wave_gain(float* out, int64_t ldo, const float* x, int64_t item_stride, int64_t ch_stride,
                  int32_t B, int32_t C, int32_t T, const int32_t* lens, const float* stats,
                  const float* target_peak, f2g_stream_t stream);

#define F2G_SADAM_NCOEF 12
#define F2G_SADAM_TSTATE 10
#define F2G_SADAM_GSTATE 1028
typedef struct {
  float* p;
  const float* g;
  float* v;
  float* m;
  int64_t numel;
  int32_t group;
  int32_t is_scalar;
} f2g_sadam_tensor;
typedef struct {
  int32_t tensor;
  int32_t count;
  int64_t offset;
} f2g_sadam_chunk;
typedef struct {
  float lr, beta1, beta2, scalar_lr_scale, eps, param_min_rms, param_max_rms, scalar_max;
  float clipping_scale;
  int32_t size_update_period;
  int32_t clipping_update_period;
  int32_t step;
  int32_t first, count;
} f2g_sadam_group;
int32_t f2g_sadam_chunk_elems(void);
int f2g_sadam_stats(const f2g_sadam_tensor* tensors, const f2g_sadam_chunk* chunks,
                    int32_t nchunks, float* stats, int32_t ntensors, f2g_stream_t stream);
int f2g_sadam_prepare(const f2g_sadam_tensor* tensors, const f2g_sadam_group* group,
                      const float* stats, float* tstate, float* gstate, float* coef,
                      f2g_stream_t stream);
int f2g_sadam_update(const f2g_sadam_tensor* tensors, const f2g_sadam_chunk* chunks,
                     int32_t nchunks, const float* coef, f2g_stream_t stream);

typedef struct {
  const void* z;
  int64_t ldz;
  const void* wp;
  const float* b1;
  const float* alpha;
  const float* b2;
  const float* res;
  int64_t ldres;
  const float* gamma;
  float* out;
  int64_t ldo;
  int32_t rows, C, H;
  int32_t parts;
} f2g_fused_mlp_desc;
int f2g_fused_mlp_ok(int32_t C, int32_t H);
// ... 13 lines not shown
```

Before: 797.0 audio-s/s.

## Batch zero-halo, limit-grad and bias colsums into the multi-kernel launch tables

Adds ZERO_HALO, LIMIT_GRAD and COLSUM kinds to the multi-entry kernel. Host code now queues these small ops into the batched launch table instead of issuing separate kernels. Bias colsums and limit_grad calls in the backward passes are deferred to a tail that is flushed as one batch at the end of each backward. Accumulator zeroing and halo buffers are hoisted so they can be batched too. The aim is to cut per-launch overhead from many tiny kernels, at the cost of sliced two-pass colsum temporaries and more complex ordering and hazard tracking.

```diff
diff --git a/flow2gan_amd/csrc/multi.hip b/flow2gan_amd/csrc/multi.hip
--- a/flow2gan_amd/csrc/multi.hip
+++ b/flow2gan_amd/csrc/multi.hip
@@ -99,7 +99,76 @@
                        b * 4 + (threadIdx.x >> 6), nb * 4);
 }
 
+__device__ __forceinline__ void run_zero_halo(const f2g_multi_entry& e, long long b, long long nb) {
+  float4* buf = reinterpret_cast<float4*>(e.out);
+  const int Hp = e.n[1], C4 = e.n[2] / 4, lo = (int)e.s[0], hi = (int)e.s[1];
+  const long long per = (long long)(lo + hi) * C4, total = (long long)e.n[0] * per;
+  for (long long i = b * 256 + threadIdx.x; i < total; i += nb * 256) {
+    const long long sq = i / per;
+    const int r = (int)(i - sq * per);
+    const int hr = r / C4, c = r - hr * C4;
+    const int row = hr < lo ? hr : Hp - hi + (hr - lo);
+    buf[(sq * Hp + row) * C4 + c] = make_float4(0.f, 0.f, 0.f, 0.f);
+  }
+}
+
+__device__ __forceinline__ void run_limit_grad(const f2g_multi_entry& e, long long b, long long nb) {
+  float* g = reinterpret_cast<float*>(e.out);
+  const float* p = reinterpret_cast<const float*>(e.in);
+  const long long n = ((long long)e.n[1] << 32) | (unsigned)e.n[0];
+  const float lo = __int_as_float((int)e.s[0]), hi = __int_as_float((int)e.s[1]);
+  for (long long i = b * 256 + threadIdx.x; i < n; i += nb * 256) {
+    float gv = g[i];
+    const float pv = p[i];
+    if (gv > 0.f && pv < lo) gv = -gv;
+    if (gv < 0.f && pv > hi) gv = -gv;
+    g[i] = gv;
+  }
+}
+
+__device__ __forceinline__ void run_colsum(const f2g_multi_entry& e, long long b, long long nb, float* red) {
+  float* out = reinterpret_cast<float*>(e.out);
+  const float* a = reinterpret_cast<const float*>(e.in);
+  const int rows = e.n[0], cols = e.n[1], acc = e.n[2], slices = e.n[3];
+  const long long ld = e.s[0], pst = e.s[1];
+  const int rps = (int)e.s[2];
+  int cs_log2 = 0;
+  while ((1 << cs_log2) < cols && cs_log2 < 6) ++cs_log2;
+  const int CS = 1 << cs_log2, RS = 256 >> cs_log2;
+  const int lane = threadIdx.x & 63, wave = threadIdx.x >> 6;
+  const int cl = lane & (CS - 1), rl = threadIdx.x >> cs_log2;
+  const int nchunk = (cols + CS - 1) >> cs_log2;
+  const long long work = (long long)nchunk * slices;
+  for (long long w = b; w < work; w += nb) {
+    const int sl = (int)(w / nchunk), c = (int)(w - (long long)sl * nchunk) * CS + cl;
+    const int r0 = sl * rps, r1 = r0 + min(rps, rows - r0);
+    float s0 = 0.f, s1 = 0.f, s2 = 0.f, s3 = 0.f;
+    if (c < cols) {
+      const float* q = a + c;
+      int r = r0 + rl;
+      for (; r + 3 * RS < r1; r += 4 * RS) {
+        s0 += q[(long long)r * ld];
+        s1 += q[(long long)(r + RS) * ld];
+        s2 += q[(long long)(r + 2 * RS) * ld];
+        s3 += q[(long long)(r + 3 * RS) * ld];
+      }
+      for (; r < r1; r += RS) s0 += q[(long long)r * ld];
+    }
+    float s = (s0 + s1) + (s2 + s3);
+    for (int o = CS; o < 64; o <<= 1) s += __shfl_xor(s, o);
+    __syncthreads();
+    if (lane < CS) red[wave * 64 + lane] = s;
+    __syncthreads();
+    if (wave == 0 && lane < CS && c < cols) {
+      const float t = (red[lane] + red[64 + lane]) + (red[128 + lane] + red[192 + lane]);
+      float* o = out + sl * pst + c;
+      *o = acc ? *o + t : t;
+    }
+  }
+}
+
 __global__ __launch_bounds__(256) void multi_kernel(const f2g_multi_desc d) {
+  __shared__ float red[256];
   int i = 0;
   long long first = 0;
   while (i + 1 < d.n && (long long)blockIdx.x >= first + d.e[i].blocks) first += d.e[i++].blocks;
@@ -111,32 +180,57 @@
     case F2G_MULTI_COPY3: run_copy3(e, b, nb); break;
     case F2G_MULTI_SPLIT3: run_split3(e, b, nb); break;
     case F2G_MULTI_SPLIT_F16: run_split_f16(e, b, nb); break;
+    case F2G_MULTI_ZERO_HALO: run_zero_halo(e, b, nb); break;
+    case F2G_MULTI_LIMIT_GRAD: run_limit_grad(e, b, nb); break;
+    case F2G_MULTI_COLSUM: run_colsum(e, b, nb, red); break;
     default: run_split3g(e, b, nb); break;
   }
 }
 
 }
 
+static int multi_bad(const char* why) {
+  f2g_set_error(why);
+  return F2G_EINVAL;
+}
+
 extern "C" int f2g_multi(const f2g_multi_desc* d, f2g_stream_t stream) {
-  if (!d || d->n < 0 || d->n > F2G_MULTI_MAX) return F2G_EINVAL;
+  if (!d || d->n < 0 || d->n > F2G_MULTI_MAX) return multi_bad("f2g_multi: no table, or more than F2G_MULTI_MAX entries");
   long long grid = 0;
   for (int i = 0; i < d->n; ++i) {
     const f2g_multi_entry& e = d->e[i];
-    if (!e.out || (e.kind != F2G_MULTI_FILL && !e.in) || e.blocks < 1 || e.kind < 0 || e.kind > F2G_MULTI_SPLIT_F16)
-      return F2G_EINVAL;
-    if (e.kind == F2G_MULTI_SPLIT3G && (e.n[0] & 31)) return F2G_EINVAL;
+    const bool no_in = e.kind == F2G_MULTI_FILL || e.kind == F2G_MULTI_ZERO_HALO;
+    if (!e.out || (!no_in && !e.in) || e.blocks < 1 || e.kind < 0 || e.kind > F2G_MULTI_COLSUM)
+      return multi_bad("f2g_multi: entry without a pointer or a block, or of an unknown kind");
+    if (e.kind == F2G_MULTI_SPLIT3G && (e.n[0] & 31)) return multi_bad("f2g_multi: SPLIT3G rows % 32 != 0");
     if ((e.kind == F2G_MULTI_SPLIT3 || e.kind == F2G_MULTI_SPLIT3G) &&
         (e.n[1] < 32 || (e.n[1] % 32) || e.s[0] < e.n[1] || (e.s[0] & 3) || (((uintptr_t)e.in) & 15) ||
          (((uintptr_t)e.out) & 15)))
-      return F2G_EINVAL;
+      return multi_bad("f2g_multi: SPLIT3 needs K % 32 == 0, ld >= K, ld % 4 == 0 and 16-byte aligned pointers");
     if (e.kind == F2G_MULTI_SPLIT_F16 &&
         (e.n[0] < 0 || e.n[1] < 32 || (e.n[1] % 32) || e.n[1] > F2G_F16_MAX_K || e.s[0] < e.n[1] || (e.s[0] & 3) ||
          e.s[1] <= 0 || (((uintptr_t)e.in) & 15) || (((uintptr_t)e.out) & 15)))
-      return F2G_EINVAL;
+      return multi_bad("f2g_multi: SPLIT_F16 needs 32 <= K <= 4096, K % 32 == 0, ld >= K and 16-byte aligned pointers");
+    if (e.kind == F2G_MULTI_ZERO_HALO) {
+      if (e.n[2] <= 0 || (e.n[2] & 3) || e.s[0] < 0 || e.s[1] < 0 || e.n[1] < 0 || e.s[0] + e.s[1] > e.n[1])
+        return multi_bad("f2g_multi: ZERO_HALO needs C % 4 == 0, top, bottom >= 0 and top + bottom <= rows per sequence");
+      if (((uintptr_t)e.out) & 15) return multi_bad("f2g_multi: ZERO_HALO map not 16-byte aligned");
+    }
+    if (e.kind == F2G_MULTI_LIMIT_GRAD && (e.n[1] < 0 || ((((uintptr_t)e.out) | ((uintptr_t)e.in)) & 3)))
+      return multi_bad("f2g_multi: LIMIT_GRAD needs n >= 0 and 4-byte aligned pointers");
+    if (e.kind == F2G_MULTI_COLSUM) {
+      const long long rows = e.n[0], cols = e.n[1], slices = e.n[3], rps = e.s[2];
+      if (rows < 1 || rows > 0x7fffffff - 1024 || cols < 1 || (e.n[2] != 0 && e.n[2] != 1) || e.s[0] < cols)
+        return multi_bad("f2g_multi: COLSUM needs 1 <= rows <= 2^31 - 1025, cols >= 1, ld >= cols and accumulate in {0, 1}");
+      if (slices < 1 || rps < 1 || rps > 0x7fffffff || (slices - 1) * rps >= rows || slices * rps < rows ||
+          (slices > 1 && e.s[1] < cols))
+        return multi_bad("f2g_multi: COLSUM slices must cover the rows once, partial rows >= cols apart");
+      if ((((uintptr_t)e.out) | ((uintptr_t)e.in)) & 3) return multi_bad("f2g_multi: COLSUM pointers not 4-byte aligned");
+    }
     grid += e.blocks;
   }
   if (grid == 0) return F2G_OK;
-  if (grid >= (1ll << 31)) return F2G_EINVAL;
+  if (grid >= (1ll << 31)) return multi_bad("f2g_multi: more than 2^31 blocks");
   hipLaunchKernelGGL(multi_kernel, dim3((unsigned)grid), dim3(256), 0, (hipStream_t)stream, *d);
   return f2g_check_launch();
 }
diff --git a/flow2gan_amd/fused.py b/flow2gan_amd/fused.py
--- a/flow2gan_amd/fused.py
+++ b/flow2gan_amd/fused.py
@@ -139,17 +139,23 @@
     return out, z, (a, p, None, zsplit)
 
 
+def block_accumulators(bp: _Blk, dev):
+    Cc, Hh = bp.C, bp.H
+    return ops.zeros_many(
+        [(Cc, Hh), (Cc,), (Hh,), (Hh,), (Hh, Cc), (Cc,), (1,), (Cc, 1, bp.K), (Cc,), (Cc, 1)], dev)
+
+
 def block_bwd(bp: _Blk, x, z, a, gout, B, F, lens, limit_norm: bool, limit_scale: bool,
               cproj=None, ldcp=0, Fc=0, up=1, cp_off=0, te=None, ldte=0, te_off=0, g_cproj=None,
-              g_te=None, g_cproj_store=False):
+              g_te=None, g_cproj_store=False, acc=None):
     a, p_act, share, zsplit = a
     if share is None:
         share = ops.split_sharing()
     dev = x.device
     rows, Cc, Hh = B * F, bp.C, bp.H
-    (g_w2, g_b2, g_alpha, g_b1, g_w1, g_beta, g_ls, g_wdw, g_bdw, g_gamma) = ops.zeros_many(
-        [(Cc, Hh), (Cc,), (Hh,), (Hh,), (Hh, Cc), (Cc,), (1,), (Cc, 1, bp.K), (Cc,), (Cc, 1)], dev)
-    ops.colsum(g_b2, gout, rows, Cc)
+    (g_w2, g_b2, g_alpha, g_b1, g_w1, g_beta, g_ls, g_wdw, g_bdw, g_gamma) = (
+        acc if acc is not None else block_accumulators(bp, dev))
+    ops.colsum(g_b2, gout, rows, Cc, late=True)
     with share, ops.split_sharing(gout):
         ops.wgrad(gout, Cc, gout.stride(0), mat(p_act, rows, Hh), g_w2)
         gemm(mat(gout, rows, Cc), mat(bp.w2.reshape(Cc, Hh)), a, form=1, aux=a, alpha_n=bp.alpha,
@@ -220,6 +226,7 @@
         return x
 
     @staticmethod
+    @ops.tailed
     def backward(ctx, g):
         melr, wp, h0, saved = ctx.saved
         params = ctx.params
@@ -231,17 +238,19 @@
         blks = [_Blk(list(params[4 + i * 10: 14 + i * 10])) for i in range(nblk)]
         g = g.contiguous()
         grads_blocks = [None] * nblk
+        with ops.weight_batch():
+            accs = [block_accumulators(bp, dev) for bp in blks]
+            g_beta, g_ls, g_bin, g_wp = ops.zeros_many([(Cc,), (1,), (Cc,), (Cc, 3 * nm)], dev)
         for i in reversed(range(nblk)):
             x, z, a = saved[i]
             fn, fs = ctx.flags[1 + i]
-            g, gb = block_bwd(blks[i], x, z, a, g, B, Fm, ctx.lens, fn, fs)
+            g, gb = block_bwd(blks[i], x, z, a, g, B, Fm, ctx.lens, fn, fs, acc=accs[i])
             grads_blocks[i] = gb
-        g_beta, g_ls, g_bin, g_wp = ops.zeros_many([(Cc,), (1,), (Cc,), (Cc, 3 * nm)], dev)
         gh0 = ops.empty(rows, Cc, device=dev)
         ops.biasnorm_bwd(h0, g, gh0, rows, Cc, beta_in, ls_in.reshape(1), g_beta, g_ls)
         if ctx.flags[0]:
             ops.limit_grad(g_ls, ls_in.reshape(1), -1.5, 1.5)
-        ops.colsum(g_bin, gh0, rows, Cc)
+        ops.colsum(g_bin, gh0, rows, Cc, late=True)
         ops.wgrad(gh0, Cc, gh0.stride(0), win1d(melr, B, Fm, nm, Fm, 1, 1, 3), g_wp)
         g_win = ops.empty(Cc, nm, 3, device=dev)
         ops.permute4(g_win, g_wp, (Cc, nm, 3, 1), (3 * nm, 1, nm, 0))
@@ -333,6 +342,7 @@
         return cproj
 
     @staticmethod
+    @ops.tailed
     def backward(ctx, g):
         cext, (a, pact), cm, wstack = ctx.saved
         params = ctx.params
@@ -344,11 +354,11 @@
         NC = nblk * Cc
         g_wstack, g_bstack, g_b2, g_w2, g_alpha, g_b0, g_w0 = ops.zeros_many(
             [(NC, Dc), (NC,), (Dc,), (Dc, Hc), (Hc,), (Hc,), (Hc, Dc)], dev)
-        ops.colsum(g_bstack, g, rows, NC)
+        ops.colsum(g_bstack, g, rows, NC, late=True)
         ops.wgrad(g, NC, g.stride(0), mat(cm, rows, Dc), g_wstack)
         g_cm = ops.empty(rows, Dc, device=dev)
         gemm(mat(g, rows, NC), mat(wstack), g_cm, form=1)
-        ops.colsum(g_b2, g_cm, rows, Dc)
+        ops.colsum(g_b2, g_cm, rows, Dc, late=True)
         ops.wgrad(g_cm, Dc, g_cm.stride(0), mat(pact, rows, Hc), g_w2)
         gemm(mat(g_cm, rows, Dc), mat(w2.reshape(Dc, Hc)), a, form=1, aux=a, alpha_n=alpha,
              colsum_alpha=g_alpha, colsum=g_b0)
@@ -459,17 +469,17 @@
     g_tew, g_teb, g_tb2, g_tw2, g_tb0, g_tw0 = acc
     dev = g_te_all.device
     Dt, Ht, NC = bv.Dt, bv.Ht, bv.nblk * bv.C
-    ops.colsum(g_teb, g_te_all, B, NC)
+    ops.colsum(g_teb, g_te_all, B, NC, late=True)
     ops.wgrad(g_te_all, NC, NC, mat(te, B, Dt), g_tew)
     g_te = ops.empty(B, Dt, device=dev)
     gemm(mat(g_te_all, B, NC), mat(tew), g_te, form=1)
-    ops.colsum(g_tb2, g_te, B, Dt)
+    ops.colsum(g_tb2, g_te, B, Dt, late=True)
     ops.wgrad(g_te, Dt, Dt, mat(ts, B, Ht), g_tw2)
     g_ts = ops.empty(B, Ht, device=dev)
     gemm(mat(g_te, B, Dt), mat(bv.tw2), g_ts, form=1)
     g_th = ops.empty(B, Ht, device=dev)
     ops.silu_bwd(g_th, g_ts, th)
-    ops.colsum(g_tb0, g_th, B, Ht)
+    ops.colsum(g_tb0, g_th, B, Ht, late=True)
     ops.wgrad(g_th, Ht, Ht, mat(emb, B, Dt), g_tw0)
 
 
@@ -637,6 +647,7 @@
                         pred, B, x.shape[1], wscale)
 
 
+@ops.tailed
 def _branch_backward(bv: _BranchView, meta, sv, x_shape, cproj, g_pred, wbranch_row, wscale,
                      lens_f, g_x, accumulate_gx, g_cproj, need_gx, lanes=None):
     n_fft, hop, up, window = meta
@@ -661,10 +672,12 @@
     if lens_f is not None:
         ops.mask_rows(gy, B, F, Cin, lens_f)
     Dt, Ht = bv.Dt, bv.Ht
-    (g_wout, g_bout, g_te_all, g_beta, g_ls, g_bin, g_win, g_tew, g_teb, g_tb2, g_tw2, g_tb0,
-     g_tw0) = ops.zeros_many([(Cin, Cc), (Cin,), (B, NC), (Cc,), (1,), (Cc,), (Cc, Cin), (NC, Dt), (NC,), (Dt,),
-                              (Dt, Ht), (Ht,), (Ht, Dt)], dev)
-    ops.colsum(g_bout, gy, rows, Cin)
+    with ops.weight_batch():
+        (g_wout, g_bout, g_te_all, g_beta, g_ls, g_bin, g_win, g_tew, g_teb, g_tb2, g_tw2, g_tb0,
+         g_tw0) = ops.zeros_many([(Cin, Cc), (Cin,), (B, NC), (Cc,), (1,), (Cc,), (Cc, Cin), (NC, Dt), (NC,), (Dt,),
+                                  (Dt, Ht), (Ht,), (Ht, Dt)], dev)
+        accs = [block_accumulators(blk, dev) for blk in bv.blks]
+    ops.colsum(g_bout, gy, rows, Cin, late=True)
     x_last = sv["x_last"]
     ops.wgrad(gy, Cin, ldp, mat(x_last, rows, Cc), g_wout)
     g = ops.empty(rows, Cc, device=dev)
@@ -676,13 +689,13 @@
         fn, fs = flags[1 + j]
         g, gb = block_bwd(bv.blks[j], xj, z, a, g, B, F, lens_f, fn, fs, cproj, NC, Fce, up,
                           j * Cc, sv["te_all"], NC, j * Cc, g_cproj=g_cproj, g_te=g_te_all,
-                          g_cproj_store=True)
+                          g_cproj_store=True, acc=accs[j])
         block_grads[j] = gb
     gh0 = ops.empty(rows, Cc, device=dev)
     ops.biasnorm_bwd(sv["h0"], g, gh0, rows, Cc, bv.beta_in, bv.ls_in.reshape(1), g_beta, g_ls)
     if flags[0]:
         ops.limit_grad(g_ls, bv.ls_in.reshape(1), -1.5, 1.5)
-    ops.colsum(g_bin, gh0, rows, Cc)
+    ops.colsum(g_bin, gh0, rows, Cc, late=True)
     ops.wgrad(gh0, Cc, gh0.stride(0), mat(sv["packed"], rows, Cin), g_win)
     if need_gx:
         gpacked = ops.empty(rows, ldp, device=dev)
diff --git a/flow2gan_amd/fused_disc.py b/flow2gan_amd/fused_disc.py
--- a/flow2gan_amd/fused_disc.py
+++ b/flow2gan_amd/fused_disc.py
@@ -89,13 +89,17 @@
     ops.period_fold(img, x2, S2, T, p, H)
     acts, hs = [img], [H]
     shares = [None] * 6
+    for l in range(5):
+        hs.append((hs[l] + 4 - 5) // MPD_STRIDE[l] + 1)
+    with ops.weight_batch():
+        ys = [_halo_rows(S, hs[l + 1], MPD_CH[l + 1], dev, x3=(0 < l < 4)) for l in range(5)]
     x = img
     for l in range(5):
         w, b = prm[2 * l], prm[2 * l + 1]
         Cin, Cout, st = MPD_CH[l], MPD_CH[l + 1], MPD_STRIDE[l]
-        Hout = (H + 4 - 5) // st + 1
+        Hout = hs[l + 1]
         wp = ops.derived(w, "pack", pack_conv_weight)
-        y = _halo_rows(S, Hout, Cout, dev, x3=(0 < l < 4))
+        y = ys[l]
         if l == 0:
             ops.mpd0_fwd(x, S, H, Hout, HALO, w.reshape(Cout, 5), b, SLOPE, y)
         else:
@@ -107,7 +111,6 @@
             else:
                 gemm(A, mat(wp), y, bias=b, lrelu=SLOPE, rowmap=_halo_map(Hout, Cout), x3_out=(l < 4))
         acts.append(y)
-        hs.append(Hout)
         x, H = y, Hout
     wpost, bpost = prm[10], prm[11]
     wpp = ops.derived(wpost, "pack", pack_conv_weight)
@@ -126,11 +129,16 @@
     return ops.derived(w, ("dgradT", stride, j0, nt), build)
 
 
-def _conv1d_dgrad(g_pre, S, Hout, Cout, w, stride, pad, Hin, mask=None, fm=None, colsum=None):
+def _dgrad_wants_image(Cin: int) -> bool:
+    return 2 * Cin >= ops.X6_MIN_K
+
+
+def _conv1d_dgrad(g_pre, S, Hout, Cout, w, stride, pad, Hin, mask=None, fm=None, colsum=None, gx=None):
     Cin, K = w.shape[1], w.shape[2] * w.shape[3]
     dev = g_pre.device
-    want_img = 2 * Cin >= ops.X6_MIN_K
-    gx = _halo_rows(S, Hin, Cin, dev, x3=want_img)
+    want_img = _dgrad_wants_image(Cin)
+    if gx is None:
+        gx = _halo_rows(S, Hin, Cin, dev, x3=want_img)
     for rho, j0, nt, e0, Lq in _residues(K, stride, pad, Hin):
         if Lq == 0:
             continue
@@ -147,6 +155,9 @@
     def __init__(self, st, Sx: int, roff: int, g1, train_disc: bool):
         self.acts, self.hs, self.Sx, self.roff, self.g1, self.train_disc = st["acts"], st["hs"], Sx, roff, g1, train_disc
 
+    def in_producer(self, l_out) -> bool:
+        return l_out == 5 or (ops.GEMM_PRECISION == 3 and l_out in (3, 4))
+
     def __call__(self, l_out, producer, cs):
         y, Sx, g1 = self.acts[l_out], self.Sx, self.g1
         Hp_, C_ = self.hs[l_out] + 2 * HALO, y.shape[1]
@@ -154,7 +165,7 @@
         fk = None
         if (not self.train_disc) and l_out >= 2:
             fk = (y, 0, 1.0 / (Sx * self.hs[l_out] * C_), g1)
-        if l_out == 5 or (ops.GEMM_PRECISION == 3 and l_out in (3, 4)):
+        if self.in_producer(l_out):
             return producer(mk, fk, cs)
         gm = producer(None, None, None)
         gm._f2g_x3_bad = True
@@ -172,6 +183,9 @@
 
     def __init__(self, st, B: int, ups: dict):
         self.acts, self.hs, self.S, self.p, self.B, self.ups = st["acts"], st["hs"], st["S"], st["p"], B, ups
+
+    def in_producer(self, l_out) -> bool:
+        return False
 
     def __call__(self, l_out, producer, cs):
         gm = producer(None, None, None)
@@ -191,6 +205,7 @@
         return gm
 
 
+@ops.tailed
 def _mpd_backward_one(st, prm: list, gs, seqs, need_w: bool, need_x: bool, land, top: int = 4):
     acts, hs, S = st["acts"], st["hs"], st["S"]
     Sx, roff = seqs
@@ -198,11 +213,21 @@
     grads_p = [None] * 12
     unpack = []
     zbuf = None
-    if need_w:
-        zshapes = [(1, 3 * 1024), (1,)]
-        for l in range(5):
-            zshapes += [(MPD_CH[l + 1], 5 * MPD_CH[l]), (MPD_CH[l + 1],)]
-        zbuf = ops.zeros_many(zshapes, dev)
+    if gs is not None:
+        top = 4
+    gmaps = {}
+    with ops.weight_batch():
+        if need_w:
+            zshapes = [(1, 3 * 1024), (1,)]
+            for l in range(5):
+                zshapes += [(MPD_CH[l + 1], 5 * MPD_CH[l]), (MPD_CH[l + 1],)]
+            zbuf = ops.zeros_many(zshapes, dev)
+        if gs is not None:
+            gmaps[5] = _halo_rows(Sx, hs[5], 1024, dev, x3=land.in_producer(5))
+        else:
+            gmaps[top + 1] = ops.zeros(Sx * (hs[top + 1] + 2 * HALO), MPD_CH[top + 1], device=dev)
+        for l in range(top, 0, -1):
+            gmaps[l] = _halo_rows(Sx, hs[l], MPD_CH[l], dev, x3=_dgrad_wants_image(MPD_CH[l]))
 
     def bias_acc(l_out):
         return zbuf[2 * l_out + 1] if need_w else None
@@ -212,15 +237,13 @@
         if need_w:
             ops.mpdpost_wgrad(acts[5], S, H5, HALO, gs, zbuf[0])
             unpack.append((10, zbuf[0], wpost.shape))
-            ops.colsum(zbuf[1], gs, S * H5, 1)
+            ops.colsum(zbuf[1], gs, S * H5, 1, late=True)
             grads_p[11] = zbuf[1]
         g = land(5, lambda mk, fk, ck: ops.mpdpost_dgrad(
             gs, Sx, H5, HALO, ops.derived(wpost, "pack", pack_conv_weight),
-            _halo_rows(Sx, H5, 1024, dev, x3=mk is not None), g_off=roff * H5, mask=mk, fm=fk, colsum=ck), bias_acc(5))
-        top = 4
+            gmaps.pop(5), g_off=roff * H5, mask=mk, fm=fk, colsum=ck), bias_acc(5))
     else:
-        g = land(top + 1, lambda mk, fk, ck: ops.zeros(Sx * (hs[top + 1] + 2 * HALO), MPD_CH[top + 1], device=dev),
-                 bias_acc(top + 1))
+        g = land(top + 1, lambda mk, fk, ck: gmaps.pop(top + 1), bias_acc(top + 1))
     for l in reversed(range(top + 1)):
         w = prm[2 * l]
         Cin, Cout, stv = MPD_CH[l], MPD_CH[l + 1], MPD_STRIDE[l]
@@ -239,12 +262,13 @@
                 unpack.append((2 * l, gwp, w.shape))
             if l > 0:
                 g = land(l, lambda mk, fk, ck: _conv1d_dgrad(g, Sx, Hout, Cout, w, stv, 2, Hin, mask=mk, fm=fk,
-                                                             colsum=ck), bias_acc(l))
+                                                             colsum=ck, gx=gmaps.pop(l)), bias_acc(l))
             elif need_x:
                 gx0 = ops.empty(Sx * Hin, 1, device=dev)
                 g = ops.mpd0_dgrad(g, Sx, Hin, Hout, HALO, w.reshape(Cout, 5), gx0)
     if need_w:
         with ops.weight_batch():
+            ops.tail_now()
             for slot_, gwp_, shape_ in unpack:
                 grads_p[slot_] = unpack_conv_grad(gwp_, shape_)
     return (g if need_x else None), grads_p
@@ -563,6 +587,7 @@
         return gm
 
 
+@ops.tailed
 def _mrd_backward_one(st, prm: list, x, win: int, gs, seqs, need_w: bool, need_x: bool, land, tops=None):
     Ft, Wcat, nb, ldp, hop = st["Ft"], st["Wcat"], st["nb"], st["ldp"], st["hop"]
     cat, packed = st["cat"], st["packed"]
@@ -574,21 +599,27 @@
     grads_w = [None] * N_MRD_PARAMS
     unpack = []
     gcat = None
+
+    def accumulators():
+        return ops.zeros_many([(C,)] * 5 + [(C, 3 * kw_ * (2 if l_ == 0 else C))
+                                            for l_, (kw_, _sw) in enumerate(MRD_LAYERS)], dev)
+
+    zs_band = None
+    if need_w:
+        with ops.weight_batch():
+            zs_band = [accumulators() if gs is not None or tops[bi] is not None else None
+                       for bi in range(len(st["bands"]))]
+            if gs is not None:
+                gwp, gb = ops.zeros_many([(1, 9 * C), (1,)], dev)
     if gs is not None:
         wpost = prm[50]
         if need_w:
-            if land.fused:
-                gwp = ops.zeros(1, 9 * C, device=dev)
-            else:
-                gwp, gb = ops.zeros_many([(1, 9 * C), (1,)], dev)
             if direct:
                 ops.convpost_wgrad(cat, S, Ft, Wcat, gs, gwp)
             else:
                 ops.wgrad(gs, 1, 1, win2d(cat, S, Ft, Wcat, C, Wcat, 3, 3, 1, 1, 1), gwp)
             unpack.append((50, gwp, wpost.shape))
-            if land.fused:
-                gb = ops.zeros(1, device=dev)
-            ops.colsum(gb, gs, S * Ft * Wcat, 1)
+            ops.colsum(gb, gs, S * Ft * Wcat, 1, late=True)
             grads_w[51] = gb
         gcat = ops.empty(Sx * Ft * Wcat, C, device=dev)
         if direct:
@@ -605,10 +636,6 @@
     ldc = Wcat * C
     foffs = _mrd_foffs(st)
 
-    def accumulators():
-        return ops.zeros_many([(C,)] * 5 + [(C, 3 * kw_ * (2 if l_ == 0 else C))
-                                            for l_, (kw_, _sw) in enumerate(MRD_LAYERS)], dev)
-
     for bi, (lo, hi) in enumerate(st["bands"]):
         foff, ws, top = foffs[bi], st["widths"][bi], tops[bi]
         if top is None:
@@ -616,7 +643,7 @@
         W4 = ws[5]
         gbs = [None] * 5
         if need_w and not land.fused:
-            zs = accumulators()
+            zs = zs_band[bi]
             gbs, gwps = zs[:5], zs[5:]
         g = None
         if top == 4:
@@ -624,7 +651,7 @@
         else:
             g = land(bi, top, lambda mk, fk, ck: ops.zeros(Sx * Ft * ws[top + 1], C, device=dev), gbs[top])
         if need_w and land.fused:
-            zs = accumulators()
+            zs = zs_band[bi]
             gbs, gwps = zs[:5], zs[5:]
         for l in reversed(range(top + 1)):
             kw, sw = MRD_LAYERS[l]
@@ -660,7 +687,7 @@
                          split_k=ops.split_for(X.rows, tiles))
                 unpack.append(((bi * 5 + l) * 2, gwp, w.shape))
                 if l == 4 and land.fused:
-                    ops.colsum_strided(gbs[4], gcat, S * Ft, W4, C, ldc, foff * C)
+                    ops.colsum_strided(gbs[4], gcat, S * Ft, W4, C, ldc, foff * C, late=True)
                 grads_w[(bi * 5 + l) * 2 + 1] = gbs[l]
             if l > 0:
                 gx = ops.empty(Sx * Ft * Win, Cin, device=dev)
@@ -690,6 +717,7 @@
         ops.peaknorm_bwd(g_x, gxn, x, st["stats"], Sx, T, row_off=soff)
     if need_w:
         with ops.weight_batch():
+            ops.tail_now()
             for slot_, gwp_, shape_ in unpack:
                 grads_w[slot_] = unpack_conv_grad(gwp_, shape_)
     return g_x, grads_w
diff --git a/flow2gan_amd/leaf.py b/flow2gan_amd/leaf.py
--- a/flow2gan_amd/leaf.py
+++ b/flow2gan_amd/leaf.py
@@ -274,6 +274,7 @@
         return ops.rows_to_bct(ops.empty(B, Cc, F, device=dev), y, B, Cc, F)
 
     @staticmethod
+    @ops.tailed
     def backward(ctx, g):
         xr, z, a, cr, cproj, te, tep, lens = ctx.saved
         params = ctx.params
@@ -358,6 +359,7 @@
         return out
 
     @staticmethod
+    @ops.tailed
     def backward(ctx, gy):
         xr, h0, blocks, x_last, tp, cproj, lens = ctx.saved
         B, F = ctx.dims
diff --git a/flow2gan_amd/ops.py b/flow2gan_amd/ops.py
--- a/flow2gan_amd/ops.py
+++ b/flow2gan_amd/ops.py
@@ -22,18 +22,33 @@
 
 def fill_(t, v: float):
     if BATCH is not None and t.numel() > 0:
-        import struct
         n = t.numel()
-        BATCH.add(0, ptr(t), 4 * n, None, 0, (n & 0xffffffff, n >> 32, 0, 0),
-                  (struct.unpack("<i", struct.pack("<f", float(v)))[0], 0, 0, 0), n, (t,))
+        BATCH.add(0, ptr(t), 4 * n, None, 0, (n & 0xffffffff, n >> 32, 0, 0), (_f32_bits(v), 0, 0, 0), n, (t,))
         return t
     call("f2g_fill", ptr(t), float(v), t.numel())
     return t
 
 
+def _f32_bits(v: float) -> int:
+    import struct
+    return struct.unpack("<i", struct.pack("<f", float(v)))[0]
+
+
 def zero_halo(buf, nseq: int, rows_per_seq: int, Cc: int, lo: int, hi: int):
+    global ZERO_HALO_LAUNCHES
+    if (BATCH is not None and MULTI_CAP > 1 and nseq > 0 and Cc > 0 and Cc % 4 == 0 and lo >= 0 and hi >= 0
+            and 0 < lo + hi <= rows_per_seq and ptr(buf) % 16 == 0):
+        BATCH.add(6, ptr(buf), 4 * nseq * rows_per_seq * Cc, None, 0, (nseq, rows_per_seq, Cc, 0), (lo, hi, 0, 0),
+                  nseq * (lo + hi) * (Cc // 4), (buf,))
+        return buf
+    ZERO_HALO_LAUNCHES += 1
     call("f2g_zero_halo", ptr(buf), nseq, rows_per_seq, Cc, lo, hi)
     return buf
+
+
+ZERO_HALO_LAUNCHES = 0
+LIMIT_GRAD_LAUNCHES = 0
+COLSUM_LAUNCHES = 0
 
 
 def pad4(n: int) -> int:
@@ -190,7 +205,7 @@
                 lvl = max(lvl, l)
         return lvl
 
-    def add(self, kind, out_ptr, out_bytes, rd_ptr, rd_bytes, n, s, items, tensors, in_ptr=None, reads_out=False):
+    def add(self, kind, out_ptr, out_bytes, rd_ptr, rd_bytes, n, s, items, tensors, in_ptr=None):
         import bisect
         self.longest = max(self.longest, out_bytes, rd_bytes or 0)
         lvl = self._level_over(self.starts, self.ranges, out_ptr, out_ptr + out_bytes)
@@ -254,6 +269,50 @@
             L.PRE_CALL = None
             b.flush()
         return False
+
+
+TAIL = None
+
+
+class small_tail:
+
+    def __enter__(self):
+        global TAIL
+        self.prev = TAIL
+        if self.prev is None and MULTI_CAP > 1:
+            TAIL = []
+        return self
+
+    def __exit__(self, *exc):
+        global TAIL
+        if self.prev is None and TAIL is not None:
+            todo, TAIL = TAIL, None
+            if exc[0] is None and todo:
+                with weight_batch():
+                    for fn in todo:
+                        fn()
+        return False
+
+
+def tail_now():
+    global TAIL
+    if TAIL and BATCH is not None:
+        todo, TAIL = TAIL, None
+        try:
+            for fn in todo:
+                fn()
+        finally:
+            TAIL = []
+
+
+def tailed(fn):
+    import functools
+
+    @functools.wraps(fn)
+    def run(*args, **kwargs):
+        with small_tail():
+            return fn(*args, **kwargs)
+    return run
 
 
 def rebuild_derived(params) -> int:
@@ -507,13 +566,13 @@
     if parts is not None:
         nrows, ncol = parts.shape[0], Bm.rows
         if colsum is not None and colsum_alpha is not None and ptr(colsum) == ptr(colsum_alpha) + 4 * ncol:
-            call("f2g_colsum", ptr(colsum_alpha), ptr(parts), parts.stride(0), None, 0, nrows, 2 * ncol)
+            _colsum(ptr(colsum_alpha), ptr(parts), parts.stride(0), nrows, 2 * ncol, (colsum_alpha, colsum, parts), True)
             return out
         if colsum_alpha is not None:
-            call("f2g_colsum", ptr(colsum_alpha), ptr(parts), parts.stride(0), None, 0, nrows, ncol)
+            _colsum(ptr(colsum_alpha), ptr(parts), parts.stride(0), nrows, ncol, (colsum_alpha, parts), True)
         if colsum is not None:
-            call("f2g_colsum", ptr(colsum), ptr(parts) + (4 * ncol if colsum_alpha is not None else 0),
-                 parts.stride(0), None, 0, nrows, ncol)
+            _colsum(ptr(colsum), ptr(parts) + (4 * ncol if colsum_alpha is not None else 0), parts.stride(0), nrows,
+                    ncol, (colsum, parts), True)
     return out
 
 
@@ -1512,14 +1571,62 @@
     return x
 
 
-def colsum(out, a, rows, cols, b=None, out_offset=0):
-    call("f2g_colsum", ptr(out) + 4 * out_offset, ptr(a), a.stride(0), ptr(b),
-         b.stride(0) if b is not None else 0, rows, cols)
+COLSUM_SLICE_ROWS = 512
+
+
+def _colsum_entries(out_ptr, a_ptr, ld, rows, cols, acc, tensors, device):
+    nchunk = (cols + 63) // 64
+    rd = 4 * ((rows - 1) * ld + cols)
+    if rows > 2 * COLSUM_SLICE_ROWS:
+        slices = (rows + COLSUM_SLICE_ROWS - 1) // COLSUM_SLICE_ROWS
+        tmp = torch.empty(slices, cols, device=device, dtype=torch.float32)
+        BATCH.add(8, ptr(tmp), 4 * slices * cols, a_ptr, rd, (rows, cols, 0, slices), (ld, cols, COLSUM_SLICE_ROWS, 0),
+                  256 * nchunk * slices, tuple(tensors) + (tmp,))
+        a_ptr, ld, rows, rd, tensors = ptr(tmp), cols, slices, 4 * slices * cols, (tmp,)
+    BATCH.add(8, out_ptr, 4 * cols, a_ptr, rd, (rows, cols, 1 if acc else 0, 1), (ld, 0, rows, 0), 256 * nchunk,
+              tuple(tensors))
+
+
+def _colsum(out_ptr, a_ptr, ld, rows, cols, tensors, late=False):
+    global COLSUM_LAUNCHES
+    if rows <= 0 or cols <= 0:
+        return
+    if late and TAIL is not None and MULTI_CAP > 1:
+        TAIL.append(lambda: _colsum(out_ptr, a_ptr, ld, rows, cols, tensors))
+        return
+    if BATCH is not None and MULTI_CAP > 1:
+        _colsum_entries(out_ptr, a_ptr, ld, rows, cols, True, tensors, tensors[0].device)
+        return
+    COLSUM_LAUNCHES += 1
+    call("f2g_colsum", out_ptr, a_ptr, ld, None, 0, rows, cols)
+
+
+def colsum(out, a, rows, cols, b=None, out_offset=0, late=False):
+    global COLSUM_LAUNCHES
+    if b is None:
+        _colsum(ptr(out) + 4 * out_offset, ptr(a), a.stride(0), rows, cols, (out, a), late)
+        return out
+    COLSUM_LAUNCHES += 1
+    call("f2g_colsum", ptr(out) + 4 * out_offset, ptr(a), a.stride(0), ptr(b), b.stride(0), rows, cols)
     return out
 
 
-def colsum_strided(out, a, nrows, W, Cc, ld, off):
+def colsum_strided(out, a, nrows, W, Cc, ld, off, late=False):
+    global COLSUM_LAUNCHES
+    if late and TAIL is not None and MULTI_CAP > 1:
+        TAIL.append(lambda: colsum_strided(out, a, nrows, W, Cc, ld, off))
+        return
+    if BATCH is not None and MULTI_CAP > 1 and nrows > 0 and W > 0 and Cc > 0:
+        slices = (nrows + COLSUM_SLICE_ROWS - 1) // COLSUM_SLICE_ROWS if nrows > 2 * COLSUM_SLICE_ROWS else 1
+        rps = COLSUM_SLICE_ROWS if slices > 1 else nrows
+        tmp = torch.empty(slices, W * Cc, device=a.device, dtype=torch.float32)
+        BATCH.add(8, ptr(tmp), 4 * slices * W * Cc, ptr(a) + 4 * off, 4 * ((nrows - 1) * ld + W * Cc),
+                  (nrows, W * Cc, 0, slices), (ld, W * Cc, rps, 0), 256 * ((W * Cc + 63) // 64) * slices, (tmp, a))
+        BATCH.add(8, ptr(out), 4 * Cc, ptr(tmp), 4 * slices * W * Cc, (slices * W, Cc, 1, 1), (Cc, 0, slices * W, 0),
+                  256 * ((Cc + 63) // 64), (out, tmp))
+        return
     tmp = zeros(W * Cc, device=a.device)
+    COLSUM_LAUNCHES += 2
     call("f2g_colsum", ptr(tmp), ptr(a) + 4 * off, ld, None, 0, nrows, W * Cc)
     call("f2g_colsum", ptr(out), ptr(tmp), Cc, None, 0, W, Cc)
 
@@ -1551,8 +1658,7 @@
     if BATCH is not None and n0 * n1 * n2 > 0 and min(so0, so1, si0, si1) >= 0:
         BATCH.add(2, ptr(out) + 4 * out_offset, 4 * ((n0 - 1) * so0 + (n1 - 1) * so1 + n2),
                   ptr(x) + 4 * in_offset, 4 * ((n0 - 1) * si0 + (n1 - 1) * si1 + n2),
-                  (n0, n1, n2, 1 if accumulate else 0), (so0, so1, si0, si1), n0 * n1 * n2, (out, x),
-                  reads_out=bool(accumulate))
+                  (n0, n1, n2, 1 if accumulate else 0), (so0, so1, si0, si1), n0 * n1 * n2, (out, x))
         return out
     call("f2g_copy3", ptr(out) + 4 * out_offset, so0, so1, ptr(x) + 4 * in_offset, si0, si1, n0,
          n1, n2, 1 if accumulate else 0)
@@ -1820,7 +1926,18 @@
 
 
 def limit_grad(g, p, lo, hi):
-    call("f2g_limit_grad", ptr(g), ptr(p), float(lo), float(hi), g.numel())
+    global LIMIT_GRAD_LAUNCHES
+    n = g.numel()
+    if MULTI_CAP > 1 and n > 0:
+        if TAIL is not None:
+            TAIL.append(lambda: limit_grad(g, p, lo, hi))
+            return g
+        if BATCH is not None:
+            BATCH.add(7, ptr(g), 4 * n, ptr(p), 4 * n, (n & 0xffffffff, n >> 32, 0, 0),
+                      (_f32_bits(lo), _f32_bits(hi), 0, 0), n, (g, p))
+            return g
+    LIMIT_GRAD_LAUNCHES += 1
+    call("f2g_limit_grad", ptr(g), ptr(p), float(lo), float(hi), n)
     return g
 
 
diff --git a/include/flow2gan_hip.h b/include/flow2gan_hip.h
--- a/include/flow2gan_hip.h
+++ b/include/flow2gan_hip.h
@@ -261,7 +261,7 @@
 int f2g_log_clip(float* x, int64_t n, float clip, f2g_stream_t stream);
 int f2g_fill(float* x, float v, int64_t n, f2g_stream_t stream);
 enum { F2G_MULTI_FILL = 0, F2G_MULTI_PERMUTE4 = 1, F2G_MULTI_COPY3 = 2, F2G_MULTI_SPLIT3 = 3, F2G_MULTI_SPLIT3G = 4,
-       F2G_MULTI_SPLIT_F16 = 5 };
+       F2G_MULTI_SPLIT_F16 = 5, F2G_MULTI_ZERO_HALO = 6, F2G_MULTI_LIMIT_GRAD = 7, F2G_MULTI_COLSUM = 8 };
 #define F2G_MULTI_MAX 48
 typedef struct {
   void* out;
```

Result: slower. 778.9 audio-s/s (-2.3%).
